# DIG-Beihang/RobustART

Measured on AMD Instinct MI355X. Metric: corrupted+attacked images/sec/node (ResNet-50, PGD-7 + IN-C x5), higher is better.
Workload: dtype bf16x3; 1 GPU; per step and GPU: gaussian_noise sev 1..5 on 256 u8 224x224 images -> normalise -> ResNet-50 eval (1280 img) + PGD-Linf-7 eps 2/255 ResNet-50 eval (256 img); global_batch=256, parallelism=dp1, streams=2

## Files before the change

include/robustart_hip.h:

```cpp
#ifndef ROBUSTART_HIP_H
#define ROBUSTART_HIP_H

#include <stddef.h>
#include <stdint.h>

#ifdef __cplusplus
extern "C" {
#endif

typedef void* rart_stream_t;

typedef enum rart_status {
  RART_OK = 0,
  RART_ERR_INVALID = 1,
  RART_ERR_UNSUPPORTED = 2,
  RART_ERR_WORKSPACE = 3,
  RART_ERR_HIP = 4
} rart_status;

enum {
  RART_GAUSSIAN_NOISE = 0, RART_SHOT_NOISE = 1, RART_IMPULSE_NOISE = 2, RART_DEFOCUS_BLUR = 3,
  RART_GLASS_BLUR = 4, RART_MOTION_BLUR = 5, RART_ZOOM_BLUR = 6, RART_SNOW = 7, RART_FROST = 8,
  RART_FOG = 9, RART_BRIGHTNESS = 10, RART_CONTRAST = 11, RART_ELASTIC_TRANSFORM = 12,
  RART_PIXELATE = 13, RART_JPEG_COMPRESSION = 14, RART_SPECKLE_NOISE = 15, RART_GAUSSIAN_BLUR = 16,
// ... 123 lines not shown
int rart_logit_loss(const float* logits, const int64_t* y, const int64_t* y_target, int batch, int classes,
                    int kind, float scale, float* loss_out, float* dlogits_out, int32_t* pred_out,
                    rart_stream_t stream);

typedef struct rart_conv_desc {
  const void* src;
  const void* wgt;
  const float* bias;
  const void* res;
  const void* mask;
  void* dst;
  int32_t batch, grid_h, grid_w;
  int32_t src_h, src_w, src_pix_stride;
  int32_t k_per_tap, n_taps;
  int32_t sy, sx;
  int32_t tap_dy[32], tap_dx[32];
  int64_t tap_src_off[32];
  int32_t n_cols;
  int32_t dst_h, dst_w, dst_sy, dst_sx, dst_oy, dst_ox, dst_pix_stride;
  int32_t flags;
  int32_t n_batched, z_inner, wgt_row_stride, reserved_;
  int64_t src_z_outer, src_z_inner, wgt_z_outer, wgt_z_inner, dst_z_outer, dst_z_inner;
  void* sign_out;
  int64_t dst_pair_off, res_pair_off;
  float* bn_stats_out;
} rart_conv_desc;

int rart_conv_igemm_bf16(const rart_conv_desc* desc_host, rart_stream_t stream);
int rart_igemm_set_bk64_min_k(long long k);
int rart_gemm_small_m_bf16(const void* a, int lda, const void* w, int ldw, const float* bias, void* out, int ldo, int out_is_f32, int m,
                           int n, int k, rart_stream_t stream);
int rart_igemm_set_gemm256(int enable);
int rart_gemm256_supported(long long rows, int k, int n_cols, int src_ld, int dst_ld);

typedef struct rart_gemm_pair_desc {
  const void *a_hi, *a_lo, *w_hi, *w_lo;
  const float* bias;
  const void *res_hi, *res_lo;
  void *dst_hi, *dst_lo;
  void *aux_hi, *aux_lo;
  int M, N, K, lda, ldw, ldc, w_rows;
  int rows_per_image, src_rows_per_image, src_row_off, dst_rows_per_image, dst_row_off;
  int flags, n_batched, z_inner;
  int64_t a_z_outer, a_z_inner, w_z_outer, w_z_inner, c_z_outer, c_z_inner;
  int conv, batch, grid_h, grid_w, src_h, src_w, sy, sx, k_per_tap, n_taps;
  int tap_dy[16], tap_dx[16];
  int dst_h, dst_w, dst_sy, dst_sx, dst_oy, dst_ox;
  const void* mask_bits;
  void* sign_out;
  int tile_n;
  int tile_m;
} rart_gemm_pair_desc;
int rart_gemm_pair_bf16(const rart_gemm_pair_desc* desc_host, rart_stream_t stream);
int rart_gemm_pair_set_schedule(int mode);
int rart_gemm_pair_get_schedule(void);

typedef struct rart_conv_tail_desc {
  const void* a_hi;  const void* a_lo;
  const void* w_hi;  const void* w_lo;
  const void* t_hi;  const void* t_lo;
  const float* bias_mid;
  const float* bias_out;
  const void* mask_mid;  const void* mask_out;
  void* sign_mid;  void* sign_out;
  const void* res_hi;  const void* res_lo;
  void* dst_hi;  void* dst_lo;
  int batch, h, w, c_mid, ldw, relu_mid, relu_out;
  int tap_dy[9], tap_dx[9];
  const void* n_hi;  const void* n_lo;
  const float* bias_next;
  const void* mask_next;
  void* sign_next;
  void* dstn_hi;  void* dstn_lo;
  int relu_next;
} rart_conv_tail_desc;
int rart_conv3x3_tail_pair_supported(int c_mid);
int rart_conv3x3_tail_pair(const rart_conv_tail_desc* desc_host, rart_stream_t stream);

int rart_vit_add_pos_cls_pair(void* x_hi, void* x_lo, const float* cls_pos0, const float* pos, int n, int tokens, int dim,
                              rart_stream_t stream);
int rart_layernorm_pair(const void* x_hi, const void* x_lo, const float* gamma, const float* beta, void* out_hi, void* out_lo, int rows,
                        int dim, int64_t in_row_stride, int64_t out_row_stride, float eps, rart_stream_t stream);
int rart_layernorm_bwd_pair(const void* dy_hi, const void* dy_lo, const void* x_hi, const void* x_lo, const float* gamma,
                            const void* res_hi, const void* res_lo, void* dx_hi, void* dx_lo, int rows, int dim, int64_t dy_row_stride,
                            int64_t x_row_stride, int64_t res_row_stride, int64_t dx_row_stride, float eps, rart_stream_t stream);
int rart_softmax_rows_pair(const float* scores, void* probs_hi, void* probs_lo, int64_t rows, int n_valid, int ld_in, int ld_out,
                           float scale, rart_stream_t stream);
int rart_softmax_bwd_rows_pair(const void* probs_hi, const void* probs_lo, const float* dprobs, void* ds_hi, void* ds_lo, int64_t rows,
                               int n_valid, int ld_p, int ld_dp, int ld_out, float scale, rart_stream_t stream);
int rart_vit_unpatchify_from_f32(const float* dpatches, float* grad, int n, int h, int w, int patch, int64_t ld, const float* std_host,
                                 rart_stream_t stream);
int rart_vit_attention_pair(const void* qkv_hi, const void* qkv_lo, void* out_hi, void* out_lo, int n, int tokens, int heads, int head_dim,
                            rart_stream_t stream);
int rart_vit_attention_bwd_pair(const void* qkv_hi, const void* qkv_lo, const void* out_hi, const void* out_lo, const void* dout_hi,
                                const void* dout_lo, void* dqkv_hi, void* dqkv_lo, float* stats, int n, int tokens, int heads, int head_dim,
                                rart_stream_t stream);

int rart_conv3x3_halo_supported(int channels, int h, int w);
int rart_conv3x3_pack_frag_bf16(const void* w_rows, void* w_frag, int channels, rart_stream_t stream);
int rart_pack_frag_bf16(const void* w_rows, void* w_frag, int rows, int k, rart_stream_t stream);
int rart_conv3x3_halo_bf16(const void* src, const void* wgt, const float* bias, const void* mask_bits, void* sign_out,
                           void* dst, int n, int h, int w, int channels, const int* tap_dy, const int* tap_dx, int relu,
                           rart_stream_t stream);

int rart_bottleneck_fused_supported(int c_io, int c_mid, int h, int w);
int rart_bottleneck_fused_bf16(const void* x, const void* w1, const void* w2, const void* w3, const float* b1, const float* b2,
                               const float* b3, void* m1, void* m2, void* m3, void* out, int n, int h, int w, int c_io,
                               int c_mid, const int* tap_dy, const int* tap_dx, int backward, rart_stream_t stream);

int rart_bottleneck_first_supported(int c_in, int c_mid, int c_out, int h, int w);
int rart_bottleneck_first_bf16(const void* x, const void* w1, const void* w2, const void* w3, const void* w4, const float* b1,
                               const float* b2, const float* b3, void* m1, void* m2, void* m3, void* out, int n, int h, int w,
                               int c_in, int c_mid, int c_out, const int* tap_dy, const int* tap_dx, int backward,
                               rart_stream_t stream);

int rart_bottleneck_s2_fwd_supported(int c_in, int c_mid, int c_out, int h, int w);
int rart_bottleneck_s2_fwd_bf16(const void* x, const void* w1, const void* w2, const void* w3, const void* wd, const float* b1,
                                const float* b2, const float* b3, void* m1, void* m2, void* m3, void* out, int n, int h, int w,
                                int c_in, int c_mid, int c_out, rart_stream_t stream);

int rart_bottleneck_s2_bwd_bf16(const void* g, const void* w3t, const void* w2t, const void* w1t, const void* wdt, const void* m2,
                                const void* m1, const void* m0, void* dx, int n, int h, int w, int c_in, int c_mid, int c_out,
                                rart_stream_t stream);

int rart_bottleneck14_fused_supported(int c_io, int c_mid, int h, int w);
int rart_bottleneck14_fused_bf16(const void* x, const void* w1, const void* w2, const void* w3, const float* b1, const float* b2,
                                 const float* b3, void* m1, void* m2, void* m3, void* out, int n, int h, int w, int c_io,
// ... 241 lines not shown
```

robustart_amd/_lib.py:

```python
import ctypes
import os

_HERE = os.path.dirname(os.path.abspath(__file__))
LIB_PATH = os.path.join(_HERE, 'lib', 'librobustart_hip.so')

c_void_p, c_int, c_size_t, c_u64, c_float = (ctypes.c_void_p, ctypes.c_int, ctypes.c_size_t,
                                              ctypes.c_uint64, ctypes.c_float)
c_double = ctypes.c_double

ABI_VERSION = 110

SIGNATURES = {
    'rart_version': (c_int, []),
    'rart_last_error_string': (ctypes.c_char_p, []),
    'rart_corruption_name': (ctypes.c_char_p, [c_int]),
    'rart_corrupt_workspace_bytes': (c_size_t, [c_int, c_int, c_int, c_int, c_int]),
    'rart_corrupt_u8': (c_int, [c_void_p, c_void_p, c_int, c_int, c_int, c_int, c_int, c_u64, c_u64,
                                ctypes.POINTER(c_void_p), c_int, c_void_p, c_size_t, c_void_p]),
    'rart_stencil_fixed_point_info': (c_int, [c_int, c_int, c_void_p, c_void_p, c_size_t]),
    'rart_noise_multi_u8': (c_int, [c_void_p, ctypes.POINTER(c_void_p), c_int, c_int, c_int, c_int, c_int, ctypes.POINTER(c_int),
                                    ctypes.POINTER(c_u64), c_u64, c_void_p]),
    'rart_frost_textures_u8': (c_int, [c_void_p, c_void_p, c_int, c_int, c_int, c_int, c_void_p, c_int, c_int, c_int, ctypes.POINTER(c_int),
                                       c_u64, c_u64, c_void_p]),
    'rart_pil_resize_workspace_bytes': (c_size_t, [c_int] * 10),
    'rart_pil_resize_u8': (c_int, [c_void_p, c_void_p] + [c_int] * 10 + [c_void_p, c_size_t, c_void_p]),
    'rart_cv_resize_workspace_bytes': (c_size_t, [c_int] * 10),
    'rart_cv_resize_u8': (c_int, [c_void_p, c_void_p] + [c_int] * 10 + [c_void_p, c_size_t, c_void_p]),
    'rart_u8_to_normalized': (c_int, [c_void_p, c_void_p, c_int, c_int, c_int, c_int, c_int, c_void_p]),
    'rart_u8_to_unit_f32_nchw': (c_int, [c_void_p, c_void_p, c_int, c_int, c_int, c_void_p]),
    'rart_rng_uniform_u32': (c_int, [c_void_p, c_int, c_size_t, c_u64, c_u64, c_int, c_void_p]),
    'rart_rng_normal_f32': (c_int, [c_void_p, c_int, c_size_t, c_u64, c_u64, c_int, c_void_p]),
    'rart_set_normal_generator': (c_int, [c_int]),
    'rart_get_normal_generator': (c_int, []),
    'rart_rng_noise_field_f32': (c_int, [c_void_p, c_int, c_size_t, c_u64, c_u64, c_void_p]),
    'rart_attack_workspace_bytes': (c_size_t, [c_int]),
    'rart_attack_init_linf': (c_int, [c_void_p, c_void_p, c_int, c_size_t, c_float, c_float, c_float,
                                      c_u64, c_u64, c_void_p, c_void_p, c_void_p]),
    'rart_pgd_step_linf': (c_int, [c_void_p, c_void_p, c_void_p, c_size_t, c_float, c_float, c_void_p]),
    'rart_pgd_step_l2': (c_int, [c_void_p, c_void_p, c_void_p, c_int, c_size_t, c_float, c_float,
                                 c_void_p, c_size_t, c_void_p]),
    'rart_pgd_step_l1': (c_int, [c_void_p, c_void_p, c_void_p, c_int, c_size_t, c_float, c_float,
                                 c_void_p, c_size_t, c_void_p]),
    'rart_random_start_l1': (c_int, [c_void_p, c_void_p, c_int, c_size_t, c_float, c_u64, c_u64, c_void_p, c_void_p, c_void_p,
                                     c_void_p, c_size_t, c_void_p]),
    'rart_mim_step': (c_int, [c_void_p, c_void_p, c_void_p, c_void_p, c_int, c_size_t, c_float, c_float,
                              c_float, c_void_p, c_size_t, c_void_p]),
    'rart_apgd_init': (c_int, [c_void_p, c_void_p, c_int, c_size_t, c_int, c_float, c_u64, c_u64, c_void_p,
                               c_void_p, c_void_p, c_size_t, c_void_p]),
    'rart_apgd_step': (c_int, [c_void_p, c_void_p, c_void_p, c_void_p, c_void_p, c_int, c_size_t, c_int,
                               c_float, c_float, c_void_p, c_size_t, c_void_p]),
    'rart_square_init_linf': (c_int, [c_void_p, c_void_p, c_int, c_int, c_int, c_int, c_float, c_u64, c_u64, c_void_p, c_void_p,
                                      c_void_p]),
    'rart_rng_signs_f32': (c_int, [c_void_p, c_int, c_int, c_u64, c_u64, c_void_p, c_int, ctypes.c_uint32, c_void_p]),
    'rart_rng_normal_rows_f32': (c_int, [c_void_p, c_int, c_size_t, c_u64, c_void_p, c_int, c_void_p]),
    'rart_square_propose_linf': (c_int, [c_void_p, c_void_p, c_void_p, c_int, c_int, c_int, c_int, c_float, c_int, c_int,
                                         c_int, c_void_p, c_void_p]),
    'rart_fab_project_linf': (c_int, [c_void_p, c_void_p, c_void_p, c_void_p, c_void_p, c_int, c_size_t, c_void_p]),
    'rart_row_dot': (c_int, [c_void_p, c_void_p, c_void_p, c_int, c_size_t, c_void_p]),
    'rart_row_absmax_diff': (c_int, [c_void_p, c_void_p, c_void_p, c_int, c_size_t, c_void_p]),
    'rart_eot_accumulate': (c_int, [c_void_p, c_void_p, c_size_t, c_int, c_float, c_void_p]),
    'rart_square_init_lp': (c_int, [c_void_p, c_void_p, c_int, c_int, c_int, c_int, c_float, c_int, c_int, c_int, c_int, c_int, c_void_p,
                                    c_void_p, c_void_p, c_void_p]),
    'rart_square_propose_lp': (c_int, [c_void_p, c_void_p, c_void_p, c_int, c_int, c_int, c_int, c_float, c_int, c_int, c_int, c_int, c_int,
                                       c_int, c_void_p, c_void_p, c_void_p]),
    'rart_fab_project': (c_int, [c_void_p, c_void_p, c_void_p, c_void_p, c_void_p, c_int, c_size_t, c_int, c_void_p]),
    'rart_row_norm_diff': (c_int, [c_void_p, c_void_p, c_void_p, c_int, c_size_t, c_int, c_void_p]),
    'rart_fab_update': (c_int, [c_void_p, c_void_p, c_void_p, c_void_p, c_void_p, c_int, c_size_t, c_float, c_void_p]),
    'rart_fab_backoff': (c_int, [c_void_p, c_void_p, c_void_p, c_int, c_size_t, c_float, c_void_p]),
    'rart_l1_project': (c_int, [c_void_p, c_void_p, c_void_p, c_int, c_size_t, c_float, c_int, c_int, c_void_p]),
    'rart_row_kth_abs': (c_int, [c_void_p, c_void_p, c_void_p, c_int, c_size_t, c_void_p]),
    'rart_apgd_l1_move': (c_int, [c_void_p, c_void_p, c_void_p, c_void_p, c_void_p, c_void_p, c_int, c_size_t, c_void_p]),
    'rart_row_count_diff': (c_int, [c_void_p, c_void_p, c_void_p, c_int, c_size_t, c_void_p]),
    'rart_select_rows': (c_int, [c_void_p, c_void_p, c_void_p, c_int, c_size_t, c_void_p]),
    'rart_logit_loss': (c_int, [c_void_p, c_void_p, c_void_p, c_int, c_int, c_int, c_float, c_void_p,
                                c_void_p, c_void_p, c_void_p]),
    'rart_conv_igemm_bf16': (c_int, [c_void_p, c_void_p]),
    'rart_conv3x3_halo_supported': (c_int, [c_int, c_int, c_int]),
    'rart_conv3x3_pack_frag_bf16': (c_int, [c_void_p, c_void_p, c_int, c_void_p]),
    'rart_pack_frag_bf16': (c_int, [c_void_p, c_void_p, c_int, c_int, c_void_p]),
    'rart_conv3x3_halo_bf16': (c_int, [c_void_p, c_void_p, c_void_p, c_void_p, c_void_p, c_void_p, c_int, c_int, c_int, c_int,
                                       ctypes.POINTER(c_int), ctypes.POINTER(c_int), c_int, c_void_p]),
    'rart_bottleneck28_fused_supported': (c_int, [c_int, c_int, c_int, c_int]),
    'rart_bottleneck28_fused_bf16': (c_int, [c_void_p] * 11 + [c_int] * 5 + [ctypes.POINTER(c_int), ctypes.POINTER(c_int), c_int,
                                             c_void_p]),
    'rart_bottleneck7_fused_supported': (c_int, [c_int, c_int, c_int, c_int]),
    'rart_bottleneck7_fused_bf16': (c_int, [c_void_p] * 11 + [c_int] * 5 + [ctypes.POINTER(c_int), ctypes.POINTER(c_int), c_int,
                                            c_void_p]),
    'rart_bottleneck_s2_fwd_supported': (c_int, [c_int] * 5),
    'rart_bottleneck_s2_fwd_bf16': (c_int, [c_void_p] * 12 + [c_int] * 6 + [c_void_p]),
    'rart_bottleneck_s2_bwd_bf16': (c_int, [c_void_p] * 9 + [c_int] * 6 + [c_void_p]),
    'rart_bottleneck14_fused_supported': (c_int, [c_int, c_int, c_int, c_int]),
    'rart_bottleneck14_fused_bf16': (c_int, [c_void_p] * 11 + [c_int] * 5 + [ctypes.POINTER(c_int), ctypes.POINTER(c_int), c_int,
                                             c_void_p]),
    'rart_bottleneck_fused_supported': (c_int, [c_int, c_int, c_int, c_int]),
    'rart_bottleneck_first_supported': (c_int, [c_int] * 5),
    'rart_bottleneck_first_bf16': (c_int, [c_void_p] * 12 + [c_int] * 6 + [ctypes.POINTER(c_int), ctypes.POINTER(c_int), c_int,
                                           c_void_p]),
    'rart_bottleneck_fused_bf16': (c_int, [c_void_p] * 11 + [c_int] * 5 + [ctypes.POINTER(c_int), ctypes.POINTER(c_int), c_int,
                                           c_void_p]),
    'rart_igemm_set_bk64_min_k': (c_int, [ctypes.c_longlong]),
    'rart_gemm_small_m_bf16': (c_int, [c_void_p, c_int, c_void_p, c_int, c_void_p, c_void_p, c_int, c_int, c_int, c_int, c_int, c_void_p]),
    'rart_igemm_set_gemm256': (c_int, [c_int]),
    'rart_gemm256_supported': (c_int, [ctypes.c_longlong, c_int, c_int, c_int, c_int]),
    'rart_gemm_pair_bf16': (c_int, [c_void_p, c_void_p]),
    'rart_copy_calibration': (c_int, [c_void_p, c_void_p, ctypes.c_size_t, c_int, c_void_p]),
    'rart_gemm_pair_set_schedule': (c_int, [c_int]),
    'rart_gemm_pair_get_schedule': (c_int, []),
    'rart_pack_jobs_bf16': (c_int, [c_void_p, c_int, c_int, c_void_p]),
    'rart_vit_add_pos_cls_pair': (c_int, [c_void_p, c_void_p, c_void_p, c_void_p, c_int, c_int, c_int, c_void_p]),
    'rart_layernorm_pair': (c_int, [c_void_p] * 6 + [c_int, c_int, ctypes.c_int64, ctypes.c_int64, c_float, c_void_p]),
    'rart_layernorm_bwd_pair': (c_int, [c_void_p] * 9 + [c_int, c_int] + [ctypes.c_int64] * 4 + [c_float, c_void_p]),
    'rart_softmax_rows_pair': (c_int, [c_void_p, c_void_p, c_void_p, ctypes.c_int64, c_int, c_int, c_int, c_float, c_void_p]),
    'rart_softmax_bwd_rows_pair': (c_int, [c_void_p] * 5 + [ctypes.c_int64, c_int, c_int, c_int, c_int, c_float, c_void_p]),
    'rart_vit_attention_pair': (c_int, [c_void_p, c_void_p, c_void_p, c_void_p, c_int, c_int, c_int, c_int, c_void_p]),
    'rart_vit_attention_bwd_pair': (c_int, [c_void_p] * 9 + [c_int, c_int, c_int, c_int, c_void_p]),
    'rart_vit_unpatchify_from_f32': (c_int, [c_void_p, c_void_p, c_int, c_int, c_int, c_int, ctypes.c_int64, ctypes.POINTER(c_float), c_void_p]),
    'rart_engine_prep_input': (c_int, [c_void_p, c_int, c_void_p, c_void_p, c_int, c_int, c_int, c_void_p, c_void_p,
                                       c_void_p]),
    'rart_engine_maxpool': (c_int, [c_void_p, c_void_p, c_void_p, c_int, c_int, c_int, c_int, c_void_p]),
    'rart_engine_maxpool_keep': (c_int, [c_void_p, c_void_p, c_void_p, c_void_p, c_int, c_int, c_int, c_int, c_void_p]),
    'rart_engine_maxpool_bwd': (c_int, [c_void_p, c_void_p, c_void_p, c_void_p, c_int, c_int, c_int, c_int, c_void_p]),
    'rart_engine_avgpool': (c_int, [c_void_p, c_void_p, c_int, c_int, c_int, c_void_p]),
    'rart_engine_avgpool_bwd': (c_int, [c_void_p, c_void_p, c_void_p, c_int, c_int, c_int, c_void_p]),
    'rart_engine_stem_col2im': (c_int, [c_void_p, c_void_p, c_int, c_int, c_int, c_int, c_void_p, c_void_p]),
    'rart_engine_stem_fwd_fused': (c_int, [c_void_p, c_int, c_void_p, c_int, c_void_p, c_void_p, c_void_p, c_void_p, c_int, c_int,
                                           c_int, c_void_p, c_void_p, c_void_p]),
    'rart_wgrad_direct_supported': (c_int, [c_int, c_int, c_int]),
    'rart_wgrad_direct_bf16': (c_int, [c_void_p, c_void_p, c_void_p] + [c_int] * 10 + [c_void_p, c_void_p, c_int, c_int, c_int, c_void_p]),
    'rart_conv3x3_tail_pair_supported': (c_int, [c_int]),
# ... 107 lines not shown
                ('k_per_tap', ctypes.c_int32), ('n_taps', ctypes.c_int32), ('sy', ctypes.c_int32), ('sx', ctypes.c_int32),
                ('tap_dy', ctypes.c_int32 * 32), ('tap_dx', ctypes.c_int32 * 32), ('tap_src_off', ctypes.c_int64 * 32),
                ('n_cols', ctypes.c_int32),
                ('dst_h', ctypes.c_int32), ('dst_w', ctypes.c_int32), ('dst_sy', ctypes.c_int32), ('dst_sx', ctypes.c_int32),
                ('dst_oy', ctypes.c_int32), ('dst_ox', ctypes.c_int32), ('dst_pix_stride', ctypes.c_int32),
                ('flags', ctypes.c_int32),
                ('n_batched', ctypes.c_int32), ('z_inner', ctypes.c_int32), ('wgt_row_stride', ctypes.c_int32),
                ('reserved_', ctypes.c_int32),
                ('src_z_outer', ctypes.c_int64), ('src_z_inner', ctypes.c_int64), ('wgt_z_outer', ctypes.c_int64),
                ('wgt_z_inner', ctypes.c_int64), ('dst_z_outer', ctypes.c_int64), ('dst_z_inner', ctypes.c_int64),
                ('sign_out', c_void_p), ('dst_pair_off', ctypes.c_int64), ('res_pair_off', ctypes.c_int64), ('bn_stats_out', c_void_p)]


class JitterRec(ctypes.Structure):
    _fields_ = [('op', ctypes.c_uint8 * 4), ('factor', ctypes.c_float * 3), ('hue_shift', ctypes.c_uint32)]


class JpegInfo(ctypes.Structure):
    _fields_ = [(n, ctypes.c_int32) for n in ('status', 'height', 'width', 'ncomp')] + \
               [(n, ctypes.c_int32 * 3) for n in ('h_samp', 'v_samp', 'blocks_w', 'blocks_h')] + \
               [('coef_count', ctypes.c_int64), ('qt', (ctypes.c_uint16 * 64) * 3)]


class JpegDesc(ctypes.Structure):
    _fields_ = [('block_start', ctypes.c_int64 * 3), ('plane_off', ctypes.c_int64 * 3), ('qt_off', ctypes.c_int64),
                ('out_off', ctypes.c_int64)] + \
               [(n, ctypes.c_int32) for n in ('height', 'width', 'ncomp', 'h_samp', 'v_samp')] + \
               [('blocks_w', ctypes.c_int32 * 3), ('blocks_h', ctypes.c_int32 * 3), ('reserved_', ctypes.c_int32)]


class FixedPointInfo(ctypes.Structure):
    _fields_ = [(n, ctypes.c_int32) for n in ('kind', 'ksize', 'n_steps', 'frac_bits', 'out_frac_bits')] + \
               [('corr', ctypes.c_longlong), ('band', ctypes.c_longlong), ('max_abs_weight_error', ctypes.c_double),
                ('sum_abs_weight_error', ctypes.c_double)]


class PackJob(ctypes.Structure):
    _fields_ = [(n, ctypes.c_int32) for n in ('kind', 'n_out', 'channels', 'r', 's', 'n_taps', 'transpose', 'rows_padded', 'rows', 'k')] + \
               [('tap_r', ctypes.c_int32 * 16), ('tap_s', ctypes.c_int32 * 16), ('weight', c_void_p), ('out_channel_scale', c_void_p),
                ('src16', c_void_p), ('out', c_void_p)]


class GemmPairDesc(ctypes.Structure):
    _fields_ = [(n, c_void_p) for n in ('a_hi', 'a_lo', 'w_hi', 'w_lo', 'bias', 'res_hi', 'res_lo', 'dst_hi', 'dst_lo', 'aux_hi', 'aux_lo')] + \
               [(n, ctypes.c_int32) for n in ('M', 'N', 'K', 'lda', 'ldw', 'ldc', 'w_rows', 'rows_per_image', 'src_rows_per_image',
                                              'src_row_off', 'dst_rows_per_image', 'dst_row_off', 'flags', 'n_batched', 'z_inner')] + \
               [(n, ctypes.c_int64) for n in ('a_z_outer', 'a_z_inner', 'w_z_outer', 'w_z_inner', 'c_z_outer', 'c_z_inner')] + \
               [(n, ctypes.c_int32) for n in ('conv', 'batch', 'grid_h', 'grid_w', 'src_h', 'src_w', 'sy', 'sx', 'k_per_tap', 'n_taps')] + \
               [('tap_dy', ctypes.c_int32 * 16), ('tap_dx', ctypes.c_int32 * 16)] + \
               [(n, ctypes.c_int32) for n in ('dst_h', 'dst_w', 'dst_sy', 'dst_sx', 'dst_oy', 'dst_ox')] + \
               [('mask_bits', c_void_p), ('sign_out', c_void_p), ('tile_n', ctypes.c_int32), ('tile_m', ctypes.c_int32)]


class TokmixDesc(ctypes.Structure):
    _fields_ = [(n, c_void_p) for n in ('a_hi', 'a_lo', 'x_hi', 'x_lo', 'dst_hi', 'dst_lo', 'res_hi', 'res_lo', 'aux_hi', 'aux_lo', 'bias')] + \
               [(n, ctypes.c_int32) for n in ('M', 'N', 'K', 'lda', 'ldx', 'ldc', 'batch', 'flags')] + \
               [(n, ctypes.c_int64) for n in ('x_stride', 'c_stride')]


class TokmixWgradDesc(ctypes.Structure):
    _fields_ = [(n, c_void_p) for n in ('p', 'q', 'partial')] + \
               [(n, ctypes.c_int32) for n in ('M', 'N', 'D', 'batch', 'splits', 'images_per_split', 'ld_partial', 'reserved')] + \
               [(n, ctypes.c_int64) for n in ('p_stride', 'q_stride')]


class ConvTailDesc(ctypes.Structure):
    _fields_ = [(n, c_void_p) for n in ('a_hi', 'a_lo', 'w_hi', 'w_lo', 't_hi', 't_lo', 'bias_mid', 'bias_out', 'mask_mid', 'mask_out',
                                        'sign_mid', 'sign_out', 'res_hi', 'res_lo', 'dst_hi', 'dst_lo')] + \
               [(n, ctypes.c_int32) for n in ('batch', 'h', 'w', 'c_mid', 'ldw', 'relu_mid', 'relu_out')] + \
               [('tap_dy', ctypes.c_int32 * 9), ('tap_dx', ctypes.c_int32 * 9)] + \
               [(n, c_void_p) for n in ('n_hi', 'n_lo', 'bias_next', 'mask_next', 'sign_next', 'dstn_hi', 'dstn_lo')] + [('relu_next', ctypes.c_int32)]


_lib = None


class RartError(RuntimeError):

    def __init__(self, status, message):
        super().__init__('robustart_hip status %d: %s' % (status, message))
        self.status = status


def load():
    global _lib
    if _lib is not None:
        return _lib
    if not os.path.exists(LIB_PATH):
        raise RuntimeError(
            'robustart_amd: %s is missing -- build it with `python robustart_amd/csrc/build.py` '
            '(or __graft_entry__.build()).  There is no CPU fallback for the product path.' % LIB_PATH)
    import torch
    lib = ctypes.CDLL(LIB_PATH)
    for name, (res, args) in SIGNATURES.items():
        fn = getattr(lib, name)
        fn.restype = res
        fn.argtypes = args
    got = lib.rart_version()
    if got != ABI_VERSION:
        raise RuntimeError('robustart_amd: %s reports ABI version %d, this binding expects %d (struct layouts / signatures '
                           'differ) -- rebuild it with `python robustart_amd/csrc/build.py --force`' % (LIB_PATH, got, ABI_VERSION))
    _lib = lib
    return lib


def check(status):
    if status != 0:
        raise RartError(status, load().rart_last_error_string().decode('utf-8', 'replace'))


def require_gpu():
    import torch
    if not torch.cuda.is_available():
        raise RuntimeError('robustart_amd: no GPU visible (torch.cuda.is_available() is False); '
                           'the HIP hot path has no CPU fallback')
    return torch


def stream_ptr():
    import torch
    return c_void_p(torch.cuda.current_stream().cuda_stream)


def ptr(t):
# ... 18 lines not shown
```

robustart_amd/csrc/conv_tail_pair.hip:

```cpp
#include "rart_common.h"
#include "rart_lds_dma.h"

typedef __attribute__((ext_vector_type(8))) __bf16 bf16x8;
typedef __attribute__((ext_vector_type(16))) float f32x16;

namespace {
constexpr int CT_TM = 128;
constexpr int CT_LDE = 68;
constexpr int CT_PLANE_A = CT_TM * 64;
constexpr int CT_NLD = 144;
constexpr int CT_WREG = 2 * 32 * CT_NLD;
static_assert(CT_WREG >= 32 * CT_LDE * 4, "the staging must fit the wave's region");

struct ConvTailDev {
  const uint16_t *a_hi, *a_lo, *w_hi, *w_lo, *t_hi, *t_lo;
  const float *bias_mid, *bias_out;
  const uint8_t *mask_mid, *mask_out;
  uint8_t *sign_mid, *sign_out;
  const uint16_t *res_hi, *res_lo;
  uint16_t *dst_hi, *dst_lo;
  int M, H, W, ldw, relu_mid, relu_out;
  int tap_dy[9], tap_dx[9];
  uint32_t w_magic, w_shift, h_magic, h_shift;
  const uint16_t *n_hi, *n_lo;
  const float* bias_next;
  const uint8_t* mask_next;
  uint8_t* sign_next;
  uint16_t *dstn_hi, *dstn_lo;
  int relu_next;
};
typedef __attribute__((ext_vector_type(4))) uint32_t ct_u4;
__device__ __forceinline__ uint4 ct_nt_load(const uint16_t* p) {
  const ct_u4 v = __builtin_nontemporal_load(reinterpret_cast<const ct_u4*>(p));
  return make_uint4(v[0], v[1], v[2], v[3]);
}
__device__ __forceinline__ void ct_nt_store(uint16_t* p, const uint4& v) {
  ct_u4 w = {v.x, v.y, v.z, v.w};
  __builtin_nontemporal_store(w, reinterpret_cast<ct_u4*>(p));
}
__device__ __forceinline__ uint32_t ct_fastdiv(uint32_t n, uint32_t magic, uint32_t shift) { return (uint32_t)(((uint64_t)n * magic) >> shift); }

__device__ __forceinline__ uint32_t ct_pack_bf16x2(float lo, float hi) {
  typedef __attribute__((ext_vector_type(2))) float f2_t;
  typedef __attribute__((ext_vector_type(2))) __bf16 b2_t;
  f2_t f = {lo, hi};
  return __builtin_bit_cast(uint32_t, __builtin_convertvector(f, b2_t));
}
__device__ __forceinline__ void ct_split8(const float* v, uint4& hi, uint4& lo) {
  uint32_t h[4], l[4];
#pragma unroll
  for (int j = 0; j < 4; ++j) {
    h[j] = ct_pack_bf16x2(v[2 * j], v[2 * j + 1]);
    l[j] = ct_pack_bf16x2(v[2 * j] - __uint_as_float(h[j] << 16), v[2 * j + 1] - __uint_as_float(h[j] & 0xFFFF0000u));
  }
  hi = make_uint4(h[0], h[1], h[2], h[3]);
  lo = make_uint4(l[0], l[1], l[2], l[3]);
}
__device__ __forceinline__ void ct_join8(const uint4& hi, const uint4& lo, float* v) {
  const uint32_t h[4] = {hi.x, hi.y, hi.z, hi.w}, l[4] = {lo.x, lo.y, lo.z, lo.w};
#pragma unroll
  for (int j = 0; j < 4; ++j) {
    v[2 * j] = __uint_as_float(h[j] << 16) + __uint_as_float(l[j] << 16);
    v[2 * j + 1] = __uint_as_float(h[j] & 0xFFFF0000u) + __uint_as_float(l[j] & 0xFFFF0000u);
  }
}
__device__ __forceinline__ uint32_t ct_sign_byte(const uint4& v) {
  const uint32_t hw[4] = {v.x, v.y, v.z, v.w};
  uint32_t sb = 0;
#pragma unroll
  for (int j = 0; j < 4; ++j) {
    sb |= ((short)(hw[j] & 0xFFFFu) > 0 ? 1u : 0u) << (2 * j);
    sb |= ((short)(hw[j] >> 16) > 0 ? 1u : 0u) << (2 * j + 1);
  }
  return sb;
}

template <int NJ>
__device__ __forceinline__ void ct_pointwise_frags(const f32x16* acc, const uint32_t* mw, bool relu, int h, uint4* fh, uint4* fl) {
#pragma unroll
  for (int j = 0; j < NJ; ++j)
#pragma unroll
    for (int ge = 0; ge < 4; ge += 2) {
      uint32_t eh[2], el[2], oh[2], ol[2];
#pragma unroll
      for (int w = 0; w < 2; ++w) {
        float ve[2], vo[2];
#pragma unroll
        for (int i = 0; i < 2; ++i) {
          ve[i] = acc[j][4 * ge + 2 * w + i];
          vo[i] = acc[j][4 * ge + 4 + 2 * w + i];
          if (relu) { ve[i] = fmaxf(ve[i], 0.f); vo[i] = fmaxf(vo[i], 0.f); }
          if (!((mw[j] >> (8 * ge + 4 * h + 2 * w + i)) & 1u)) ve[i] = 0.f;
          if (!((mw[j] >> (8 * ge + 8 + 4 * h + 2 * w + i)) & 1u)) vo[i] = 0.f;
        }
        eh[w] = ct_pack_bf16x2(ve[0], ve[1]);
        el[w] = ct_pack_bf16x2(ve[0] - __uint_as_float(eh[w] << 16), ve[1] - __uint_as_float(eh[w] & 0xFFFF0000u));
        oh[w] = ct_pack_bf16x2(vo[0], vo[1]);
        ol[w] = ct_pack_bf16x2(vo[0] - __uint_as_float(oh[w] << 16), vo[1] - __uint_as_float(oh[w] & 0xFFFF0000u));
        const auto sh = __builtin_amdgcn_permlane32_swap(eh[w], oh[w], false, false);
        eh[w] = sh[0]; oh[w] = sh[1];
        const auto sl = __builtin_amdgcn_permlane32_swap(el[w], ol[w], false, false);
        el[w] = sl[0]; ol[w] = sl[1];
      }
      fh[j * 2 + ge / 2] = make_uint4(eh[0], eh[1], oh[0], oh[1]);
      fl[j * 2 + ge / 2] = make_uint4(el[0], el[1], ol[0], ol[1]);
    }
}

template <int C, bool NEXT>
__global__ __launch_bounds__(256, (C == 64 && !NEXT) ? 3 : 2) void k_conv3x3_tail_pair(const ConvTailDev d) {
  constexpr int NJ = C / 32;
  constexpr int KS = C / 16;
  constexpr int NOUT = 4 * C, NC = NOUT / 64;
  constexpr int TPT_SHIFT = C == 64 ? 1 : 2;
  constexpr int KT = 9 << TPT_SHIFT;
  constexpr int PLANE_B = C * 64, STAGE = 2 * CT_PLANE_A + 2 * PLANE_B;
  constexpr int BQ = (C / 16) / 4;
  static_assert(4 * CT_WREG <= 2 * STAGE, "the waves' epilogue regions must fit the tile buffers");
  __shared__ __attribute__((aligned(16))) uint8_t lds[2 * STAGE];
  const int tid = threadIdx.x, lane = tid & 63;
  const int wave = __builtin_amdgcn_readfirstlane(tid >> 6);
  uint32_t tile;
  {
    const uint32_t nb = gridDim.x, bid = blockIdx.x, xcd = bid & 7u, slot = bid >> 3, q = nb >> 3, r = nb & 7u;
    tile = (xcd < r ? xcd * (q + 1u) : r * (q + 1u) + (xcd - r) * q) + slot;
  }
  const int m0 = (int)tile * CT_TM;

  uint32_t avoff[2], nok[2] = {0u, 0u};
  int tap_min = 0;
  for (int t = 0; t < 9; ++t) tap_min = min(tap_min, (d.tap_dy[t] * d.W + d.tap_dx[t]) * (C * 2));
  const int tapreg = lane < 9 ? (d.tap_dy[lane] * d.W + d.tap_dx[lane]) * (C * 2) - tap_min : 0;
#pragma unroll
  for (int q = 0; q < 2; ++q) {
    const int r = 16 * (wave + 4 * q) + (lane >> 2);
    const int cs = ((lane & 3) ^ ((r >> 2) & 3)) * 16;
    const int m = m0 + r;
    const bool ok = m < d.M;
    const uint32_t mm = ok ? (uint32_t)m : 0u;
    const uint32_t t = ct_fastdiv(mm, d.w_magic, d.w_shift);
    const int ax = (int)(mm - t * (uint32_t)d.W);
    const int n = (int)ct_fastdiv(t, d.h_magic, d.h_shift);
    const int ay = (int)(t - (uint32_t)n * (uint32_t)d.H);
    avoff[q] = (uint32_t)((n * d.H * d.W + ay * d.W + ax) * (C * 2) + cs);
    for (int t2 = 0; t2 < 9; ++t2) {
      const int iy = ay + d.tap_dy[t2], ix = ax + d.tap_dx[t2];
      if (!(ok && (unsigned)iy < (unsigned)d.H && (unsigned)ix < (unsigned)d.W)) nok[q] |= 1u << t2;
    }
  }
  uint32_t wvoff[BQ];
#pragma unroll
  for (int q = 0; q < BQ; ++q) {
    const int r = 16 * (wave + 4 * q) + (lane >> 2);
    wvoff[q] = (uint32_t)((r * d.ldw + (((lane & 3) ^ ((r >> 2) & 3)) * 8)) * 2);
  }
  const rart_srd_t srd_ah = rart_dma_srd(reinterpret_cast<const char*>(d.a_hi) + tap_min), srd_al = rart_dma_srd(reinterpret_cast<const char*>(d.a_lo) + tap_min);
  const rart_srd_t srd_wh = rart_dma_srd(d.w_hi), srd_wl = rart_dma_srd(d.w_lo);
  const uint32_t lds_base = (uint32_t)(uintptr_t)(__attribute__((address_space(3))) uint8_t*)lds;
#define RART_CT_ISSUE(KT_, BUF)                                                                                 \
  {                                                                                                             \
    const uint32_t st_ = lds_base + (BUF)*STAGE;                                                                \
    const int kt_ = (KT_);                                                                                      \
    const int tap_ = kt_ >> TPT_SHIFT;                                                                          \
// ... 19 lines not shown
    for (int g = 0; g < 4; ++g) {
      float4 bv = make_float4(0.f, 0.f, 0.f, 0.f);
      if (d.bias_mid) bv = *reinterpret_cast<const float4*>(d.bias_mid + j * 32 + 8 * g + 4 * h);
      acc[j][4 * g] = bv.x; acc[j][4 * g + 1] = bv.y; acc[j][4 * g + 2] = bv.z; acc[j][4 * g + 3] = bv.w;
    }
  RART_CT_ISSUE(0, 0)
  rart_dma_wait<0>();
  __syncthreads();
  for (int kt = 0; kt < KT; ++kt) {
    const int buf = kt & 1;
    if (kt + 1 < KT) RART_CT_ISSUE(kt + 1, buf ^ 1)
    const uint8_t* Pb = lds + buf * STAGE + (wave * 32) * 64;
    const uint8_t* Wb = lds + buf * STAGE + 2 * CT_PLANE_A;
#pragma unroll
    for (int ks = 0; ks < 2; ++ks) {
      const bf16x8 ph = *reinterpret_cast<const bf16x8*>(Pb + xo[ks]);
      const bf16x8 pl = *reinterpret_cast<const bf16x8*>(Pb + CT_PLANE_A + xo[ks]);
#pragma unroll
      for (int j = 0; j < NJ; ++j) {
        const bf16x8 wh = *reinterpret_cast<const bf16x8*>(Wb + j * 32 * 64 + xo[ks]);
        const bf16x8 wl = *reinterpret_cast<const bf16x8*>(Wb + PLANE_B + j * 32 * 64 + xo[ks]);
        acc[j] = __builtin_amdgcn_mfma_f32_32x32x16_bf16(wh, pl, acc[j], 0, 0, 0);
        acc[j] = __builtin_amdgcn_mfma_f32_32x32x16_bf16(wl, ph, acc[j], 0, 0, 0);
        acc[j] = __builtin_amdgcn_mfma_f32_32x32x16_bf16(wh, ph, acc[j], 0, 0, 0);
      }
    }
    rart_dma_wait<0>();
    __syncthreads();
  }
#undef RART_CT_ISSUE

  const int p = m0 + wave * 32 + fr;
  const bool p_ok = p < d.M;
  bf16x8 a2h[KS], a2l[KS];
  {
    uint32_t mw[NJ];
#pragma unroll
    for (int j = 0; j < NJ; ++j) mw[j] = 0xFFFFFFFFu;
    if (d.mask_mid && p_ok) {
      const uint32_t* mp = reinterpret_cast<const uint32_t*>(d.mask_mid + (size_t)p * (C / 8));
#pragma unroll
      for (int j = 0; j < NJ; ++j) mw[j] = mp[j];
    }
    uint4 fh[KS], fl[KS];
    ct_pointwise_frags<NJ>(acc, mw, d.relu_mid != 0, h, fh, fl);
#pragma unroll
    for (int s = 0; s < KS; ++s) {
      a2h[s] = __builtin_bit_cast(bf16x8, fh[s]);
      a2l[s] = __builtin_bit_cast(bf16x8, fl[s]);
      if (d.sign_mid && p_ok) d.sign_mid[(size_t)p * (C / 8) + 2 * s + h] = (uint8_t)ct_sign_byte(fh[s]);
    }
  }

  uint8_t* const wreg = lds + wave * CT_WREG;
  float* sE = reinterpret_cast<float*>(wreg);
  const int cw = lane & 7, rw = lane >> 3;
  f32x16 accn[NEXT ? NJ : 1];
  if (NEXT) {
#pragma unroll
    for (int j = 0; j < NJ; ++j)
#pragma unroll
      for (int g = 0; g < 4; ++g) {
        float4 bv = make_float4(0.f, 0.f, 0.f, 0.f);
        if (d.bias_next) bv = *reinterpret_cast<const float4*>(d.bias_next + j * 32 + 8 * g + 4 * h);
        accn[j][4 * g] = bv.x; accn[j][4 * g + 1] = bv.y; accn[j][4 * g + 2] = bv.z; accn[j][4 * g + 3] = bv.w;
      }
  }
  const uint4* th_base = reinterpret_cast<const uint4*>(d.t_hi) + lane;
  const uint4* tl_base = reinterpret_cast<const uint4*>(d.t_lo) + lane;
  const bool relu_out = d.relu_out != 0;
#pragma unroll 1
  for (int c = 0; c < NC; ++c) {
    int eo[4];
    uint4 rh[4], rl[4];
    uint32_t mb[4];
#pragma unroll
    for (int q = 0; q < 4; ++q) {
      const int pp = m0 + wave * 32 + q * 8 + rw;
      eo[q] = -1;
      rh[q] = rl[q] = make_uint4(0, 0, 0, 0);
      mb[q] = 0xFFu;
      if (pp < d.M) {
        const int e = pp * NOUT + c * 64 + cw * 8;
        eo[q] = e;
        if (d.res_hi) {
          rh[q] = ct_nt_load(d.res_hi + e);
          rl[q] = ct_nt_load(d.res_lo + e);
        }
        if (d.mask_out) mb[q] = d.mask_out[e >> 3];
      }
    }
    f32x16 acc2[2];
#pragma unroll
    for (int b = 0; b < 2; ++b) {
#pragma unroll
      for (int g = 0; g < 4; ++g) {
        float4 bv = make_float4(0.f, 0.f, 0.f, 0.f);
        if (d.bias_out) bv = *reinterpret_cast<const float4*>(d.bias_out + c * 64 + b * 32 + 8 * g + 4 * h);
        acc2[b][4 * g] = bv.x; acc2[b][4 * g + 1] = bv.y; acc2[b][4 * g + 2] = bv.z; acc2[b][4 * g + 3] = bv.w;
      }
#pragma unroll
      for (int sg = 0; sg < KS; sg += 4) {
        uint4 th[4], tl[4];
#pragma unroll
        for (int s = 0; s < 4; ++s) {
          th[s] = th_base[((c * 2 + b) * KS + sg + s) * 64];
          tl[s] = tl_base[((c * 2 + b) * KS + sg + s) * 64];
        }
#pragma unroll
        for (int s = 0; s < 4; ++s) {
          const bf16x8 wh = __builtin_bit_cast(bf16x8, th[s]), wl = __builtin_bit_cast(bf16x8, tl[s]);
          acc2[b] = __builtin_amdgcn_mfma_f32_32x32x16_bf16(wh, a2l[sg + s], acc2[b], 0, 0, 0);
          acc2[b] = __builtin_amdgcn_mfma_f32_32x32x16_bf16(wl, a2h[sg + s], acc2[b], 0, 0, 0);
          acc2[b] = __builtin_amdgcn_mfma_f32_32x32x16_bf16(wh, a2h[sg + s], acc2[b], 0, 0, 0);
        }
      }
    }
#pragma unroll
    for (int b = 0; b < 2; ++b)
#pragma unroll
      for (int g = 0; g < 4; ++g)
        *reinterpret_cast<float4*>(sE + fr * CT_LDE + b * 32 + 8 * g + 4 * h) =
            make_float4(acc2[b][4 * g], acc2[b][4 * g + 1], acc2[b][4 * g + 2], acc2[b][4 * g + 3]);
    __builtin_amdgcn_fence(__ATOMIC_RELEASE, "wavefront");
    __builtin_amdgcn_wave_barrier();
    __builtin_amdgcn_fence(__ATOMIC_ACQUIRE, "wavefront");
    uint4 oph[4], opl[4];
#pragma unroll
    for (int q = 0; q < 4; ++q) {
      const int r = q * 8 + rw;
      const float4 v0 = *reinterpret_cast<const float4*>(sE + r * CT_LDE + cw * 8);
      const float4 v1 = *reinterpret_cast<const float4*>(sE + r * CT_LDE + cw * 8 + 4);
      const int e = eo[q];
      oph[q] = opl[q] = make_uint4(0, 0, 0, 0);
      if (e >= 0) {
        float v[8] = {v0.x, v0.y, v0.z, v0.w, v1.x, v1.y, v1.z, v1.w};
        if (d.res_hi) {
          float rv[8];
          ct_join8(rh[q], rl[q], rv);
#pragma unroll
          for (int j = 0; j < 8; ++j) v[j] += rv[j];
        }
#pragma unroll
        for (int j = 0; j < 8; ++j)
          if (!((mb[q] >> j) & 1u)) v[j] = 0.f;
        if (relu_out) {
#pragma unroll
          for (int j = 0; j < 8; ++j) v[j] = fmaxf(v[j], 0.f);
        }
        uint4 ph, pl;
        ct_split8(v, ph, pl);
        ct_nt_store(d.dst_hi + e, ph);
        ct_nt_store(d.dst_lo + e, pl);
        if (d.sign_out) d.sign_out[e >> 3] = (uint8_t)ct_sign_byte(ph);
        oph[q] = ph;
        opl[q] = pl;
      }
    }
    __builtin_amdgcn_fence(__ATOMIC_RELEASE, "wavefront");
    __builtin_amdgcn_wave_barrier();
    if (NEXT) {
#pragma unroll
      for (int q = 0; q < 4; ++q) {
        *reinterpret_cast<uint4*>(wreg + (q * 8 + rw) * CT_NLD + cw * 16) = oph[q];
        *reinterpret_cast<uint4*>(wreg + 32 * CT_NLD + (q * 8 + rw) * CT_NLD + cw * 16) = opl[q];
      }
      __builtin_amdgcn_fence(__ATOMIC_RELEASE, "wavefront");
      __builtin_amdgcn_wave_barrier();
      __builtin_amdgcn_fence(__ATOMIC_ACQUIRE, "wavefront");
// ... 17 lines not shown
        for (int s = 0; s < 4; ++s) {
          const bf16x8 wh = __builtin_bit_cast(bf16x8, nh[s]), wl = __builtin_bit_cast(bf16x8, nl[s]);
          accn[j] = __builtin_amdgcn_mfma_f32_32x32x16_bf16(wh, xl[s], accn[j], 0, 0, 0);
          accn[j] = __builtin_amdgcn_mfma_f32_32x32x16_bf16(wl, xh[s], accn[j], 0, 0, 0);
          accn[j] = __builtin_amdgcn_mfma_f32_32x32x16_bf16(wh, xh[s], accn[j], 0, 0, 0);
        }
      }
      __builtin_amdgcn_fence(__ATOMIC_RELEASE, "wavefront");
      __builtin_amdgcn_wave_barrier();
    }
  }
  if (NEXT) {
    uint32_t mw[NJ];
#pragma unroll
    for (int j = 0; j < NJ; ++j) mw[j] = 0xFFFFFFFFu;
    if (d.mask_next && p_ok) {
      const uint32_t* mp = reinterpret_cast<const uint32_t*>(d.mask_next + (size_t)p * (C / 8));
#pragma unroll
      for (int j = 0; j < NJ; ++j) mw[j] = mp[j];
    }
    uint4 fh[KS], fl[KS];
    ct_pointwise_frags<NJ>(accn, mw, d.relu_next != 0, h, fh, fl);
    if (p_ok) {
#pragma unroll
      for (int s = 0; s < KS; ++s) {
        ct_nt_store(d.dstn_hi + (size_t)p * C + 16 * s + 8 * h, fh[s]);
        ct_nt_store(d.dstn_lo + (size_t)p * C + 16 * s + 8 * h, fl[s]);
        if (d.sign_next) d.sign_next[(size_t)p * (C / 8) + 2 * s + h] = (uint8_t)ct_sign_byte(fh[s]);
      }
    }
  }
}

void ct_magic(uint32_t dv, uint32_t& mg, uint32_t& sh) {
  uint32_t l = 0;
  while ((1ull << l) < dv) ++l;
  sh = 31 + l;
  mg = (uint32_t)(((1ull << sh) + dv - 1) / dv);
}
}

extern "C" int rart_conv3x3_tail_pair_supported(int c_mid) { return (c_mid == 64 || c_mid == 128) ? 1 : 0; }

extern "C" int rart_conv3x3_tail_pair(const rart_conv_tail_desc* t, rart_stream_t stream) {
  RART_CHECK_ARG(t != nullptr, "rart_conv3x3_tail_pair: null descriptor");
  RART_CHECK_ARG(t->a_hi && t->a_lo && t->w_hi && t->w_lo && t->t_hi && t->t_lo && t->dst_hi && t->dst_lo,
                 "rart_conv3x3_tail_pair: null operand plane");
  RART_CHECK_ARG(t->c_mid == 64 || t->c_mid == 128, "rart_conv3x3_tail_pair: c_mid must be 64 or 128 (layer1 / layer2)");
  RART_CHECK_ARG(t->batch > 0 && t->h > 0 && t->w > 0, "rart_conv3x3_tail_pair: empty geometry");
  RART_CHECK_ARG((t->res_hi == nullptr) == (t->res_lo == nullptr), "rart_conv3x3_tail_pair: the skip is a pair: both planes or none");
  RART_CHECK_ARG(t->ldw % 8 == 0 && t->ldw >= 9 * t->c_mid, "rart_conv3x3_tail_pair: ldw must cover 9 taps x c_mid and keep 16-byte alignment");
  const long long M = (long long)t->batch * t->h * t->w;
  RART_CHECK_ARG(M * 4 * t->c_mid < (1ll << 31), "rart_conv3x3_tail_pair: tensors must stay below 2^31 elements (split the batch)");
  ConvTailDev d;
  d.a_hi = (const uint16_t*)t->a_hi; d.a_lo = (const uint16_t*)t->a_lo; d.w_hi = (const uint16_t*)t->w_hi; d.w_lo = (const uint16_t*)t->w_lo;
  d.t_hi = (const uint16_t*)t->t_hi; d.t_lo = (const uint16_t*)t->t_lo;
  d.bias_mid = t->bias_mid; d.bias_out = t->bias_out;
  d.mask_mid = (const uint8_t*)t->mask_mid; d.mask_out = (const uint8_t*)t->mask_out;
  d.sign_mid = (uint8_t*)t->sign_mid; d.sign_out = (uint8_t*)t->sign_out;
  d.res_hi = (const uint16_t*)t->res_hi; d.res_lo = (const uint16_t*)t->res_lo;
  d.dst_hi = (uint16_t*)t->dst_hi; d.dst_lo = (uint16_t*)t->dst_lo;
  d.M = (int)M; d.H = t->h; d.W = t->w; d.ldw = t->ldw; d.relu_mid = t->relu_mid; d.relu_out = t->relu_out;
  for (int i = 0; i < 9; ++i) { d.tap_dy[i] = t->tap_dy[i]; d.tap_dx[i] = t->tap_dx[i]; }
  const bool next = t->n_hi != nullptr;
  RART_CHECK_ARG(!next || (t->n_lo && t->dstn_hi && t->dstn_lo), "rart_conv3x3_tail_pair: the neighbour's reduction needs both table planes and its destination pair");
  d.n_hi = (const uint16_t*)t->n_hi; d.n_lo = (const uint16_t*)t->n_lo; d.bias_next = t->bias_next; d.mask_next = (const uint8_t*)t->mask_next;
  d.sign_next = (uint8_t*)t->sign_next; d.dstn_hi = (uint16_t*)t->dstn_hi; d.dstn_lo = (uint16_t*)t->dstn_lo; d.relu_next = t->relu_next;
  ct_magic((uint32_t)d.W, d.w_magic, d.w_shift);
  ct_magic((uint32_t)d.H, d.h_magic, d.h_shift);
  const dim3 grid((uint32_t)((M + CT_TM - 1) / CT_TM));
  hipStream_t st = (hipStream_t)stream;
  if (t->c_mid == 64) {
    if (next) hipLaunchKernelGGL((k_conv3x3_tail_pair<64, true>), grid, dim3(256), 0, st, d);
    else hipLaunchKernelGGL((k_conv3x3_tail_pair<64, false>), grid, dim3(256), 0, st, d);
  } else {
    if (next) hipLaunchKernelGGL((k_conv3x3_tail_pair<128, true>), grid, dim3(256), 0, st, d);
    else hipLaunchKernelGGL((k_conv3x3_tail_pair<128, false>), grid, dim3(256), 0, st, d);
  }
  RART_CHECK_LAUNCH("rart_conv3x3_tail_pair");
  return RART_OK;
}
```

robustart_amd/csrc/gemm_pair.hip:

```cpp
#include "rart_common.h"
#include <stdlib.h>

#include "rart_gemm_pair_dev.h"
#include "rart_lds_dma.h"

namespace {
template <int TM, int TN, bool CONV>
__global__ __launch_bounds__(TM * 2, 1) void k_gemm_pair(const GemmPairDev d) {
  constexpr int NW = TM / 32;
  constexpr int WN = (TN / 64 < NW) ? TN / 64 : NW, WM = NW / WN, RW = TM / WM, MI = RW / 32, NJ = TN / (32 * WN);
  static_assert(NJ == 2, "a wave owns 64 columns");
  constexpr int GP_PLANE_A = TM * GP_BK * 2;
  constexpr int PLANE_B = TN * GP_BK * 2, STAGE = 2 * GP_PLANE_A + 2 * PLANE_B;
  constexpr int A_PIECES = TM / 16, AQ = A_PIECES / NW;
  constexpr int B_PIECES = TN / 16, BQ = (B_PIECES + NW - 1) / NW;
  constexpr int GP_STAGING = NW * 32 * GP_LDE * 4;
  static_assert(AQ == 2, "two A pieces per wave");
  static_assert(GP_STAGING + TM * 4 <= 2 * STAGE, "epilogue staging + row table must fit the tile buffers");
  __shared__ __attribute__((aligned(16))) uint8_t lds[2 * STAGE];
  const int tid = threadIdx.x, lane = tid & 63;
  const int wave = __builtin_amdgcn_readfirstlane(tid >> 6), wm = wave / WN, wn = wave % WN;
  const uint16_t *a_hi = d.a_hi, *a_lo = d.a_lo, *w_hi = d.w_hi, *w_lo = d.w_lo;
  long long c_off = 0;
  if (!CONV && gridDim.y > 1) {
    const int z = blockIdx.y, zo = z / d.z_inner, zi = z - zo * d.z_inner;
    const long long ao = zo * d.a_zo + zi * d.a_zi, wo = zo * d.w_zo + zi * d.w_zi;
    a_hi += ao; a_lo += ao; w_hi += wo; w_lo += wo;
    c_off = zo * d.c_zo + zi * d.c_zi;
  }
  const int TMV = d.tile_rows;
  const int n_tiles = (d.N + TN - 1) / TN, m_tiles = (d.M + TMV - 1) / TMV;
  int m_tile, n_tile;
  if (m_tiles >= 16) {
    const int bid = blockIdx.x, xcd = bid & 7, slot = bid >> 3;
    m_tile = (slot / n_tiles) * 8 + xcd;
    n_tile = slot % n_tiles;
    if (m_tile >= m_tiles) return;
  } else {
    m_tile = blockIdx.x / n_tiles;
    n_tile = blockIdx.x - m_tile * n_tiles;
  }
  const int m0 = m_tile * TMV, n0 = n_tile * TN;

  uint32_t avoff[2], nok[2] = {0u, 0u};
  int tapreg = 0, tap_min = 0;
  const bool one_tap = !CONV || d.n_taps == 1;
  if (CONV) {
    for (int t = 0; t < d.n_taps; ++t) tap_min = min(tap_min, (d.tap_dy[t] * d.src_w + d.tap_dx[t]) * d.lda * 2);
    if (lane < d.n_taps) tapreg = (d.tap_dy[lane] * d.src_w + d.tap_dx[lane]) * d.lda * 2 - tap_min;
  }
  const uint32_t tap0 = CONV ? (uint32_t)__builtin_amdgcn_readfirstlane((d.tap_dy[0] * d.src_w + d.tap_dx[0]) * d.lda * 2 - tap_min) : 0u;
#pragma unroll
  for (int q = 0; q < 2; ++q) {
    const int r = 16 * (wave + NW * q) + (lane >> 2);
    const int csrc = (lane & 3) ^ ((r >> 2) & 3);
    const int m = m0 + r;
    const bool ok = m < d.M;
    if (CONV) {
      const uint32_t mm = ok ? (uint32_t)m : 0u;
      const uint32_t t = gp_fastdiv(mm, d.gw_magic, d.gw_shift);
      const int ox = (int)(mm - t * (uint32_t)d.grid_w);
      const int n = (int)gp_fastdiv(t, d.gh_magic, d.gh_shift);
      const int oy = (int)(t - (uint32_t)n * (uint32_t)d.grid_h);
      const int by = oy * d.sy, bx = ox * d.sx;
      avoff[q] = (uint32_t)((n * d.src_h * d.src_w + by * d.src_w + bx) * d.lda * 2 + csrc * 16);
      for (int t2 = 0; t2 < d.n_taps; ++t2) {
        const int iy = by + d.tap_dy[t2], ix = bx + d.tap_dx[t2];
        if (!(ok && (unsigned)iy < (unsigned)d.src_h && (unsigned)ix < (unsigned)d.src_w)) nok[q] |= 1u << t2;
      }
      if (one_tap && (nok[q] & 1u)) avoff[q] = RART_DMA_OOR;
    } else {
      long long srow = m;
      if (d.map_rows) {
        const int img = m / d.rpi;
        srow = (long long)img * d.src_rpi + (m - img * d.rpi);
      }
      avoff[q] = ok ? (uint32_t)(((srow + d.src_off) * d.lda + csrc * 8) * 2) : RART_DMA_OOR;
    }
  }
  uint32_t wvoff[BQ];
#pragma unroll
  for (int q = 0; q < BQ; ++q) {
    const int r = 16 * (wave + NW * q) + (lane >> 2);
    const int csrc = (lane & 3) ^ ((r >> 2) & 3);
    const int n = n0 + r;
    wvoff[q] = (r < TN && n < d.w_rows) ? (uint32_t)((n * d.ldw + csrc * 8) * 2) : RART_DMA_OOR;
  }
  const rart_srd_t srd_ah = rart_dma_srd(reinterpret_cast<const char*>(a_hi) + tap_min), srd_al = rart_dma_srd(reinterpret_cast<const char*>(a_lo) + tap_min);
  const rart_srd_t srd_wh = rart_dma_srd(w_hi), srd_wl = rart_dma_srd(w_lo);
  const uint32_t lds_base = (uint32_t)(uintptr_t)(__attribute__((address_space(3))) uint8_t*)lds;
  const int w_step = (d.flags & GP_W_INTERLEAVED) ? 128 : 64;
#define RART_GP_ISSUE(KT, BUF)                                                                                  \
  {                                                                                                             \
    const uint32_t st_ = lds_base + (BUF)*STAGE;                                                                \
    const int kt_ = (KT);                                                                                       \
    if (one_tap) {                                                                                              \
      const uint32_t so_ = tap0 + (uint32_t)kt_ * 64u;                                                          \
      _Pragma("unroll") for (int q = 0; q < 2; ++q) {                                                           \
        rart_dma_load16(avoff[q], srd_ah, so_, st_ + (wave + NW * q) * 1024);                                   \
        rart_dma_load16(avoff[q], srd_al, so_, st_ + GP_PLANE_A + (wave + NW * q) * 1024);                      \
      }                                                                                                         \
    } else {                                                                                                    \
      const int tap_ = kt_ >> d.tpt_shift;                                                                      \
      const uint32_t so_ = (uint32_t)(__builtin_amdgcn_readlane(tapreg, tap_) + (kt_ - (tap_ << d.tpt_shift)) * 64); \
      _Pragma("unroll") for (int q = 0; q < 2; ++q) {                                                           \
        const uint32_t vo_ = avoff[q] | ((uint32_t)__builtin_amdgcn_sbfe(nok[q], tap_, 1) & RART_DMA_OOR);      \
        rart_dma_load16(vo_, srd_ah, so_, st_ + (wave + NW * q) * 1024);                                        \
        rart_dma_load16(vo_, srd_al, so_, st_ + GP_PLANE_A + (wave + NW * q) * 1024);                           \
      }                                                                                                         \
    }                                                                                                           \
    {                                                                                                           \
      const uint32_t so_ = (uint32_t)(kt_ * w_step);                                                            \
      _Pragma("unroll") for (int q = 0; q < BQ; ++q) {                                                          \
        if (NW * q + NW <= B_PIECES || wave + NW * q < B_PIECES) {     \
          rart_dma_load16(wvoff[q], srd_wh, so_, st_ + 2 * GP_PLANE_A + (wave + NW * q) * 1024);                \
          rart_dma_load16(wvoff[q], srd_wl, so_, st_ + 2 * GP_PLANE_A + PLANE_B + (wave + NW * q) * 1024);      \
        }                                                                                                       \
      }                                                                                                         \
    }                                                                                                           \
  }
  const int fr = lane & 31, h = lane >> 5;
  uint32_t xo[2];
#pragma unroll
  for (int ks = 0; ks < 2; ++ks) xo[ks] = (uint32_t)(fr * 64 + (((2 * ks + h) ^ ((fr >> 2) & 3)) << 4));
  f32x16 acc[MI][2];
#pragma unroll
  for (int j = 0; j < 2; ++j) {
    const int bc = n0 + wn * 64 + j * 32 + fr;
    const float bv = (d.bias && bc < d.N) ? d.bias[bc] : 0.f;
#pragma unroll
    for (int i = 0; i < MI; ++i)
#pragma unroll
      for (int r = 0; r < 16; ++r) acc[i][j][r] = bv;
  }
  const int KT = d.K / GP_BK;
  const bool skip_last = wm * RW + MI * 32 > TMV;
  RART_GP_ISSUE(0, 0)
  rart_dma_wait<0>();
  __syncthreads();
  for (int kt = 0; kt < KT; ++kt) {
    const int buf = kt & 1;
    if (kt + 1 < KT) RART_GP_ISSUE(kt + 1, buf ^ 1)
    const uint8_t* Ah = lds + buf * STAGE + (wm * RW) * 64;
    const uint8_t* Bh = lds + buf * STAGE + 2 * GP_PLANE_A + (wn * 64) * 64;
#pragma unroll
    for (int ks = 0; ks < 2; ++ks) {
      bf16x8 ah[MI], al[MI], bh[2], bl[2];
#pragma unroll
      for (int i = 0; i < MI; ++i) {
// ... 23 lines not shown
  gp_epilogue<TM, TN, CONV, MI>(d, lds, acc, m0, n0, c_off, TMV);
}

int g_pair_schedule = -1;
int gp_schedule() {
  if (g_pair_schedule < 0) {
    const char* e = getenv("RART_PAIR_SCHEDULE");
    g_pair_schedule = e ? atoi(e) : 1;
  }
  return g_pair_schedule;
}

int gp_rows224() {
  const char* e = getenv("RART_PAIR_ROWS224");
  return e ? atoi(e) : 1;
}
int gp_split() {
  const char* e = getenv("RART_PAIR_SPLIT");
  return e ? atoi(e) : 1;
}

void gp_magic(uint32_t dv, uint32_t& mg, uint32_t& sh) {
  uint32_t l = 0;
  while ((1ull << l) < dv) ++l;
  sh = 31 + l;
  mg = (uint32_t)(((1ull << sh) + dv - 1) / dv);
}
}

bool rart_gemm_pair_pp_launch(const void* dev_desc, int tn, bool conv, unsigned grid_x, unsigned grid_y, hipStream_t st, unsigned walk_wgs);
void rart_gemm_pair_ps_launch(const void* dev_desc, bool conv, unsigned wgs, hipStream_t st);

namespace {
int gp_cu_count() {
  static int cus[64] = {0};
  int dev = 0;
  if (hipGetDevice(&dev) != hipSuccess || dev < 0 || dev >= 64) return 256;
  if (cus[dev] == 0) {
    int n = 0;
    cus[dev] = (hipDeviceGetAttribute(&n, hipDeviceAttributeMultiprocessorCount, dev) == hipSuccess && n > 0) ? n : 256;
  }
  return cus[dev];
}
}

extern "C" int rart_gemm_pair_set_schedule(int mode) {
  RART_CHECK_ARG(mode >= 0 && mode <= 3,
                 "rart_gemm_pair_set_schedule: mode must be 0 (two-stage loop), 1 (ping-pong), 2 (ping-pong + deferred-epilogue persistent) or 3 (ping-pong, tiles walked)");
  g_pair_schedule = mode;
  return RART_OK;
}
extern "C" int rart_gemm_pair_get_schedule(void) { return gp_schedule(); }

extern "C" int rart_gemm_pair_bf16(const rart_gemm_pair_desc* h, rart_stream_t stream) {
  RART_CHECK_ARG(h != nullptr, "rart_gemm_pair_bf16: null descriptor");
  RART_CHECK_ARG(h->a_hi && h->a_lo && h->w_hi && h->w_lo && h->dst_hi, "rart_gemm_pair_bf16: null operand plane");
  const bool conv = h->conv != 0;
  GemmPairDev d;
  d.M = h->M; d.K = h->K;
  if (conv) {
    RART_CHECK_ARG(h->batch > 0 && h->grid_h > 0 && h->grid_w > 0 && h->src_h > 0 && h->src_w > 0 && h->dst_h > 0 && h->dst_w > 0,
                   "rart_gemm_pair_bf16 (conv): empty geometry");
    RART_CHECK_ARG(h->n_taps >= 1 && h->n_taps <= 16, "rart_gemm_pair_bf16 (conv): n_taps must be 1..16");
    RART_CHECK_ARG(h->k_per_tap >= 32 && (h->k_per_tap & (h->k_per_tap - 1)) == 0,
                   "rart_gemm_pair_bf16 (conv): k_per_tap must be a power of two >= 32");
    RART_CHECK_ARG(h->n_batched <= 1 && h->rows_per_image == 0 && h->src_row_off == 0 && h->dst_row_off == 0,
                   "rart_gemm_pair_bf16 (conv): no batching / row re-basing in conv mode");
    const long long M = (long long)h->batch * h->grid_h * h->grid_w;
    RART_CHECK_ARG(M < (1ll << 31), "rart_gemm_pair_bf16 (conv): row grid must stay below 2^31 rows");
    RART_CHECK_ARG((long long)h->batch * h->src_h * h->src_w * h->lda < (1ll << 30) && (long long)h->batch * h->dst_h * h->dst_w * h->ldc < (1ll << 31),
                   "rart_gemm_pair_bf16 (conv): a source plane must stay below 2 GiB (32-bit byte offsets of the stage loads) and the destination "
                   "below 2^31 elements (split the batch)");
    RART_CHECK_ARG(h->lda % 8 == 0 || h->lda == 4, "rart_gemm_pair_bf16 (conv): source pixels must keep 16-byte alignment of the K chunks");
    d.M = (int)M;
    d.K = h->k_per_tap * h->n_taps;
    d.grid_h = h->grid_h; d.grid_w = h->grid_w; d.src_h = h->src_h; d.src_w = h->src_w; d.sy = h->sy; d.sx = h->sx; d.n_taps = h->n_taps;
    int sh = 0;
    while ((32 << sh) < h->k_per_tap) ++sh;
    d.tpt_shift = sh;
    for (int i = 0; i < 16; ++i) { d.tap_dy[i] = i < h->n_taps ? h->tap_dy[i] : 0; d.tap_dx[i] = i < h->n_taps ? h->tap_dx[i] : 0; }
    d.dst_h = h->dst_h; d.dst_w = h->dst_w; d.dst_sy = h->dst_sy; d.dst_sx = h->dst_sx; d.dst_oy = h->dst_oy; d.dst_ox = h->dst_ox;
    gp_magic((uint32_t)d.grid_w, d.gw_magic, d.gw_shift);
    gp_magic((uint32_t)d.grid_h, d.gh_magic, d.gh_shift);
    d.mask_bits = (const uint8_t*)h->mask_bits; d.sign_out = (uint8_t*)h->sign_out;
    RART_CHECK_ARG(!(d.sign_out && (h->flags & GP_OUT_F32)), "rart_gemm_pair_bf16 (conv): sign_out needs a pair destination");
  } else {
    RART_CHECK_ARG(!h->mask_bits && !h->sign_out, "rart_gemm_pair_bf16: mask_bits / sign_out are served by conv mode only");
    RART_CHECK_ARG(h->lda % 8 == 0 && h->lda >= h->K, "rart_gemm_pair_bf16: lda must cover the row and keep 16-byte alignment");
    d.grid_h = d.grid_w = d.src_h = d.src_w = d.sy = d.sx = d.n_taps = 1; d.tpt_shift = 0;
    for (int i = 0; i < 16; ++i) d.tap_dy[i] = d.tap_dx[i] = 0;
    d.dst_h = d.dst_w = d.dst_sy = d.dst_sx = 1; d.dst_oy = d.dst_ox = 0;
    d.gw_magic = d.gw_shift = d.gh_magic = d.gh_shift = 0;
    d.mask_bits = nullptr; d.sign_out = nullptr;
  }
  d.N = h->N;
  RART_CHECK_ARG(d.M > 0 && d.N > 0 && d.N % 8 == 0, "rart_gemm_pair_bf16: M > 0, N a positive multiple of 8");
  RART_CHECK_ARG(d.K > 0 && d.K % GP_BK == 0, "rart_gemm_pair_bf16: K must be a positive multiple of 32");
  RART_CHECK_ARG(h->ldw % 8 == 0 && h->ldc % 8 == 0 && h->ldw >= d.K && h->ldc >= d.N,
                 "rart_gemm_pair_bf16: leading dimensions must cover the row and keep 16-byte alignment");
  RART_CHECK_ARG((long long)(h->w_rows > 0 ? h->w_rows : h->N) * h->ldw < (1ll << 30), "rart_gemm_pair_bf16: a weight plane must stay below 2 GiB");
  if (!conv) {
    const long long imgs = (h->rows_per_image > 0 && h->rows_per_image < d.M) ? (d.M + h->rows_per_image - 1) / h->rows_per_image : 1;
    const long long src_rows = imgs > 1 ? imgs * (h->src_rows_per_image > 0 ? h->src_rows_per_image : h->rows_per_image) : d.M;
    RART_CHECK_ARG((src_rows + h->src_row_off) * h->lda < (1ll << 30), "rart_gemm_pair_bf16: a source plane must stay below 2 GiB (per batched problem)");
  }
  const bool out_f32 = (h->flags & GP_OUT_F32) != 0;
  RART_CHECK_ARG(out_f32 || h->dst_lo, "rart_gemm_pair_bf16: a pair destination needs its lo plane");
  RART_CHECK_ARG((h->res_hi == nullptr) == (h->res_lo == nullptr), "rart_gemm_pair_bf16: the residual is a pair: both planes or none");
  RART_CHECK_ARG(!(h->flags & (GP_GELU_KEEP | GP_GELU_BWD)) || (h->aux_hi && h->aux_lo),
                 "rart_gemm_pair_bf16: GELU_KEEP / GELU_BWD need the pre-activation pair (aux)");
  RART_CHECK_ARG(!(h->flags & ~(GP_OUT_F32 | GP_GELU | GP_GELU_BWD | GP_GELU_KEEP | GP_RELU | GP_W_INTERLEAVED)), "rart_gemm_pair_bf16: unknown flag");
  RART_CHECK_ARG(!(h->flags & GP_W_INTERLEAVED) || h->ldw >= 2 * d.K, "rart_gemm_pair_bf16: an interleaved weight table has rows of 2 K elements");
  {
    const int g = (h->flags & GP_GELU ? 1 : 0) + (h->flags & GP_GELU_BWD ? 1 : 0) + (h->flags & GP_GELU_KEEP ? 1 : 0);
    RART_CHECK_ARG(g <= 1 && !((h->flags & GP_GELU_KEEP) && out_f32), "rart_gemm_pair_bf16: at most one GELU mode; GELU_KEEP writes pairs");
  }
  d.a_hi = (const uint16_t*)h->a_hi; d.a_lo = (const uint16_t*)h->a_lo; d.w_hi = (const uint16_t*)h->w_hi; d.w_lo = (const uint16_t*)h->w_lo;
  d.bias = h->bias; d.res_hi = (const uint16_t*)h->res_hi; d.res_lo = (const uint16_t*)h->res_lo;
  d.dst_hi = (uint16_t*)h->dst_hi; d.dst_lo = (uint16_t*)h->dst_lo; d.aux_hi = (uint16_t*)h->aux_hi; d.aux_lo = (uint16_t*)h->aux_lo;
  d.lda = h->lda; d.ldw = h->ldw; d.ldc = h->ldc;
  d.w_rows = h->w_rows > 0 ? h->w_rows : h->N;
  d.map_rows = (!conv && h->rows_per_image > 0 && h->rows_per_image < d.M) ? 1 : 0;
  d.rpi = d.map_rows ? h->rows_per_image : d.M;
  d.src_rpi = h->src_rows_per_image > 0 ? h->src_rows_per_image : d.rpi;
  d.dst_rpi = h->dst_rows_per_image > 0 ? h->dst_rows_per_image : d.rpi;
  d.src_off = h->src_row_off; d.dst_off = h->dst_row_off;
  RART_CHECK_ARG(d.src_off >= 0 && d.dst_off >= 0, "rart_gemm_pair_bf16: row offsets must be >= 0");
  d.flags = h->flags;
  {
    const char* e = getenv("RART_PAIR_NT_MIN_MB");
    const long long min_mb = e ? atoll(e) : 0;
    d.nt = (long long)d.M * d.N * 4 >= min_mb * (1ll << 20) ? 1 : 0;
  }
  const int nz = h->n_batched > 1 ? h->n_batched : 1;
  RART_CHECK_ARG(nz <= 65535, "rart_gemm_pair_bf16: n_batched must be <= 65535");
  d.z_inner = h->z_inner > 0 ? h->z_inner : 1;
  d.a_zo = h->a_z_outer; d.a_zi = h->a_z_inner; d.w_zo = h->w_z_outer; d.w_zi = h->w_z_inner; d.c_zo = h->c_z_outer; d.c_zi = h->c_z_inner;
  int tn = d.N <= 64 ? 64 : (d.N <= 128 ? 128 : 256), tm = 256;
  if (conv) {
    if (gp_schedule() >= 1 && d.N >= 256 && (d.K >= 512 || (d.K >= 256 && d.N <= 512))) {
      tm = 256;
      tn = (long long)((d.M + 255) / 256) * ((d.N + 255) / 256) < 128 ? 128 : 256;
    } else if (d.K <= 256) { tm = 256; tn = 64; }
    else if (d.K < 1024 || d.N <= 128) { tm = 128; tn = d.N <= 64 ? 64 : 128; }
    else if ((long long)((d.M + 255) / 256) * ((d.N + 255) / 256) < 128) { tm = 256; tn = 128; }
    if (d.M <= 256) { tm = 128; tn = 64; }
  }
  if (h->tile_n == 64 || h->tile_n == 128 || h->tile_n == 256) tn = h->tile_n;
  if (h->tile_m == 128 || h->tile_m == 256) tm = h->tile_m;
  if (h->tile_m == 224) tm = 256;
  const int m_tiles = (d.M + tm - 1) / tm, n_tiles = (d.N + tn - 1) / tn;
  const int m_enum = m_tiles >= 16 ? (m_tiles + 7) / 8 * 8 : m_tiles;
  const long long blocks = (long long)m_enum * n_tiles;
  RART_CHECK_ARG(blocks < (1ll << 31), "rart_gemm_pair_bf16: grid too large");
  const dim3 grid((uint32_t)blocks, nz);
  hipStream_t st = (hipStream_t)stream;
  if (gp_schedule() == 2 && tm == 256 && tn >= 128 && h->tile_n == 0 && h->tile_m == 0 && nz == 1 && !d.map_rows && d.src_off == 0 &&
      (conv ? d.n_taps == 1 : true) && !(h->flags & (GP_GELU | GP_GELU_BWD | GP_GELU_KEEP)) && d.K / GP_BK >= 6) {
    const int cus = gp_cu_count();
    const long long tiles = (long long)((d.M + 255) / 256) * ((d.N + 127) / 128);
    if (tiles >= 2ll * cus) {
      rart_gemm_pair_ps_launch(&d, conv, (unsigned)cus, st);
      RART_CHECK_LAUNCH("rart_gemm_pair_bf16 (persistent)");
      return RART_OK;
    }
  }
  d.m_begin = 0;
  d.tile_rows = 256;
  if (tm == 256 && tn >= 128 && gp_schedule() >= 1 && nz == 1 && (h->tile_m == 224 || (h->tile_m == 0 && gp_rows224()))) {
    auto passes = [&](int mt, int nt) { const int cx = gp_cu_count() / 8; return ((mt >= 16 ? (mt + 7) / 8 * nt : (mt * nt + 7) / 8) + cx - 1) / cx; };
    const int mt224 = (d.M + 223) / 224;
    if (h->tile_m == 224 || passes(mt224, n_tiles) * 0.92 < passes(m_tiles, n_tiles) - 0.01) {
      d.tile_rows = 224;
      const int me = mt224 >= 16 ? (mt224 + 7) / 8 * 8 : mt224;
      if (rart_gemm_pair_pp_launch(&d, tn, conv, (unsigned)(me * n_tiles), 1, st, 0)) {
        RART_CHECK_LAUNCH("rart_gemm_pair_bf16 (ping-pong, 224-row tiles)");
        return RART_OK;
      }
      d.tile_rows = 256;
    }
  }
  if (!conv && tm == 256 && tn == 256 && gp_schedule() >= 1 && gp_split() && nz == 1 && h->tile_n == 0 && h->tile_m == 0) {
    const int cx = gp_cu_count() / 8;
    auto passes = [&](int mt, int nt) { return ((mt >= 16 ? (mt + 7) / 8 * nt : (mt * nt + 7) / 8) + cx - 1) / cx; };
    const double half_cost = 0.8;
    const int n128 = (d.N + 127) / 128;
    double best = passes(m_tiles, n_tiles);
    int best_ma = 0;
    for (int pa = 1; pa < passes(m_tiles, n_tiles); ++pa) {
      const int ma = pa * cx / n_tiles * 8;
      if (ma < 16 || ma >= m_tiles) continue;
      const double c = passes(ma, n_tiles) + half_cost * passes(m_tiles - ma, n128) + 0.05;
      if (c < best - 0.1) { best = c; best_ma = ma; }
    }
    if (best_ma > 0) {
      GemmPairDev da = d, db = d;
      da.M = best_ma * 256;
      db.m_begin = best_ma * 256;
      const int mb = m_tiles - best_ma, mb_enum = mb >= 16 ? (mb + 7) / 8 * 8 : mb;
      if (rart_gemm_pair_pp_launch(&da, 256, conv, (unsigned)(best_ma * n_tiles), 1, st, 0) &&
          rart_gemm_pair_pp_launch(&db, 128, conv, (unsigned)(mb_enum * n128), 1, st, 0)) {
        RART_CHECK_LAUNCH("rart_gemm_pair_bf16 (ping-pong, remainder split)");
        return RART_OK;
      }
    }
  }
  const unsigned walk_wgs = (gp_schedule() == 3 && nz == 1 && blocks > (long long)gp_cu_count()) ? (unsigned)(gp_cu_count() & ~7) : 0u;
  if (tm == 256 && tn >= 128 && gp_schedule() >= 1 && rart_gemm_pair_pp_launch(&d, tn, conv, grid.x, grid.y, st, walk_wgs)) {
    RART_CHECK_LAUNCH("rart_gemm_pair_bf16 (ping-pong)");
    return RART_OK;
  }
  d.tile_rows = tm;
  dim3 grid2 = grid;
  if ((gp_rows224() == 2 || (gp_rows224() == 3 && d.K >= 1024)) && nz == 1 && h->tile_m == 0 && h->tile_n == 0 && gp_schedule() >= 1) {
    const int lds = 2 * (2 * tm * 64 + 2 * tn * 64), res = lds > 80 * 1024 ? 1 : (lds > 53 * 1024 ? 2 : 3), cx = gp_cu_count() / 8 * res;
    auto passes = [&](int mt) { return ((mt >= 16 ? (mt + 7) / 8 * n_tiles : (mt * n_tiles + 7) / 8) + cx - 1) / cx; };
    const int rows = tm - 32, mt2 = (d.M + rows - 1) / rows;
    if (passes(mt2) * (double)rows / tm * 1.03 < passes(m_tiles)) {
      d.tile_rows = rows;
      grid2 = dim3((uint32_t)((mt2 >= 16 ? (mt2 + 7) / 8 * 8 : mt2) * n_tiles), nz);
    }
  }
#define RART_GP_LAUNCH(TM_, TN_, CONV_) hipLaunchKernelGGL((k_gemm_pair<TM_, TN_, CONV_>), grid2, dim3(TM_ * 2), 0, st, d)
#define RART_GP_BY_TN(TM_, CONV_)                                          \
  do {                                                                     \
    if (tn == 64) RART_GP_LAUNCH(TM_, 64, CONV_);                          \
    else if (tn == 128) RART_GP_LAUNCH(TM_, 128, CONV_);                   \
    else RART_GP_LAUNCH(TM_, 256, CONV_);                                  \
  } while (0)
  if (conv) {
    if (tm == 128) RART_GP_BY_TN(128, true);
    else RART_GP_BY_TN(256, true);
  } else {
    if (tm == 128) RART_GP_BY_TN(128, false);
    else RART_GP_BY_TN(256, false);
  }
#undef RART_GP_BY_TN
#undef RART_GP_LAUNCH
  RART_CHECK_LAUNCH("rart_gemm_pair_bf16");
  return RART_OK;
}
```

robustart_amd/csrc/gemm_pair_pp.hip:

```cpp
#include "rart_common.h"
#include <stdlib.h>

#include "rart_gemm_pair_dev.h"
#include "rart_lds_dma.h"

namespace {

typedef rart_srd_t pp_srd_t;
__device__ __forceinline__ void pp_bload(uint32_t voff, pp_srd_t srd, uint32_t soff, uint32_t lds_addr) { rart_dma_load16(voff, srd, soff, lds_addr); }
__device__ __forceinline__ pp_srd_t pp_make_srd(const void* base) { return rart_dma_srd(base); }
constexpr uint32_t PP_OOR = RART_DMA_OOR;
template <int N>
__device__ __forceinline__ void pp_vmcnt() { rart_dma_wait<N>(); }
__device__ __forceinline__ void pp_slot_end() {
  __builtin_amdgcn_sched_barrier(0);
  __builtin_amdgcn_s_barrier();
  asm volatile("" ::: "memory");
  __builtin_amdgcn_sched_barrier(0);
}

#ifdef RART_PP_STAMPS
__device__ unsigned long long g_pp_stamps[2][16];
__device__ unsigned long long g_pp_trace[4096][4];
#define PP_T(V) const unsigned long long V = __builtin_amdgcn_s_memtime();
#define PP_ACC(I, A, B) st_acc[I] += (B) - (A);
#else
#define PP_T(V)
#define PP_ACC(I, A, B)
#endif
#ifdef RART_PP_KO_NOLOAD
#define PP_LOOP_LOADS false
#else
#define PP_LOOP_LOADS true
#endif
#ifdef RART_PP_KO_NOWAIT
#define PP_VM(N) ((void)0)
#else
#define PP_VM(N) pp_vmcnt<N>()
#endif

template <int TN, bool CONV, int OPT>
__global__ __launch_bounds__(512, 1) void k_gemm_pair_pp(const GemmPairDev d) {
  constexpr bool BAL = OPT & 1, WALK = OPT & 2;
  constexpr int TM = 256, NW = 8, WN = TN / 64, WM = NW / WN, RW = TM / WM, MI = RW / 32, MH = MI / 2;
  static_assert(TN == 256 || TN == 128, "column tiles of 256 or 128");
  constexpr int PLANE_A = TM * 64, PLANE_B = TN * 64, STAGE = 2 * PLANE_A + 2 * PLANE_B;
  constexpr int WQ = TN / 64;
  constexpr int WH = WQ / 2, NB = WH + 2;
  constexpr int N0 = 2, N1 = WQ + 2;
  constexpr int VM_ALPHA = BAL ? 3 * NB : 2 * N1 + N0, VM_BETA = BAL ? 2 + NB : N0 + N1, VM_GAMMA = BAL ? 2 + NB : 2 + N0 + N1,
                VM_DELTA = 2 * N0 + N1;
  constexpr int GP_STAGING = NW * 32 * GP_LDE * 4;
  static_assert(GP_STAGING + TM * 4 <= 2 * STAGE, "epilogue staging + row table must fit the tile buffers");
  constexpr int EP_OFF = WALK ? STAGE : 0;
  constexpr int LDS_BYTES = (WALK && STAGE + GP_STAGING + TM * 4 > 2 * STAGE) ? STAGE + GP_STAGING + TM * 4 : 2 * STAGE;
  __shared__ __attribute__((aligned(16))) uint8_t lds[LDS_BYTES];
  const uint32_t lds_base = (uint32_t)(uintptr_t)(__attribute__((address_space(3))) uint8_t*)lds;
#ifdef RART_PP_STAMPS
  unsigned long long t_tile = __builtin_amdgcn_s_memtime();
#endif
  const int tid = threadIdx.x, lane = tid & 63;
  const int wave = __builtin_amdgcn_readfirstlane(tid >> 6), wm = wave / WN, wn = wave % WN;
  const int g = wave >> 2, w4 = wave & 3, og = 1 - g;
  const uint16_t *a_hi = d.a_hi, *a_lo = d.a_lo, *w_hi = d.w_hi, *w_lo = d.w_lo;
  long long c_off = 0;
  if (!CONV && gridDim.y > 1) {
    const int z = blockIdx.y, zo = z / d.z_inner, zi = z - zo * d.z_inner;
    const long long ao = zo * d.a_zo + zi * d.a_zi, wo = zo * d.w_zo + zi * d.w_zi;
    a_hi += ao; a_lo += ao; w_hi += wo; w_lo += wo;
    c_off = zo * d.c_zo + zi * d.c_zi;
  }
  const int TMV = d.tile_rows;
  const int n_tiles = (d.N + TN - 1) / TN, m_tiles = (d.M - d.m_begin + TMV - 1) / TMV;
#define RART_PP_TILE_OF(BID, M0_, N0_, OK_)                                                                      \
  {                                                                                                              \
    const int bid_ = (BID);                                                                                      \
    int mt_, nt_;                                                                                                \
    if (m_tiles >= 16) {                                                                                         \
      const int xcd_ = bid_ & 7, slot_ = bid_ >> 3;                                                              \
      mt_ = (slot_ / n_tiles) * 8 + xcd_;                                                                        \
      nt_ = slot_ % n_tiles;                                                                                     \
    } else {                                                                                                     \
      mt_ = bid_ / n_tiles;                                                                                      \
      nt_ = bid_ - mt_ * n_tiles;                                                                                \
    }                                                                                                            \
    OK_ = mt_ < m_tiles;                                                                                         \
    M0_ = d.m_begin + mt_ * TMV; N0_ = nt_ * TN;                                                                             \
  }
  const int n_blocks = (m_tiles >= 16 ? (m_tiles + 7) / 8 * 8 : m_tiles) * n_tiles;
  int bid = blockIdx.x, m0 = 0, n0 = 0;
  {
    bool ok = false;
    while (bid < n_blocks) {
      RART_PP_TILE_OF(bid, m0, n0, ok)
      if (ok || !WALK) break;
      bid += gridDim.x;
    }
    if (!ok) return;
  }

  int pr[2];
#pragma unroll
  for (int q = 0; q < 2; ++q) {
    const int hh = q == 0 ? og : g;
    pr[q] = (WM == 2) ? og * 128 + hh * 64 + 16 * w4 : (2 * og + (w4 >> 1)) * 64 + hh * 32 + (w4 & 1) * 16;
  }
  uint32_t avoff[2], nok[2];
  int tapreg = 0, tap_min = 0;
  const bool one_tap = !CONV || d.n_taps == 1;
  if (CONV) {
    for (int t = 0; t < d.n_taps; ++t) tap_min = min(tap_min, (d.tap_dy[t] * d.src_w + d.tap_dx[t]) * d.lda * 2);
    if (lane < d.n_taps) tapreg = (d.tap_dy[lane] * d.src_w + d.tap_dx[lane]) * d.lda * 2 - tap_min;
  }
  const uint32_t tap0 = CONV ? (uint32_t)__builtin_amdgcn_readfirstlane((d.tap_dy[0] * d.src_w + d.tap_dx[0]) * d.lda * 2 - tap_min) : 0u;
  uint32_t wvoff[WQ];
#define RART_PP_ADDR(M0_, N0_)                                                                                   \
  {                                                                                                              \
    nok[0] = nok[1] = 0u;                                                                                        \
  _Pragma("unroll")                                                                                              \
    for (int q = 0; q < 2; ++q) {                                                                                \
      const int r = pr[q] + (lane >> 2);                                                                         \
      const int csrc = (lane & 3) ^ ((r >> 2) & 3);                                                              \
      const int m = (M0_) + r;                                                                                   \
      const bool ok = m < d.M && r < TMV;       \
      if (CONV) {                                                                                                \
        const uint32_t mm = ok ? (uint32_t)m : 0u;                                                               \
        const uint32_t t = gp_fastdiv(mm, d.gw_magic, d.gw_shift);                                               \
        const int ox = (int)(mm - t * (uint32_t)d.grid_w);                                                       \
        const int n = (int)gp_fastdiv(t, d.gh_magic, d.gh_shift);                                                \
        const int oy = (int)(t - (uint32_t)n * (uint32_t)d.grid_h);                                              \
        const int by = oy * d.sy, bx = ox * d.sx;                                                                \
        avoff[q] = (uint32_t)((n * d.src_h * d.src_w + by * d.src_w + bx) * d.lda * 2 + csrc * 16);              \
        for (int t2 = 0; t2 < d.n_taps; ++t2) {                                                                  \
          const int iy = by + d.tap_dy[t2], ix = bx + d.tap_dx[t2];                                              \
          if (!(ok && (unsigned)iy < (unsigned)d.src_h && (unsigned)ix < (unsigned)d.src_w)) nok[q] |= 1u << t2; \
        }                                                                                                        \
        if (one_tap && (nok[q] & 1u)) avoff[q] = PP_OOR;                                                         \
      } else {                                                                                                   \
        long long srow = m;                                                                                      \
        if (d.map_rows) {                                                                                        \
          const int img = m / d.rpi;                                                                             \
          srow = (long long)img * d.src_rpi + (m - img * d.rpi);                                                 \
        }                                                                                                        \
        avoff[q] = ok ? (uint32_t)(((srow + d.src_off) * d.lda + csrc * 8) * 2) : PP_OOR;                        \
      }                                                                                                          \
    }                                                                                                            \
  _Pragma("unroll")                                                                                              \
    for (int q = 0; q < WQ; ++q) {                                                                               \
      const int r = 16 * (w4 + 4 * q) + (lane >> 2);                                                             \
      const int csrc = (lane & 3) ^ ((r >> 2) & 3);                                                              \
      const int n = (N0_) + r;                                                                                   \
      wvoff[q] = n < d.w_rows ? (uint32_t)((n * d.ldw + csrc * 8) * 2) : PP_OOR;                                 \
    }                                                                                                            \
  }
  RART_PP_ADDR(m0, n0)
  const pp_srd_t srd_ah = pp_make_srd(reinterpret_cast<const char*>(a_hi) + tap_min), srd_al = pp_make_srd(reinterpret_cast<const char*>(a_lo) + tap_min);
  const pp_srd_t srd_w = pp_make_srd(g ? w_lo : w_hi);
  const int w_step = (d.flags & GP_W_INTERLEAVED) ? 128 : 64;
  const uint32_t w_dst = lds_base + 2 * PLANE_A + g * PLANE_B + w4 * 1024;
  const int KT = d.K / GP_BK;

#define RART_PP_ISSUE_A(Q, ST)                                                                                   \
  {                                                                                                              \
    const int s_ = (ST);                                                                                         \
    const uint32_t dst_ = lds_base + (s_ & 1) * STAGE + pr[Q] * 64;                                              \
    if (one_tap) {                                                                                               \
      const uint32_t so_ = tap0 + (uint32_t)s_ * 64u;                                                            \
      pp_bload(avoff[Q], srd_ah, so_, dst_);                                                                     \
      pp_bload(avoff[Q], srd_al, so_, dst_ + PLANE_A);                                                           \
    } else {                                                                                                     \
      const int tap_ = s_ >> d.tpt_shift;                                                                        \
      const uint32_t so_ = (uint32_t)(__builtin_amdgcn_readlane(tapreg, tap_) + (s_ - (tap_ << d.tpt_shift)) * 64); \
      const uint32_t vo_ = avoff[Q] | ((uint32_t)__builtin_amdgcn_sbfe(nok[Q], tap_, 1) & PP_OOR);               \
      pp_bload(vo_, srd_ah, so_, dst_);                                                                          \
      pp_bload(vo_, srd_al, so_, dst_ + PLANE_A);                                                                \
    }                                                                                                            \
  }
#define RART_PP_ISSUE_W(ST, Q0, Q1)                                                                              \
  {                                                                                                              \
    const int s_ = (ST);                                                                                         \
    const uint32_t so_ = (uint32_t)(s_ * w_step);                                                                \
    _Pragma("unroll") for (int q = (Q0); q < (Q1); ++q) pp_bload(wvoff[q], srd_w, so_, w_dst + (s_ & 1) * STAGE + q * 4096); \
  }

  const int fr = lane & 31, h = lane >> 5;
  uint32_t xo[2];
#pragma unroll
  for (int ks = 0; ks < 2; ++ks) xo[ks] = (uint32_t)(fr * 64 + (((2 * ks + h) ^ ((fr >> 2) & 3)) << 4));
  f32x16 acc[MI][2];
  RART_PP_ISSUE_W(0, 0, WQ)
  RART_PP_ISSUE_A(0, 0)
  RART_PP_ISSUE_A(1, 0)
  bf16x8 ah[MH][2], al[MH][2], bh[2][2], bl[2][2];
  const bool skip_last = wm * RW + MI * 32 > TMV;
#define RART_PP_READ_A(HALF)                                                                                     \
  _Pragma("unroll") for (int ii = 0; ii < MH; ++ii) if (!((HALF) == 1 && ii == MH - 1 && skip_last))           \
      _Pragma("unroll") for (int ks = 0; ks < 2; ++ks) {                                                        \
    ah[ii][ks] = *reinterpret_cast<const bf16x8*>(Ah + ((HALF)*MH + ii) * 32 * 64 + xo[ks]);                     \
    al[ii][ks] = *reinterpret_cast<const bf16x8*>(Ah + PLANE_A + ((HALF)*MH + ii) * 32 * 64 + xo[ks]);           \
  }
#ifdef RART_PP_KO_NOMFMA
#define RART_PP_MFMA(HALF)                                                                                       \
  _Pragma("unroll") for (int ks = 0; ks < 2; ++ks) _Pragma("unroll") for (int ii = 0; ii < MH; ++ii)           \
      _Pragma("unroll") for (int j = 0; j < 2; ++j)                                                             \
          asm volatile("" ::"v"(al[ii][ks]), "v"(ah[ii][ks]), "v"(bh[j][ks]), "v"(bl[j][ks]));
#else
#define RART_PP_MFMA(HALF)                                                                                       \
  __builtin_amdgcn_s_setprio(1);                                                                                 \
  _Pragma("unroll") for (int ks = 0; ks < 2; ++ks) _Pragma("unroll") for (int ii = 0; ii < MH; ++ii)           \
      if (!((HALF) == 1 && ii == MH - 1 && skip_last)) _Pragma("unroll") for (int j = 0; j < 2; ++j) {          \
    acc[(HALF)*MH + ii][j] = __builtin_amdgcn_mfma_f32_32x32x16_bf16(al[ii][ks], bh[j][ks], acc[(HALF)*MH + ii][j], 0, 0, 0); \
    acc[(HALF)*MH + ii][j] = __builtin_amdgcn_mfma_f32_32x32x16_bf16(ah[ii][ks], bl[j][ks], acc[(HALF)*MH + ii][j], 0, 0, 0); \
    acc[(HALF)*MH + ii][j] = __builtin_amdgcn_mfma_f32_32x32x16_bf16(ah[ii][ks], bh[j][ks], acc[(HALF)*MH + ii][j], 0, 0, 0); \
  }                                                                                                              \
  __builtin_amdgcn_s_setprio(0);
#endif
#ifdef RART_PP_STAMPS
  unsigned long long st_acc[12] = {0, 0, 0, 0, 0, 0, 0, 0, 0, 0, 0, 0};
#endif
// ... 353 lines not shown
      RART_PS_ISSUE_W(kt + 2, 0, WH)
      RART_PS_ISSUE_A(1, kt + 2)
#pragma unroll
      for (int ks = 0; ks < 2; ++ks) {
        ah[ks] = *reinterpret_cast<const bf16x8*>(Ah + 32 * 64 + xo[ks]);
        al[ks] = *reinterpret_cast<const bf16x8*>(Ah + PLANE_A + 32 * 64 + xo[ks]);
      }
      RART_PS_EP_STEP()
      asm volatile("s_waitcnt lgkmcnt(0)" ::: "memory");
      if (tail) pp_vmcnt<0>();
      else if (g) pp_vmcnt<VM_GAMMA>();
      else pp_vmcnt<VM_ALPHA>();
      pp_slot_end();
      RART_PS_MFMA(1)
      RART_PS_EP_STEP()
      asm volatile("s_waitcnt lgkmcnt(0)" ::: "memory");
      if (!g) {
        if (tail) pp_vmcnt<0>(); else pp_vmcnt<VM_BETA>();
      }
      pp_slot_end();
    }
#undef RART_PS_MFMA
    while (esp < NMS) { RART_PS_EP_STEP() }
#pragma unroll
    for (int i = 0; i < MI; ++i)
#pragma unroll
      for (int j = 0; j < 2; ++j) accp[i][j] = acc[i][j];
    esp = 0; n0p = n0; tabp = s % 3;
    par = (par + KT) & 1;
#pragma unroll
    for (int q = 0; q < 2; ++q) av[q] = avn[q];
#pragma unroll
    for (int q = 0; q < WQ; ++q) wv[q] = wvn[q];
    has_next = s + 2 < count;
    if (has_next) RART_PS_ADDR(first + s + 2, avn, wvn)
  }
  if (!g) pp_slot_end();
  pp_vmcnt<0>();
  __syncthreads();
  while (esp < NMS) { RART_PS_EP_STEP() }
#undef RART_PS_EP_STEP
#undef RART_PS_EP_PUT
#undef RART_PS_EP_LOAD
#undef RART_PS_ISSUE_W
#undef RART_PS_ISSUE_A
#undef RART_PS_ADDR
}

#ifndef RART_PP_DEFAULT_OPT
#define RART_PP_DEFAULT_OPT 1
#endif
template <int OPT>
bool pp_launch_opt(const GemmPairDev& d, int tn, bool conv, dim3 grid, hipStream_t st, unsigned walk_wgs = 0) {
  if (walk_wgs && !(OPT & 2)) return pp_launch_opt<OPT | 2>(d, tn, conv, dim3(walk_wgs < grid.x ? walk_wgs : grid.x, 1), st);
  if (tn == 256) {
    if (conv) hipLaunchKernelGGL((k_gemm_pair_pp<256, true, OPT>), grid, dim3(512), 0, st, d);
    else hipLaunchKernelGGL((k_gemm_pair_pp<256, false, OPT>), grid, dim3(512), 0, st, d);
  } else if (tn == 128) {
    if (conv) hipLaunchKernelGGL((k_gemm_pair_pp<128, true, OPT>), grid, dim3(512), 0, st, d);
    else hipLaunchKernelGGL((k_gemm_pair_pp<128, false, OPT>), grid, dim3(512), 0, st, d);
  } else {
    return false;
  }
  return true;
}
}

__attribute__((visibility("hidden"))) bool rart_gemm_pair_pp_launch(const void* dev_desc, int tn, bool conv, unsigned grid_x, unsigned grid_y,
                                                                    hipStream_t st, unsigned walk_wgs) {
  const GemmPairDev& d = *static_cast<const GemmPairDev*>(dev_desc);
  const dim3 grid(grid_x, grid_y);
#ifdef RART_PP_LAB
  const char* e = getenv("RART_PP_OPT");
  if ((e ? atoi(e) : RART_PP_DEFAULT_OPT) & 1) return pp_launch_opt<1>(d, tn, conv, grid, st, walk_wgs);
  return pp_launch_opt<0>(d, tn, conv, grid, st, walk_wgs);
#else
  return pp_launch_opt<RART_PP_DEFAULT_OPT>(d, tn, conv, grid, st, walk_wgs);
#endif
}

__attribute__((visibility("hidden"))) void rart_gemm_pair_ps_launch(const void* dev_desc, bool conv, unsigned wgs, hipStream_t st) {
  const GemmPairDev& d = *static_cast<const GemmPairDev*>(dev_desc);
  if (conv) hipLaunchKernelGGL((k_gemm_pair_ps<true>), dim3(wgs), dim3(512), 0, st, d);
  else hipLaunchKernelGGL((k_gemm_pair_ps<false>), dim3(wgs), dim3(512), 0, st, d);
}

#ifdef RART_PP_STAMPS
extern "C" int rart_debug_pp_trace(unsigned long long* out) {
  if (hipDeviceSynchronize() != hipSuccess) return RART_ERR_HIP;
  return hipMemcpyFromSymbol(out, HIP_SYMBOL(g_pp_trace), sizeof(unsigned long long) * 4096 * 4) == hipSuccess ? RART_OK : RART_ERR_HIP;
}
extern "C" int rart_debug_pp_stamps(unsigned long long* out) {
  if (hipDeviceSynchronize() != hipSuccess) return RART_ERR_HIP;
  if (hipMemcpyFromSymbol(out, HIP_SYMBOL(g_pp_stamps), sizeof(unsigned long long) * 32) != hipSuccess) return RART_ERR_HIP;
  unsigned long long z[32] = {0};
  if (hipMemcpyToSymbol(HIP_SYMBOL(g_pp_stamps), z, sizeof(z)) != hipSuccess) return RART_ERR_HIP;
  return RART_OK;
}
#endif
```

robustart_amd/csrc/rart_gemm_pair_dev.h:

```cpp
#pragma once
#include "rart_common.h"

typedef __attribute__((ext_vector_type(8))) __bf16 bf16x8;
typedef __attribute__((ext_vector_type(16))) float f32x16;

namespace {
enum { GP_OUT_F32 = 2, GP_GELU = 4, GP_GELU_BWD = 8, GP_GELU_KEEP = 64, GP_RELU = 1, GP_W_INTERLEAVED = 16 };
constexpr int GP_BK = 32;
constexpr int GP_LDE = 68;

struct GemmPairDev {
  const uint16_t *a_hi, *a_lo, *w_hi, *w_lo;
  const float* bias;
  const uint16_t *res_hi, *res_lo;
  uint16_t *dst_hi, *dst_lo;
  uint16_t *aux_hi, *aux_lo;
  int M, N, K, lda, ldw, ldc, w_rows;
  int rpi, src_rpi, src_off, dst_rpi, dst_off, map_rows;
  int flags, z_inner;
  long long a_zo, a_zi, w_zo, w_zi, c_zo, c_zi;
  int grid_h, grid_w, src_h, src_w, sy, sx, n_taps, tpt_shift;
  int tap_dy[16], tap_dx[16];
  int dst_h, dst_w, dst_sy, dst_sx, dst_oy, dst_ox;
  uint32_t gw_magic, gw_shift, gh_magic, gh_shift;
  const uint8_t* mask_bits;
  uint8_t* sign_out;
  int m_begin;
  int tile_rows;
  int nt;
};
__device__ __forceinline__ uint32_t gp_fastdiv(uint32_t n, uint32_t magic, uint32_t shift) {
  return (uint32_t)(((uint64_t)n * magic) >> shift);
}

__device__ __forceinline__ uint32_t gp_pack_bf16x2(float lo, float hi) {
  typedef __attribute__((ext_vector_type(2))) float f2_t;
  typedef __attribute__((ext_vector_type(2))) __bf16 b2_t;
  f2_t f = {lo, hi};
  return __builtin_bit_cast(uint32_t, __builtin_convertvector(f, b2_t));
}
__device__ __forceinline__ float gp_half_erfc_abs(float u, float& e) {
  const float x = fabsf(u) * 0.70710678118654752f;
  const float t = __builtin_amdgcn_rcpf(fmaf(0.5f, x, 1.0f));
  float q = fmaf(-2.548219442e-02f, t, 1.698278524e-01f);
  q = fmaf(q, t, -4.384240636e-01f);
  q = fmaf(q, t, 4.869355765e-01f);
  q = fmaf(q, t, -1.740313807e-01f);
  q = fmaf(q, t, 2.156719095e-01f);
  q = fmaf(q, t, 1.229157723e-01f);
  q = fmaf(q, t, 1.425865282e-01f);
  e = __builtin_amdgcn_exp2f(x * x * -1.4426950408889634f);
  return q * t * e;
}
__device__ __forceinline__ float gp_gelu(float v) {
  float e;
  const float hc = gp_half_erfc_abs(v, e);
  return v * (v < 0.f ? hc : 1.0f - hc);
}
__device__ __forceinline__ float gp_gelu_grad(float u) {
  float e;
  const float hc = gp_half_erfc_abs(u, e);
  return fmaf(u * 0.3989422804014327f, e, u < 0.f ? hc : 1.0f - hc);
}
__device__ __forceinline__ void gp_split8(const float* v, uint4& hi, uint4& lo) {
  uint32_t h[4], l[4];
#pragma unroll
  for (int j = 0; j < 4; ++j) {
    h[j] = gp_pack_bf16x2(v[2 * j], v[2 * j + 1]);
    l[j] = gp_pack_bf16x2(v[2 * j] - __uint_as_float(h[j] << 16), v[2 * j + 1] - __uint_as_float(h[j] & 0xFFFF0000u));
  }
  hi = make_uint4(h[0], h[1], h[2], h[3]);
  lo = make_uint4(l[0], l[1], l[2], l[3]);
}
typedef __attribute__((ext_vector_type(4))) uint32_t gp_u4;
__device__ __forceinline__ uint4 gp_nt_load(const uint16_t* p) {
  const gp_u4 v = __builtin_nontemporal_load(reinterpret_cast<const gp_u4*>(p));
  return make_uint4(v[0], v[1], v[2], v[3]);
}
__device__ __forceinline__ void gp_nt_store(uint16_t* p, const uint4& v) {
  gp_u4 w = {v.x, v.y, v.z, v.w};
  __builtin_nontemporal_store(w, reinterpret_cast<gp_u4*>(p));
}
// ... 175 lines not shown
```

robustart_amd/model/engine.py:

```python
import ctypes
import os as _os

from .. import _lib
from .engine_base import (F_MASK_BITS, F_OUT_F32, F_PAIR, F_RELU, EngineBase, cints as _cints, conv_desc, conv_tap_classes,
                          gemm_pair_desc, interleave_k32, k32, lo_off, pad_k, pad_rows, rows_mult, pair, split_hi_lo, stem_rows)


def _bf16(t):
    import torch
    return t.to(torch.bfloat16).contiguous()


def _planes(w, split):
    hi, lo = split_hi_lo(w)
    return (hi.float(), lo.float()) if split else (hi.float(),)


def _table(build, planes, device):
    import torch
    t = [build(p) for p in planes]
    return _bf16(torch.cat(t + t[:1], 1) if len(t) == 2 else t[0]).to(device)


class _Conv:

    def __init__(self, conv, bn, device, split=False):
        import torch
        w = conv.weight.detach().float()
        if bn is not None:
            inv = (bn.running_var.detach().float() + bn.eps).rsqrt() * bn.weight.detach().float()
            w = w * inv.view(-1, 1, 1, 1)
            b = bn.bias.detach().float() - bn.running_mean.detach().float() * inv
        else:
            b = conv.bias.detach().float() if conv.bias is not None else torch.zeros(w.shape[0])
        self.cout, self.cin, self.r, self.s = w.shape
        self.stride = conv.stride[0]
        self.pad = pad = conv.padding[0]
        self.w_folded = w
        self.b_folded = b
        self.bias = b.contiguous().to(device)
        self.fwd_taps, rs_all, classes = conv_tap_classes(self.r, self.s, self.stride, pad)
        planes = _planes(w, split)

        def table(rs, transpose):
            rows = self.cin if transpose else self.cout
            return _table(lambda wb: pad_rows(torch.cat([wb[:, :, r, s].t() if transpose else wb[:, :, r, s] for r, s in rs], 1),
                                              rows_mult(rows)), planes, device)
        self.w_fwd = table(rs_all, False)
        self.bwd = [(parity, taps, table(rs, True) if rs else None) for parity, taps, rs in classes]


class ResNet50Engine(EngineBase):

    def __init__(self, model, device='cuda', precision='bf16'):
        super().__init__(device, precision)
        torch = _lib.require_gpu()
        split = self.x3
        m = model
        assert not m.training, 'the attack / eval engine folds BatchNorm: call model.eval() first'
        dev = self.device
        st = _Conv(m.conv1, m.bn1, dev, split)
        self.stem = st
        pl = _planes(st.w_folded, split)
        self.stem_patch_cols = 152
        self.stem_wd = _table(lambda p: pad_rows(p.permute(2, 3, 1, 0).reshape(147, 64), rows_mult(self.stem_patch_cols)), pl, dev)
        if not split:
            self.stem_w = _table(lambda p: stem_rows(p).repeat(1, 2), pl, dev)
            self.stem_wt = self._stem_bwd_table(pl[0]).to(dev)
        else:
            self.stem_w = _table(stem_rows, pl, dev)
            self.stem_w_pair = _bf16(torch.stack([stem_rows(p) for p in pl])).to(dev)
            self.stem_wt_pair = pair(self._stem_bwd_table(st.w_folded, dtype=torch.float32)).to(dev)
        self.fused_stem_bwd = True
        self.sign_bit_masks = True
        self.halo_conv3x3 = True
        self.fused_stem_fwd = True
        self.fused_bottleneck = True
        self.fused_bottleneck14 = True
        self.fused_bottleneck28 = True
        self.fused_bottleneck7 = True
        self.fused_bottleneck_s2 = True
        self.fused_bottleneck_s2_bwd = True
        self.small_m_fc = True
        self.pair_tile = (0, 0)
        self.fused_next_pair = True
        self.fused_next_channels = (64,)
        self.fused_tail_channels = (64,)
        self.fused_tail_pair = True
        self.pair_gemm_kernel = True
        self.blocks = []
        for layer in (m.layer1, m.layer2, m.layer3, m.layer4):
            for blk in layer:
                ds = _Conv(blk.downsample[0], blk.downsample[1], dev, split) if blk.downsample is not None else None
                self.blocks.append((_Conv(blk.conv1, blk.bn1, dev, split), _Conv(blk.conv2, blk.bn2, dev, split),
                                    _Conv(blk.conv3, blk.bn3, dev, split), ds))
        wfc = m.fc.weight.detach().float()
        self.n_classes, self.fc_in = wfc.shape
        self.fc_b = m.fc.bias.detach().float().contiguous().to(dev)
        self.fc_kpad = k32(self.n_classes)
        pl = _planes(wfc, split)
        self.fc_w = _table(lambda p: pad_rows(p, 128), pl, dev)
        self.fc_wd = _table(lambda p: pad_k(p.t(), self.fc_kpad), pl, dev)
        self.pair_w_interleaved = _os.environ.get('RART_PAIR_WIL', '0') == '1'
        if not split:
            self._pack_frag_tables()
        else:
            self._pack_tail_tables()

    def _pack_tail_tables(self):
        torch = _lib.require_gpu()

        def frag(tab, rows, k):
            out = []
            for pl in range(2):
                w = tab[:rows, pl * k:(pl + 1) * k]
                out.append(w.reshape(rows // 32, 32, k // 16, 2, 8).permute(0, 2, 3, 1, 4).contiguous().view(-1))
            return torch.stack(out).contiguous()
        def frag_next(tab, rows, k):
            out = []
            for pl in range(2):
                w = tab[:rows, pl * k:(pl + 1) * k]
                out.append(w.reshape(rows // 32, 32, k // 64, 4, 2, 8).permute(2, 0, 3, 4, 1, 5).contiguous().view(-1))
            return torch.stack(out).contiguous()
        for bi, (ca, cb, cc, ds) in enumerate(self.blocks):
            if not (cb.r == 3 and cb.stride == 1 and cb.pad == 1 and cb.cin == cb.cout and self.lib.rart_conv3x3_tail_pair_supported(cb.cin)):
                continue
            if cc.cin == cb.cout and cc.cout == 4 * cb.cout and cc.r == 1 and cc.stride == 1:
                cc.tail_fwd = frag(cc.w_fwd, cc.cout, cc.cin)
                if bi + 1 < len(self.blocks):
                    na = self.blocks[bi + 1][0]
                    if na.r == 1 and na.stride == 1 and na.cin == cc.cout and na.cout == cb.cout:
                        na.next_fwd = frag_next(na.w_fwd, na.cout, na.cin)
            if ds is None and ca.cout == cb.cin and ca.cin == 4 * cb.cin and ca.r == 1 and ca.stride == 1:
                ca.tail_bwd = frag(ca.bwd[0][2], ca.cin, ca.cout)
                pc = self.blocks[bi - 1][2]
                if bi > 0 and pc.r == 1 and pc.stride == 1 and pc.cout == ca.cin and pc.cin == cb.cin:
                    pc.next_bwd = frag_next(pc.bwd[0][2], pc.cin, pc.cout)

    def _pack_frag_tables(self, record=None, sums=None):
        torch = _lib.require_gpu()
        sp = _lib.stream_ptr()
        lib_pack = self.lib.rart_pack_frag_bf16

        def pack(tab, dst, rows, k):
            if record is not None:
                record.append((tab, dst, rows, k))
            else:
                _lib.check(lib_pack(_lib.ptr(tab), _lib.ptr(dst), rows, k, sp))

        def bias_sum(a, b, out):
            if sums is not None:
                sums.append((a, b, out))
            else:
                torch.add(a, b, out=out)
        for ca, cb, cc, ds in self.blocks:
            if cb.r == 3 and cb.stride == 1 and cb.cin == cb.cout and cb.cin in (64, 128, 256, 512):
                for name, tab in (('w_fwd_frag', cb.w_fwd), ('w_bwd_frag', cb.bwd[0][2])):
                    if getattr(cb, name, None) is None:
                        setattr(cb, name, torch.empty(9 * cb.cin * cb.cin, dtype=torch.bfloat16, device=self.device))
                    pack(tab, getattr(cb, name), cb.cin, 9 * cb.cin)
            if ds is None and cb.stride == 1 and (ca.cin, ca.cout, cc.cout) in ((1024, 256, 1024), (512, 128, 512), (2048, 512, 2048)):
                for c_, rows, k in ((ca, ca.cout, ca.cin), (cc, cc.cout, cc.cin)):
                    for name, tab in (('w_fwd_frag', c_.w_fwd), ('w_bwd_frag', c_.bwd[0][2])):
                        r_, k_ = (rows, k) if name == 'w_fwd_frag' else (k, rows)
                        if getattr(c_, name, None) is None:
                            setattr(c_, name, torch.empty(rows * k, dtype=torch.bfloat16, device=self.device))
                        pack(tab, getattr(c_, name), r_, k_)
            if (ds is not None and cb.stride == 2 and cb.r == 3 and ds.stride == 2 and ds.r == 1
                    and (ca.cin, ca.cout, cc.cout) in ((256, 128, 512), (512, 256, 1024))):
                for c_, name, rows, k in ((ca, 's2_w1', ca.cout, ca.cin), (cb, 's2_w2', cb.cout, 9 * cb.cin), (cc, 's2_w3', cc.cout, cc.cin),
                                          (ds, 's2_wd', ds.cout, ds.cin)):
                    if getattr(c_, name, None) is None:
                        setattr(c_, name, torch.empty(rows * k, dtype=torch.bfloat16, device=self.device))
                    pack(c_.w_fwd, getattr(c_, name), rows, k)
                if getattr(ds, 'bias_sum', None) is None:
                    ds.bias_sum = torch.empty_like(cc.bias)
                bias_sum(cc.bias, ds.bias, ds.bias_sum)
# ... 107 lines not shown
        for nm in ('var', 'gamma', 'beta', 'mean', 'scale', 'tmp', 'bias'):
            st[nm] = torch.empty(n_tot, dtype=torch.float32, device=dev)
        jobs, big, off = [], [], 0
        for c, conv, bn in pairs:
            w = conv.weight
            assert w.is_cuda and w.dtype == torch.float32 and w.is_contiguous()
            old = c.bias
            c.bias = st['bias'][off:off + c.cout]
            c.bias.copy_(old)
            scale_ptr = st['scale'][off:off + c.cout].data_ptr()
            rs = [(r, s_) for r in range(c.r) for s_ in range(c.s)]
            todo = [(c.w_fwd, rs, 0)]
            for parity, taps, tab in c.bwd:
                if tab is not None:
                    prs = rs if parity is None else [(r, s_) for r, s_ in rs if (parity[0] + c.pad - r) % 2 == 0 and (parity[1] + c.pad - s_) % 2 == 0]
                    todo.append((tab, prs, 1))
            for tab, trs, tr in todo:
                if len(trs) <= 16:
                    jobs.append(self._pack_job(w, scale_ptr, tab, c, trs, tr))
                else:
                    big.append((w, st['scale'][off:off + c.cout], tab, c, trs, tr))
            off += c.cout
        frag, sums = [], []
        self._pack_frag_tables(record=frag, sums=sums)
        fj = []
        for src, dst, rows, k in frag:
            j = _lib.PackJob()
            j.kind, j.rows, j.k, j.src16, j.out = 1, rows, k, src.data_ptr(), dst.data_ptr()
            fj.append(j)
        st['pack_jobs'], st['n_pack'] = self._upload_jobs(jobs), len(jobs)
        st['frag_jobs'], st['n_frag'] = (self._upload_jobs(fj) if fj else None), len(fj)
        st['bias_sums'], st['big'] = sums, big
        st['_keep'] = (jobs, fj)
        self._refold_state = st
        return st

    @staticmethod
    def _pack_job(w, scale_ptr, tab, c, rs, transpose):
        j = _lib.PackJob()
        j.kind, j.n_out, j.channels, j.r, j.s, j.n_taps, j.transpose, j.rows_padded = 0, c.cout, c.cin, c.r, c.s, len(rs), transpose, tab.shape[0]
        for i, (a, b) in enumerate(rs):
            j.tap_r[i], j.tap_s[i] = a, b
        j.weight, j.out_channel_scale, j.out = w.data_ptr(), scale_ptr, tab.data_ptr()
        return j

    def _upload_jobs(self, jobs):
        torch = _lib.require_gpu()
        arr = (_lib.PackJob * len(jobs))(*jobs)
        host = torch.frombuffer(bytearray(bytes(arr)), dtype=torch.uint8)
        return host.to(self.device)

    def _gemm(self, src, wgt, dst, batch, grid, src_hw, src_pix, k_per_tap, taps, n_cols, dst_hw, dst_pix,
              bias=None, res=None, mask=None, flags=0, stride=(1, 1), dst_stride=(1, 1), dst_off=(0, 0),
              tap_src_off=None, sign_out=None, pair=False):
        if pair and self.pair_gemm_kernel and len(taps) <= 16 and k_per_tap >= 32 and (k_per_tap & (k_per_tap - 1)) == 0:
            return self._gemm_pair(src, wgt, dst, batch, grid, src_hw, src_pix, k_per_tap, taps, n_cols, dst_hw, dst_pix, bias, res,
                                   mask, flags, stride, dst_stride, dst_off, sign_out)
        dst_pair_off = res_pair_off = 0
        if pair:
            assert tap_src_off is None and src.shape[0] == 2
            tap_src_off = [0] * (2 * len(taps)) + [lo_off(src)] * len(taps)
            taps = list(taps) * 3
            flags |= F_PAIR
            if not (flags & F_OUT_F32):
                dst_pair_off = lo_off(dst)
            if res is not None:
                res_pair_off = lo_off(res)
        self._launch_conv(conv_desc(src, wgt, dst, batch, grid, src_hw, src_pix, k_per_tap, taps, n_cols, dst_hw, dst_pix, bias=bias,
                                    res=res, mask=mask, sign_out=sign_out, flags=flags, stride=stride, dst_stride=dst_stride,
                                    dst_org=dst_off, tap_src_off=tap_src_off, dst_pair_off=dst_pair_off, res_pair_off=res_pair_off))

    def _gemm_pair(self, src, wgt, dst, batch, grid, src_hw, src_pix, k_per_tap, taps, n_cols, dst_hw, dst_pix, bias, res, mask, flags,
                   stride, dst_stride, dst_off, sign_out):
        assert src.shape[0] == 2
        k_tot = k_per_tap * len(taps)
        assert wgt.shape[1] == 3 * k_tot
        il = None
        if self.pair_w_interleaved:
            il = self._w_il.get(wgt.data_ptr())
            if il is None:
                il = self._w_il[wgt.data_ptr()] = interleave_k32(wgt[:, :k_tot], wgt[:, k_tot:2 * k_tot])
        nbytes = None
        if self.profile is not None:
            rows = batch * grid[0] * grid[1]
            nbytes = 4.0 * batch * src_hw[0] * src_hw[1] * k_per_tap + 4.0 * rows * n_cols * (2 if res is not None else 1) + 4.0 * k_tot * n_cols \
                + rows * n_cols / 8.0 * ((mask is not None) + (sign_out is not None))
        self._launch_pair(gemm_pair_desc(src, wgt, dst, n_cols, src_pix, 3 * k_tot, dst_pix, wgt.shape[0], bias=bias, res=res, mask_bits=mask,
                                         sign_out=sign_out, flags=flags & (F_RELU | F_OUT_F32), w_lo_off=k_tot, w_il=il, batch=batch,
                                         grid=grid, src_hw=src_hw, stride=stride, k_per_tap=k_per_tap, taps=taps, dst_hw=dst_hw,
                                         dst_stride=dst_stride, dst_org=dst_off, tile=self.pair_tile), nbytes)

    def _tail(self, src, wgt, taps, tail, dst, batch, hw, c_mid, bias_mid=None, bias_out=None, res=None, mask_mid=None, mask_out=None,
              sign_mid=None, sign_out=None, relu=False, nxt=None):
        k_tot = 9 * c_mid
        assert src.shape[0] == 2 and wgt.shape[1] == 3 * k_tot and len(taps) == 9
        d = _lib.ConvTailDesc()
        d.a_hi, d.a_lo = src[0].data_ptr(), src[1].data_ptr()
        d.w_hi, d.w_lo = wgt.data_ptr(), wgt.data_ptr() + 2 * k_tot
        d.t_hi, d.t_lo = tail[0].data_ptr(), tail[1].data_ptr()
        d.bias_mid, d.bias_out = _lib.ptr(bias_mid), _lib.ptr(bias_out)
        d.mask_mid, d.mask_out, d.sign_mid, d.sign_out = _lib.ptr(mask_mid), _lib.ptr(mask_out), _lib.ptr(sign_mid), _lib.ptr(sign_out)
        if res is not None:
            d.res_hi, d.res_lo = res[0].data_ptr(), res[1].data_ptr()
        d.dst_hi, d.dst_lo = dst[0].data_ptr(), dst[1].data_ptr()
        d.batch, d.h, d.w, d.c_mid, d.ldw = batch, hw[0], hw[1], c_mid, 3 * k_tot
        d.relu_mid = d.relu_out = 1 if relu else 0
        for i, (dy, dx) in enumerate(taps):
            d.tap_dy[i], d.tap_dx[i] = dy, dx
        if nxt is not None:
            d.n_hi, d.n_lo = nxt['tab'][0].data_ptr(), nxt['tab'][1].data_ptr()
            d.dstn_hi, d.dstn_lo = nxt['dst'][0].data_ptr(), nxt['dst'][1].data_ptr()
            d.bias_next, d.mask_next, d.sign_next = _lib.ptr(nxt.get('bias')), _lib.ptr(nxt.get('mask')), _lib.ptr(nxt.get('sign'))
            d.relu_next = 1 if nxt.get('relu') else 0
        ev = self._prof_begin()
        _lib.check(self.lib.rart_conv3x3_tail_pair(ctypes.byref(d), _lib.stream_ptr()))
        if ev is not None:
            px = batch * hw[0] * hw[1]
            nbytes = 4.0 * px * c_mid * (1 + 4 + (4 if res is not None else 0) + (1 if nxt is not None else 0)) \
                + 4.0 * c_mid * c_mid * (9 + 4 + (4 if nxt is not None else 0))
            self._prof_end(ev, 3 * 2.0 * px * (k_tot * c_mid + (8 if nxt is not None else 4) * c_mid * c_mid), 'conv_tail_pair',
                           nbytes)

    def _fc(self, a, w, out, m, n, k, bias=None):
        torch = _lib.require_gpu()
        ev = self._prof_begin()
        _lib.check(self.lib.rart_gemm_small_m_bf16(_lib.ptr(a), a.shape[-1], _lib.ptr(w), w.shape[-1], _lib.ptr(bias), _lib.ptr(out),
                                                   out.shape[-1], 1 if out.dtype == torch.float32 else 0, m, n, k, _lib.stream_ptr()))
        if ev is not None:
            self._prof_end(ev, 2.0 * m * n * k, 'fc_small_m')

    @staticmethod
    def _fits32(n, hw, channels):
        return n * hw[0] * hw[1] * channels < (1 << 31)

    def _halo_ok(self, c, hw, n=1):
        return (self._fits32(n, hw, c.cin) and self.halo_conv3x3 and c.r == 3 and c.s == 3 and c.stride == 1 and c.pad == 1
                and c.cin == c.cout and getattr(c, 'w_fwd_frag', None) is not None and self.lib.rart_conv3x3_halo_supported(c.cin, hw[0], hw[1]))

    def _halo(self, src, w, dst, B, hw, ch, taps, bias=None, mask=None, sign=None, relu=False):
        ev = self._prof_begin()
        _lib.check(self.lib.rart_conv3x3_halo_bf16(_lib.ptr(src), _lib.ptr(w), _lib.ptr(bias), _lib.ptr(mask), _lib.ptr(sign),
                                                   _lib.ptr(dst), B, hw[0], hw[1], ch, _cints([t[0] for t in taps]),
                                                   _cints([t[1] for t in taps]), 1 if relu else 0, _lib.stream_ptr()))
        if ev is not None:
            self._prof_end(ev, 2.0 * B * hw[0] * hw[1] * 9 * ch * ch, 'halo3x3')

    def _bneck_ok(self, ca, cb, cc, ds, xhw, n=1):
        return (self._fits32(n, xhw, cc.cout) and self.fused_bottleneck and ds is None and cb.stride == 1 and cb.r == 3 and ca.r == 1 and cc.r == 1
                and ca.cin == cc.cout and getattr(cb, 'w_fwd_frag', None) is not None
                and self.lib.rart_bottleneck_fused_supported(cc.cout, ca.cout, xhw[0], xhw[1]))

    def _image_block_fn(self, ca, cb, cc, ds, xhw, n=1):
        if not (self._fits32(n, xhw, cc.cout) and self.fused_bottleneck14 and ds is None and getattr(ca, 'w_fwd_frag', None) is not None
                and getattr(cb, 'w_fwd_frag', None) is not None and getattr(cc, 'w_fwd_frag', None) is not None):
            return None
        if self.lib.rart_bottleneck14_fused_supported(cc.cout, ca.cout, xhw[0], xhw[1]):
            return self.lib.rart_bottleneck14_fused_bf16
        if self.fused_bottleneck28 and self.lib.rart_bottleneck28_fused_supported(cc.cout, ca.cout, xhw[0], xhw[1]):
            return self.lib.rart_bottleneck28_fused_bf16
        if self.fused_bottleneck7 and self.lib.rart_bottleneck7_fused_supported(cc.cout, ca.cout, xhw[0], xhw[1]):
            return self.lib.rart_bottleneck7_fused_bf16
        return None

    def _bneck_image(self, x, w1, w2, w3, b1, b2, b3, m1, m2, m3, out, B, hw, c_io, c_mid, taps, backward, fn):
        ev = self._prof_begin()
        _lib.check(fn(
            _lib.ptr(x), _lib.ptr(w1), _lib.ptr(w2), _lib.ptr(w3), _lib.ptr(b1), _lib.ptr(b2), _lib.ptr(b3), _lib.ptr(m1),
            _lib.ptr(m2), _lib.ptr(m3), _lib.ptr(out), B, hw[0], hw[1], c_io, c_mid, _cints([t[0] for t in taps]),
            _cints([t[1] for t in taps]), 1 if backward else 0, _lib.stream_ptr()))
        if ev is not None:
            m_ = B * hw[0] * hw[1]
            by = 2 * m_ * c_io * 2 + (2 * c_io * c_mid + 9 * c_mid * c_mid) * 2 + sum(m_ * c // 8 for c, t in ((c_mid, m1), (c_mid, m2), (c_io, m3)) if t is not None)
            self._prof_end(ev, 2.0 * B * hw[0] * hw[1] * c_mid * (2 * c_io + 9 * c_mid), {14: 'bottleneck14', 28: 'bottleneck28', 7: 'bottleneck7'}[hw[0]],
# ... 138 lines not shown
            else:
                self._gemm(hi[0], self.stem_w, y1, B, (h1, w1), (H + 8, W + 8), 4, 32, rows * 2, 64, (h1, w1), 64, bias=self.stem.bias,
                           flags=F_RELU, stride=(2, 2), tap_src_off=[0] * 7 + [lo_off(hi)] * 7)
            _lib.check((lib.rart_engine_maxpool_pair if x3 else lib.rart_engine_maxpool_keep)(
                *self._po(y1), *self._po(p1), _lib.ptr(parg), _lib.ptr(xs), B, h1, w1, 64, sp))
        acts['y1'], acts['p1'], acts['p1_argmax'] = y1, p1, parg
        return p1, (h2, w2), xs

    def _fused_block(self, ca, cb, cc, ds, xhw, B, backward):
        if self.x3:
            c = ca if backward else cc
            return 'tail' if (self.fused_tail_pair and cb.cin in self.fused_tail_channels
                              and getattr(c, 'tail_bwd' if backward else 'tail_fwd', None) is not None
                              and self._fits32(B, xhw, c.cin if backward else c.cout)) else None
        if self._bneck_ok(ca, cb, cc, ds, xhw, B):
            return 'bneck'
        fn = self._image_block_fn(ca, cb, cc, ds, xhw, B)
        if fn is not None:
            return fn
        if self._first_ok(ca, cb, cc, ds, xhw, B):
            return 'first'
        if (not backward or (self.fused_bottleneck_s2_bwd and getattr(cb, 's2_w2t', None) is not None)) and self._s2_ok(ca, cb, cc, ds, xhw, B):
            return 's2'
        return None

    def _block_fwd(self, bi, x, xhw, xs, B, keep, bits, pre_a, acts):
        import torch
        x3 = self.x3
        get, lead = self._get, ((2, B) if x3 else (B,))
        ca, cb, cc, ds = self.blocks[bi]
        ohw = (xhw[0] // cb.stride, xhw[1] // cb.stride)
        sa = get('b%d_a_sign' % bi, (B, xhw[0], xhw[1], ca.cout // 8), torch.uint8) if bits else None
        sb = get('b%d_b_sign' % bi, (B, ohw[0], ohw[1], cb.cout // 8), torch.uint8) if bits else None
        sc = get('b%d_c_sign' % bi, (B, ohw[0], ohw[1], cc.cout // 8), torch.uint8) if bits else None
        yc = get('b%d_c' % bi, lead + (ohw[0], ohw[1], cc.cout))
        ya = yb = None
        nxt = None
        kind = self._fused_block(ca, cb, cc, ds, xhw, B, False) if (bits or not keep) else None
        if kind == 'bneck':
            self._bneck(x, ca.w_fwd, cb.w_fwd_frag, cc.w_fwd, ca.bias, cb.bias, cc.bias, sa, sb, sc, yc, B, xhw, cc.cout, ca.cout,
                        cb.fwd_taps, False)
        elif kind == 'first':
            self._bneck(x, ca.w_fwd, cb.w_fwd_frag, cc.w_fwd, ca.bias, cb.bias, ds.bias_sum, sa, sb, sc, yc, B, xhw, cc.cout, ca.cout,
                        cb.fwd_taps, False, w4=ds.w_fwd_frag, c_in=ca.cin)
        elif kind == 's2':
            self._bneck_s2(x, ca, cb, cc, ds, sa, sb, sc, yc, B, xhw)
        elif kind not in (None, 'tail'):
            self._bneck_image(x, ca.w_fwd_frag, cb.w_fwd_frag, cc.w_fwd_frag, ca.bias, cb.bias, cc.bias, sa, sb, sc, yc, B, xhw, cc.cout,
                              ca.cout, cb.fwd_taps, False, kind)
        else:
            ya = get('b%d_a' % bi, lead + (xhw[0], xhw[1], ca.cout))
            if not pre_a:
                self._conv_fwd(ca, x, xhw, ya, True, sign=sa, pair=x3)
            if x3:
                sk = x if ds is None else self._shortcut_fwd(bi, ds, x, xhw, ohw, B)
            if kind == 'tail':
                na = self.blocks[bi + 1][0] if bi + 1 < len(self.blocks) else None
                if self.fused_next_pair and na is not None and getattr(na, 'next_fwd', None) is not None and cb.cout in self.fused_next_channels:
                    nxt = dict(tab=na.next_fwd, bias=na.bias, relu=True, dst=get('b%d_a' % (bi + 1), lead + (ohw[0], ohw[1], na.cout)),
                               sign=get('b%d_a_sign' % (bi + 1), (B, ohw[0], ohw[1], na.cout // 8), torch.uint8) if keep else None)
                self._tail(ya, cb.w_fwd, cb.fwd_taps, cc.tail_fwd, yc, B, ohw, cb.cout, bias_mid=cb.bias, bias_out=cc.bias, res=sk,
                           sign_mid=sb, sign_out=sc, relu=True, nxt=nxt)
            else:
                yb = get('b%d_b' % bi, lead + (ohw[0], ohw[1], cb.cout))
                self._conv_fwd(cb, ya, xhw, yb, True, sign=sb, pair=x3)
                if not x3:
                    sk = x if ds is None else self._shortcut_fwd(bi, ds, x, xhw, ohw, B)
                self._conv_fwd(cc, yb, ohw, yc, True, res=sk, sign=sc, pair=x3)
        acts['b%d' % bi] = (x, xhw, ya, yb, yc, ohw)
        acts['b%d_masks' % bi] = (xs, sa, sb) if (bits or x3 or kind is not None) else (x, ya, yb)
        return yc, ohw, sc, nxt is not None

    def _shortcut_fwd(self, bi, ds, x, xhw, ohw, B):
        sk = self._act('b%d_ds' % bi, (B, ohw[0], ohw[1], ds.cout))
        self._conv_fwd(ds, x, xhw, sk, False, pair=self.x3)
        return sk

    def _head_fwd(self, x, xhw, B):
        torch = _lib.require_gpu()
        lib, x3 = self.lib, self.x3
        pooled = self._act('pooled', (B, self.fc_in))
        _lib.check((lib.rart_engine_avgpool_pair if x3 else lib.rart_engine_avgpool)(
            *self._po(x), *self._po(pooled), B, xhw[0] * xhw[1], self.fc_in, _lib.stream_ptr()))
        logits = torch.empty(B, self.n_classes, dtype=torch.float32, device=self.device)
        if self.small_m_fc and not x3:
            self._fc(pooled, self.fc_w, logits, B, self.n_classes, self.fc_in, bias=self.fc_b)
        else:
            self._gemm(pooled, self.fc_w, logits, B, (1, 1), (1, 1), self.fc_in, self.fc_in, [(0, 0)], self.n_classes,
                       (1, 1), self.n_classes, bias=self.fc_b, flags=F_OUT_F32, pair=x3)
        return logits

    def _head_bwd(self, acts, dl, B):
        lib, x3 = self.lib, self.x3
        dlb = self._dlogits_rows(dl, 'g_dl', B, self.fc_kpad)
        dpool = self._act('dpool', (B, self.fc_in))
        if self.small_m_fc and not x3:
            self._fc(dlb, self.fc_wd, dpool, B, self.fc_in, self.fc_kpad)
        else:
            self._gemm(dlb, self.fc_wd, dpool, B, (1, 1), (1, 1), self.fc_kpad, self.fc_kpad, [(0, 0)], self.fc_in, (1, 1),
                       self.fc_in, pair=x3)
        xl, xlhw = acts['last']
        dz = self._get('g_out_%d' % (len(self.blocks) - 1), tuple(xl.shape))
        _lib.check((lib.rart_engine_avgpool_bwd_pair if x3 else lib.rart_engine_avgpool_bwd)(
            _lib.ptr(acts['last_sign'] if x3 else xl), *self._po(dpool), *self._po(dz), B, xlhw[0] * xlhw[1], self.fc_in, _lib.stream_ptr()))
        return dz

    def _block_bwd(self, bi, dz, B, pre_b, acts):
        import torch
        x3 = self.x3
        get, lead = self._get, ((2, B) if x3 else (B,))
        ca, cb, cc, ds = self.blocks[bi]
        x, xhw, ya, yb, yc, ohw = acts['b%d' % bi]
        mx, ma, mb = acts['b%d_masks' % bi]
        dx = get('g_out_%d' % (bi - 1), tuple(x.shape))
        if x3:
            bits = ma is not None and mx is not None
        else:
            bits = ma is not None and ma.dtype == torch.uint8 and mb is not None
        kind = self._fused_block(ca, cb, cc, ds, xhw, B, True) if bits else None
        if kind == 'bneck':
            self._bneck(dz, cc.bwd[0][2], cb.w_bwd_frag, ca.bwd[0][2], None, None, None, mb, ma, mx, dx, B, xhw, cc.cout, ca.cout,
                        cb.bwd[0][1], True)
        elif kind == 'first':
            self._bneck(dz, cc.bwd[0][2], cb.w_bwd_frag, ds.bwd[0][2], None, None, None, mb, ma, mx, dx, B, xhw, cc.cout, ca.cout,
                        cb.bwd[0][1], True, w4=ca.bwd[0][2], c_in=ca.cin)
        elif kind == 's2':
            self._bneck_s2_bwd(dz, ca, cb, cc, ds, mb, ma, mx, dx, B, xhw)
        elif kind not in (None, 'tail'):
            self._bneck_image(dz, cc.w_bwd_frag, cb.w_bwd_frag, ca.w_bwd_frag, None, None, None, mb, ma, mx, dx, B, xhw, cc.cout, ca.cout,
                              cb.bwd[0][1], True, kind)
        else:
            dzb = get('g_b%d' % (bi & 1) if x3 else 'g_b', lead + (ohw[0], ohw[1], cb.cout))
            if not pre_b:
                self._conv_bwd(cc, dz, ohw, dzb, ohw, mask=mb, pair=x3)
            if kind == 'tail':
                nxt = None
                pc = self.blocks[bi - 1][2] if bi > 0 else None
                if self.fused_next_pair and pc is not None and getattr(pc, 'next_bwd', None) is not None and cb.cin in self.fused_next_channels:
                    mask = acts['b%d_masks' % (bi - 1)][2]
                    if mask is not None:
                        nxt = dict(tab=pc.next_bwd, mask=mask, dst=get('g_b%d' % ((bi - 1) & 1), lead + (xhw[0], xhw[1], pc.cin)))
                self._tail(dzb, cb.bwd[0][2], cb.bwd[0][1], ca.tail_bwd, dx, B, xhw, cb.cin, res=dz, mask_mid=ma, mask_out=mx, nxt=nxt)
                return dx, nxt is not None
            dza = get('g_a', lead + (xhw[0], xhw[1], ca.cout))
            self._conv_bwd(cb, dzb, ohw, dza, xhw, mask=ma, pair=x3)
            if ds is None:
                self._conv_bwd(ca, dza, xhw, dx, xhw, res=dz, mask=mx, pair=x3)
            else:
                self._conv_bwd(ca, dza, xhw, dx, xhw, mask=mx, pair=x3)
                self._conv_bwd(ds, dz, ohw, dx, xhw, res=dx, mask=mx, pair=x3)
        return dx, False

    def _stem_bwd(self, acts, dz, std):
        torch = _lib.require_gpu()
        lib, sp, x3 = self.lib, _lib.stream_ptr(), self.x3
        B, H, W = acts['in_shape']
        grad = torch.empty(B, 3, H, W, dtype=torch.float32, device=self.device)
        stdf = (ctypes.c_float * 3)(*std)
        parg = acts['p1_argmax']
        if self.fused_stem_bwd and x3:
            ev = self._prof_begin()
            _lib.check(lib.rart_engine_stem_bwd_fused_pair(*self._hl(dz), _lib.ptr(parg), *self._hl(self.stem_wt_pair), _lib.ptr(grad),
                                                           B, H, W, stdf, sp))
            if ev is not None:
                self._prof_end(ev, 3 * 2.0 * B * (H // 2) * (W // 2) * 16 * 64 * 16, 'stem_pair', 4.0 * B * (H // 4) * (W // 4) * 64 * 1.25 + 4.0 * B * H * W * 3)
            return grad
        if self.fused_stem_bwd:
            _lib.check(lib.rart_engine_stem_bwd_fused(_lib.ptr(dz), _lib.ptr(parg), _lib.ptr(self.stem_wt), _lib.ptr(grad), B, H, W, stdf, sp))
            return grad
        y1 = acts['y1']
        assert x3 or y1 is not None, 'the unfused stem backward needs the stem output: set fused_stem_fwd = False as well'
        h1, w1 = H // 2, W // 2
        dz1 = self._act('g_y1', (B, h1, w1, 64))
        if x3:
            _lib.check(lib.rart_engine_maxpool_bwd_pair(_lib.ptr(parg), *self._po(dz), *self._po(dz1), B, h1, w1, 64, sp))
        else:
            _lib.check(lib.rart_engine_maxpool_bwd(_lib.ptr(y1), _lib.ptr(parg), _lib.ptr(dz), _lib.ptr(dz1), B, h1, w1, 64, sp))
        pc = self.stem_patch_cols
        patches = self._get('patches', (B, h1, w1, pc), torch.float32 if x3 else torch.bfloat16)
        self._gemm(dz1, self.stem_wd, patches, B, (h1, w1), (h1, w1), 64, 64, [(0, 0)], pc, (h1, w1), pc, flags=F_OUT_F32 if x3 else 0,
                   pair=x3)
        _lib.check((lib.rart_engine_stem_col2im_f32 if x3 else lib.rart_engine_stem_col2im)(_lib.ptr(patches), _lib.ptr(grad), B, H, W, pc,
                                                                                             stdf, sp))
        return grad

    def forward_backward(self, x01, mean, std, y, kind, y_target=None, scale=1.0):
        from ..noise.adv import logit_loss
        logits, acts = self._forward(x01.detach().float().contiguous(), False, mean, std, keep=True)
        self.last_acts = acts
        loss, dl, pred = logit_loss(logits, y, kind, y_target, scale)
        self.last_dlogits = dl
        return logits, loss, self._backward(acts, dl, std), pred


def make_engine(torch_model, device='cuda', precision='bf16'):
    from .resnet_torch import ResNet
    from .vit_torch import VisionTransformer
    if isinstance(torch_model, ResNet):
        return ResNet50Engine(torch_model, device, precision)
    if isinstance(torch_model, VisionTransformer):
# ... 40 lines not shown
```

robustart_amd/model/engine_base.py:

```python
import ctypes

from .. import _lib

F_RELU, F_OUT_F32, F_GELU, F_GELU_BWD = 1, 2, 4, 8
F_MASK_BITS = 16
F_PAIR = 32
F_GELU_KEEP = 64
F_MASK_RES = 128
GP_RELU, GP_OUT_F32, GP_GELU, GP_GELU_BWD, GP_W_INTERLEAVED, GP_GELU_KEEP = 1, 2, 4, 8, 16, 64

PRECISIONS = {'bf16': 'bf16', 'bf16x3': 'bf16x3', 'fp32x': 'bf16x3'}

ROW_TAPS = [((0, 0),) * n for n in range(33)]


def check_precision(precision):
    if precision not in PRECISIONS:
        raise ValueError('precision must be one of %s' % sorted(PRECISIONS))
    return PRECISIONS[precision]


def _addr(t):
    return None if t is None else t.data_ptr()

# ... 54 lines not shown
    import torch
    t = torch.zeros(64, 7, 8, 4, dtype=w.dtype, device=w.device)
    t[:, :, :7, :3] = w.permute(0, 2, 3, 1)
    return t.reshape(64, 7 * 32)


def conv_tap_classes(r, s, stride, pad):
    all_rs = [(a, b) for a in range(r) for b in range(s)]
    fwd_taps = [(a - pad, b - pad) for a, b in all_rs]
    if stride == 1:
        return fwd_taps, all_rs, [(None, [(pad - a, pad - b) for a, b in all_rs], all_rs)]
    assert stride == 2
    bwd = []
    for ph in range(2):
        for pw in range(2):
            rs = [(a, b) for a, b in all_rs if (ph + pad - a) % 2 == 0 and (pw + pad - b) % 2 == 0]
            bwd.append(((ph, pw), [((ph + pad - a) // 2, (pw + pad - b) // 2) for a, b in rs], rs))
    return fwd_taps, all_rs, bwd


def conv_desc(src, wgt, dst, batch, grid, src_hw, src_pix, k_per_tap, taps, n_cols, dst_hw, dst_pix, bias=None, res=None, mask=None,
              sign_out=None, stats_out=None, flags=0, stride=(1, 1), dst_stride=(1, 1), dst_org=(0, 0), tap_src_off=None, batched=None,
              dst_pair_off=0, res_pair_off=0):
    d = _lib.ConvDesc()
    d.src, d.wgt, d.dst = src.data_ptr(), wgt.data_ptr(), dst.data_ptr()
    d.bias, d.res, d.mask, d.sign_out, d.bn_stats_out = _addr(bias), _addr(res), _addr(mask), _addr(sign_out), _addr(stats_out)
    d.batch, d.grid_h, d.grid_w = batch, grid[0], grid[1]
    d.src_h, d.src_w, d.src_pix_stride = src_hw[0], src_hw[1], src_pix
    d.k_per_tap, d.n_taps = k_per_tap, len(taps)
    d.sy, d.sx = stride
    for i, (dy, dx) in enumerate(taps):
        d.tap_dy[i], d.tap_dx[i] = dy, dx
        if tap_src_off:
            d.tap_src_off[i] = tap_src_off[i]
    d.n_cols = n_cols
    d.dst_h, d.dst_w = dst_hw
    d.dst_sy, d.dst_sx = dst_stride
    d.dst_oy, d.dst_ox = dst_org
    d.dst_pix_stride = dst_pix
    d.flags = flags
    d.dst_pair_off, d.res_pair_off = dst_pair_off, res_pair_off
    if batched:
        d.n_batched, d.z_inner = batched['n'], batched['inner']
        d.src_z_outer, d.src_z_inner = batched['src']
        d.wgt_z_outer, d.wgt_z_inner = batched['wgt']
        d.dst_z_outer, d.dst_z_inner = batched['dst']
        d.wgt_row_stride = batched.get('wgt_row_stride', 0)
    return d


def gemm_pair_desc(a, w, dst, N, lda, ldw, ldc, w_rows, M=0, K=0, bias=None, res=None, aux=None, mask_bits=None, sign_out=None, flags=0,
                   a_off=0, w_off=0, dst_off=0, w_lo_off=None, w_il=None, rows_per_image=0, src_rows_per_image=0, src_row_off=0,
                   dst_rows_per_image=0, dst_row_off=0, batched=None, batch=0, grid=None, src_hw=(0, 0), stride=(1, 1), k_per_tap=0,
                   taps=(), dst_hw=(0, 0), dst_stride=(1, 1), dst_org=(0, 0), tile=(0, 0)):
    d = _lib.GemmPairDesc()
    if grid is not None:
        M, K = batch * grid[0] * grid[1], k_per_tap * len(taps)
    d.a_hi, d.a_lo = a[0].data_ptr() + 2 * a_off, a[1].data_ptr() + 2 * a_off
    if w_il is not None:
        d.w_hi, d.w_lo, ldw = w_il.data_ptr(), w_il.data_ptr() + 64, 2 * K
        flags |= GP_W_INTERLEAVED
    elif w_lo_off is not None:
        w_hi = w.data_ptr() + 2 * w_off
        d.w_hi, d.w_lo = w_hi, w_hi + 2 * w_lo_off
    else:
        d.w_hi, d.w_lo = w[0].data_ptr() + 2 * w_off, w[1].data_ptr() + 2 * w_off
    d.bias = _addr(bias)
    if res is not None:
        d.res_hi, d.res_lo = res[0].data_ptr() + 2 * dst_off, res[1].data_ptr() + 2 * dst_off
    if flags & GP_OUT_F32:
        d.dst_hi = dst.data_ptr() + 4 * dst_off
    else:
        d.dst_hi, d.dst_lo = dst[0].data_ptr() + 2 * dst_off, dst[1].data_ptr() + 2 * dst_off
    if aux is not None:
        d.aux_hi, d.aux_lo = aux[0].data_ptr() + 2 * dst_off, aux[1].data_ptr() + 2 * dst_off
    d.M, d.N, d.K, d.lda, d.ldw, d.ldc, d.w_rows = M, N, K, lda, ldw, ldc, w_rows
    d.rows_per_image, d.src_rows_per_image, d.src_row_off = rows_per_image, src_rows_per_image, src_row_off
    d.dst_rows_per_image, d.dst_row_off = dst_rows_per_image, dst_row_off
    d.flags = flags
    if batched:
        d.n_batched, d.z_inner = batched['n'], batched['inner']
        d.a_z_outer, d.a_z_inner = batched['a']
        d.w_z_outer, d.w_z_inner = batched['w']
        d.c_z_outer, d.c_z_inner = batched['c']
    if grid is not None:
        d.conv, d.batch, d.grid_h, d.grid_w = 1, batch, grid[0], grid[1]
        d.src_h, d.src_w, d.sy, d.sx = src_hw[0], src_hw[1], stride[0], stride[1]
        d.k_per_tap, d.n_taps = k_per_tap, len(taps)
        for i, (dy, dx) in enumerate(taps):
            d.tap_dy[i], d.tap_dx[i] = dy, dx
        d.dst_h, d.dst_w = dst_hw
        d.dst_sy, d.dst_sx = dst_stride
        d.dst_oy, d.dst_ox = dst_org
    d.mask_bits, d.sign_out = _addr(mask_bits), _addr(sign_out)
    d.tile_m, d.tile_n = tile
    return d


def tokmix_desc(a, x, dst, M, N, K, batch, x_stride, c_stride, ldx=None, ldc=None, bias=None, res=None, aux=None, flags=0, pair=False):
    d = _lib.TokmixDesc()
    if pair:
        d.a_hi, d.a_lo, d.x_hi, d.x_lo = a[0].data_ptr(), a[1].data_ptr(), x[0].data_ptr(), x[1].data_ptr()
        if flags & GP_OUT_F32:
            d.dst_hi = dst.data_ptr()
        else:
            d.dst_hi, d.dst_lo = dst[0].data_ptr(), dst[1].data_ptr()
        if res is not None:
            d.res_hi, d.res_lo = res[0].data_ptr(), res[1].data_ptr()
        if aux is not None:
            d.aux_hi, d.aux_lo = aux[0].data_ptr(), aux[1].data_ptr()
    else:
        d.a_hi, d.x_hi, d.dst_hi, d.res_hi, d.aux_hi = a.data_ptr(), x.data_ptr(), dst.data_ptr(), _addr(res), _addr(aux)
    d.bias = _addr(bias)
    d.M, d.N, d.K, d.lda = M, N, K, a.shape[-1]
    d.ldx, d.ldc = ldx or N, ldc or N
    d.batch, d.flags = batch, flags
    d.x_stride, d.c_stride = x_stride, c_stride
    return d


def tokmix_wgrad_desc(p, q, partial, M, N, D, batch, splits, images_per_split, ld_partial, p_stride=None, q_stride=None):
    d = _lib.TokmixWgradDesc()
    d.p, d.q, d.partial = p.data_ptr(), q.data_ptr(), partial.data_ptr()
    d.M, d.N, d.D, d.batch = M, N, D, batch
    d.splits, d.images_per_split, d.ld_partial = splits, images_per_split, ld_partial
    d.p_stride, d.q_stride = p_stride or M * D, q_stride or N * D
    return d


def wgrad_split_direct(M, x_c, n_taps, n_cols, target_wgs, min_chunk):
    tmr = 128
    if x_c == 4:
        row_tiles = (n_taps + 31) // 32
    else:
        row_tiles = n_taps * (x_c // tmr) if x_c >= tmr else (n_taps + tmr // x_c - 1) // (tmr // x_c)
    tiles = row_tiles * (n_cols // (128 if n_cols % 128 == 0 else 64))
    splits = max(1, min(target_wgs // max(tiles, 1), M // min_chunk if M >= 2 * min_chunk else 1, 1024))
    chunk = ((M + splits - 1) // splits + 31) // 32 * 32
    return (M + chunk - 1) // chunk, chunk


def wgrad_split_transposed(M, kp, n_pad):
    bn_tile = 128 if n_pad > 64 else 64
    tiles = ((kp + 127) // 128) * ((n_pad + bn_tile - 1) // bn_tile)
    splits = max(1, min(1024 // max(tiles, 1), M // 512 if M >= 1024 else 1, 256))
    chunk = ((M + splits - 1) // splits + 63) // 64 * 64
    return splits, chunk, (n_pad + bn_tile - 1) // bn_tile * bn_tile

# ... 23 lines not shown

    def _get(self, name, shape, dtype=None, zero=False):
        torch = _lib.require_gpu()
        dtype = dtype or torch.bfloat16
        t = self._buf.get(name)
        if t is None or tuple(t.shape) != tuple(shape) or t.dtype != dtype:
            t = (torch.zeros if zero else torch.empty)(shape, dtype=dtype, device=self.device)
            self._buf[name] = t
        return t

    def _scratch(self, name, nbytes):
        torch = _lib.require_gpu()
        t = self._buf.get(name)
        if t is None or t.numel() < nbytes:
            t = torch.empty(int(nbytes), dtype=torch.uint8, device=self.device)
            self._buf[name] = t
        return t

    def _act(self, name, shape):
        return self._get(name, ((2,) + tuple(shape)) if self.x3 else tuple(shape))

    def _hl(self, t):
        return (_lib.ptr(t[0]), _lib.ptr(t[1])) if self.x3 else (_lib.ptr(t), None)

    def _dlogits_rows(self, dl, name, B, kpad):
        lib, sp = self.lib, _lib.stream_ptr()
        dlb = self._act(name, (B, kpad))
        if self.x3:
            _lib.check(lib.rart_f32_to_pair_rows(_lib.ptr(dl), _lib.ptr(dlb[0]), lo_off(dlb), B, self.n_classes, kpad, sp))
        else:
            _lib.check(lib.rart_f32_to_bf16_rows(_lib.ptr(dl), _lib.ptr(dlb), B, self.n_classes, kpad, sp))
        return dlb

    def _prof_begin(self):
        if self.profile is None:
            return None
        e0 = _lib.require_gpu().cuda.Event(enable_timing=True)
        e0.record()
        return e0

    def _prof_end(self, e0, flops, kind, nbytes=None):
        e1 = _lib.require_gpu().cuda.Event(enable_timing=True)
        e1.record()
        self.profile.append((flops, e0, e1, kind) if nbytes is None else (flops, e0, e1, kind, nbytes))

    def _launch_conv(self, d):
        ev = self._prof_begin()
        _lib.check(self.lib.rart_conv_igemm_bf16(ctypes.byref(d), _lib.stream_ptr()))
        if ev is not None:
            self._prof_end(ev, 2.0 * d.batch * d.grid_h * d.grid_w * d.k_per_tap * d.n_taps * d.n_cols * max(d.n_batched, 1), 'igemm')

    def _launch_pair(self, d, nbytes=None):
        ev = self._prof_begin()
        _lib.check(self.lib.rart_gemm_pair_bf16(ctypes.byref(d), _lib.stream_ptr()))
        if ev is not None:
            self._prof_end(ev, 3 * 2.0 * max(d.n_batched, 1) * d.M * d.N * d.K, 'gemm_pair', nbytes)

    def _launch_tokmix(self, d, pair):
        ev = self._prof_begin()
        _lib.check((self.lib.rart_tokmix_pair if pair else self.lib.rart_tokmix_bf16)(ctypes.byref(d), _lib.stream_ptr()))
        if ev is not None:
            self._prof_end(ev, (3 if pair else 1) * 2.0 * d.batch * d.M * d.N * d.K, 'tokmix')

    def _wgrad_direct(self, x, dz, B, x_hw, x_c, grid_hw, n_out, n_pad_cols, taps, stride, grad, c_valid=None):
        lib, sp = self.lib, _lib.stream_ptr()
        splits, chunk = wgrad_split_direct(B * grid_hw[0] * grid_hw[1], x_c, len(taps), n_pad_cols, self.wgrad_target_wgs,
                                           self.wgrad_min_chunk)
        part = self._scratch('wg_part', splits * len(taps) * x_c * n_pad_cols * 4)
        _lib.check(lib.rart_wgrad_direct_bf16(_lib.ptr(x), _lib.ptr(dz), _lib.ptr(part), B, x_hw[0], x_hw[1], x_c, grid_hw[0], grid_hw[1],
                                              n_pad_cols, stride, stride, len(taps), cints([t[0] for t in taps]), cints([t[1] for t in taps]),
                                              splits, chunk, n_pad_cols, sp))
        _lib.check(lib.rart_wgrad_reduce_f32(_lib.ptr(part), splits, len(taps), c_valid if c_valid is not None else x_c, x_c, n_out,
                                             n_pad_cols, _lib.ptr(grad), 0, sp))

    def _wgrad_transposed(self, dz, dz_geom, x, x_geom, n_out, grad, reduce, row_grid=False):
        lib, sp = self.lib, _lib.stream_ptr()
        n_pad = dz_geom[3]
        images, x_h, x_w, x_c, grid_h, grid_w, stride, taps = x_geom
        kp = len(taps) * x_c
        splits, chunk, n_rows = wgrad_split_transposed(images * grid_h * grid_w, kp, n_pad)
        m_pad = chunk * splits
        dzt = self._scratch('wg_dzT', n_rows * m_pad * 2)
        colt = self._scratch('wg_colT', kp * m_pad * 2)
        zero = cints([0])
        if n_rows > n_pad:
            dzt[:n_rows * m_pad * 2].zero_()
        _lib.check(lib.rart_transpose_gather_bf16(_lib.ptr(dz), _lib.ptr(dzt), *dz_geom, 1, 1, 1, zero, zero, m_pad, chunk, n_rows, sp))
        _lib.check(lib.rart_transpose_gather_bf16(_lib.ptr(x), _lib.ptr(colt), images, x_h, x_w, x_c, grid_h, grid_w, stride, stride,
                                                  len(taps), cints([t[0] for t in taps]), cints([t[1] for t in taps]), m_pad, chunk,
                                                  kp, sp))
        ld_n = (n_pad + 7) // 8 * 8
        part = self._scratch('wg_part', splits * kp * ld_n * 4)
        grid = (kp, 1) if row_grid else (1, kp)
        self._launch_conv(conv_desc(colt, dzt, part, 1, grid, grid, chunk, chunk, ROW_TAPS[1], ld_n, grid, ld_n, flags=F_OUT_F32,
                                    batched=dict(n=splits, inner=splits, src=(0, kp * chunk), wgt=(0, n_rows * chunk), dst=(0, kp * ld_n),
                                                 wgt_row_stride=chunk)))
        _lib.check(lib.rart_wgrad_reduce_f32(_lib.ptr(part), splits, *reduce, n_out, ld_n, _lib.ptr(grad), 0, sp))

    def _colsum(self, x, ld, rows, cols, out):
        lib = self.lib
        need = lib.rart_colsum_workspace_bytes(rows, cols)
        ws = self._scratch('cs_ws', need)
        _lib.check(lib.rart_colsum_bf16(_lib.ptr(x), ld, rows, cols, _lib.ptr(out), 0, _lib.ptr(ws), need, _lib.stream_ptr()))

    def logits(self, x01, mean, std):
        return self._logits(x01.detach().float().contiguous(), False, mean, std)

# ... 179 lines not shown
```

scratch/prof_engine2.py:

```python
import os, sys; sys.path.insert(0, os.path.dirname(os.path.dirname(os.path.abspath(__file__))))
import os, time, torch
if os.environ.get('RART_LIB'):
    from robustart_amd import _lib as _l; _l.LIB_PATH = os.environ['RART_LIB']
from robustart_amd.model import get_model
from robustart_amd.model.engine import ResNet50Engine
MEAN, STD = (0.485, 0.456, 0.406), (0.229, 0.224, 0.225)
PEAK_F, PEAK_B = 2.5e15, 8.0e12
torch.manual_seed(0)
eng = ResNet50Engine(get_model({'type': 'resnet50_official'}).eval(), 'cuda', os.environ.get('PREC', 'bf16'))
for a in sys.argv[1:]:
    if '=' in a:
        k, v = a.split('='); setattr(eng, k, bool(int(v)))
import os
if os.environ.get('BK64'):
    eng.lib.rart_igemm_set_bk64_min_k(int(os.environ['BK64']))
B = 256
x = torch.rand(B, 3, 224, 224, device='cuda'); y = torch.randint(0, 1000, (B,), device='cuda')
rows = []
orig = eng._gemm
def wrapped(src, wgt, dst, batch, grid, src_hw, src_pix, k_per_tap, taps, n_cols, dst_hw, dst_pix, **kw):
    M = batch * grid[0] * grid[1]; K = k_per_tap * len(taps)
    stride = kw.get('stride', (1, 1))
    src_bytes = min(src.numel() * src.element_size(), M * K * 2) if len(taps) > 1 else M * K * 2
    by = src_bytes + K * n_cols * 2 + M * n_cols * (4 if kw.get('flags', 0) & 2 else 2)
    if kw.get('res') is not None: by += M * n_cols * 2
    mk = kw.get('mask')
    if mk is not None: by += M * n_cols * (2 if mk.dtype != torch.uint8 else 0.125)
    if kw.get('sign_out') is not None: by += M * n_cols * 0.125
    fl = 2.0 * M * K * n_cols
    e0, e1 = torch.cuda.Event(enable_timing=True), torch.cuda.Event(enable_timing=True)
    e0.record(); r = orig(src, wgt, dst, batch, grid, src_hw, src_pix, k_per_tap, taps, n_cols, dst_hw, dst_pix, **kw); e1.record()
    rows.append(((M, K, n_cols, len(taps)), fl, by, e0, e1))
    return r
orig_halo = eng._halo
def wrapped_halo(src, w, dst, B_, hw, ch, taps, **kw):
    M = B_ * hw[0] * hw[1]
    by = 2 * M * ch * 2 + 9 * ch * ch * 2 + (M * ch * 0.125 if (kw.get('mask') is not None or kw.get('sign') is not None) else 0)
    e0, e1 = torch.cuda.Event(enable_timing=True), torch.cuda.Event(enable_timing=True)
    e0.record(); r = orig_halo(src, w, dst, B_, hw, ch, taps, **kw); e1.record()
    rows.append(((M, 9 * ch, ch, 99), 2.0 * M * 9 * ch * ch, by, e0, e1))
    return r
orig_bneck = eng._bneck
def wrapped_bneck(x_, w1, w2, w3, b1, b2, b3, m1, m2, m3, out, B_, hw, c_io, c_mid, taps, backward, w4=None, c_in=None):
    M = B_ * hw[0] * hw[1]
    cin = c_io if w4 is None else c_in
    by = M * (c_io + cin) * 2 + ((c_io + cin) * c_mid + 9 * c_mid * c_mid + (0 if w4 is None else c_in * c_io)) * 2 + sum(M * c * 0.125 for c, m_ in ((c_mid, m1), (c_mid, m2), (c_io, m3)) if m_ is not None)
    e0, e1 = torch.cuda.Event(enable_timing=True), torch.cuda.Event(enable_timing=True)
    e0.record(); r = orig_bneck(x_, w1, w2, w3, b1, b2, b3, m1, m2, m3, out, B_, hw, c_io, c_mid, taps, backward, w4, c_in); e1.record()
    k_all = (2 * c_io + 9 * c_mid) if w4 is None else (c_in + 9 * c_mid + c_io + c_in * c_io // c_mid)
    rows.append(((M, k_all, c_mid, 98), 2.0 * M * c_mid * k_all, by, e0, e1))
    return r
orig_b14 = eng._bneck_image
def wrapped_b14(x_, w1, w2, w3, b1, b2, b3, m1, m2, m3, out, B_, hw, c_io, c_mid, taps, backward, fn=None):
    M = B_ * hw[0] * hw[1]
    by = 2 * M * c_io * 2 + (2 * c_io * c_mid + 9 * c_mid * c_mid) * 2 + sum(M * c * 0.125 for c, m_ in ((c_mid, m1), (c_mid, m2), (c_io, m3)) if m_ is not None)
    e0, e1 = torch.cuda.Event(enable_timing=True), torch.cuda.Event(enable_timing=True)
    e0.record(); r = orig_b14(x_, w1, w2, w3, b1, b2, b3, m1, m2, m3, out, B_, hw, c_io, c_mid, taps, backward, fn); e1.record()
    rows.append(((M, 2 * c_io + 9 * c_mid, c_mid, {14: 97, 28: 96, 7: 95}[hw[0]]), 2.0 * M * c_mid * (2 * c_io + 9 * c_mid), by, e0, e1))
    return r
orig_s2 = eng._bneck_s2
def wrapped_s2(x_, ca, cb, cc, ds, m1, m2, m3, out, B_, xhw):
    pin, pout = B_ * xhw[0] * xhw[1], B_ * xhw[0] * xhw[1] // 4
    fl = 2.0 * (pin * ca.cin * ca.cout + pout * (9 * cb.cin * cb.cout + cc.cin * cc.cout + ds.cin * ds.cout))
    by = pin * ca.cin * 2 + pout * cc.cout * 2 + (ca.cin * ca.cout + 9 * cb.cin * cb.cout + cc.cin * cc.cout + ds.cin * ds.cout) * 2 + \
        sum(n_ * c * 0.125 for n_, c, m_ in ((pin, ca.cout, m1), (pout, cb.cout, m2), (pout, cc.cout, m3)) if m_ is not None)
    e0, e1 = torch.cuda.Event(enable_timing=True), torch.cuda.Event(enable_timing=True)
    e0.record(); r = orig_s2(x_, ca, cb, cc, ds, m1, m2, m3, out, B_, xhw); e1.record()
    rows.append(((pout, ca.cin * 4 + 9 * cb.cin + cc.cin + ds.cin, cc.cout, 94), fl, by, e0, e1))
    return r
orig_s2b = eng._bneck_s2_bwd
def wrapped_s2b(g_, ca, cb, cc, ds, m2, m1, m0, dx_, B_, xhw):
    pin, pout = B_ * xhw[0] * xhw[1], B_ * xhw[0] * xhw[1] // 4
    fl = 2.0 * (pin * ca.cin * ca.cout + pout * (9 * cb.cin * cb.cout + cc.cin * cc.cout + ds.cin * ds.cout))
    by = pin * ca.cin * 2 + pout * cc.cout * 2 + (ca.cin * ca.cout + 9 * cb.cin * cb.cout + cc.cin * cc.cout + ds.cin * ds.cout) * 2 + \
        (pin * ca.cout + pout * cb.cout + (pin * ca.cin if m0 is not None else 0)) * 0.125
    e0, e1 = torch.cuda.Event(enable_timing=True), torch.cuda.Event(enable_timing=True)
# ... 50 lines not shown
```

Measured before the change: 8513 images/s.

## Fuse Bottleneck downsample shortcut into expansion GEMM via a second K source

```diff
diff --git a/include/robustart_hip.h b/include/robustart_hip.h
--- a/include/robustart_hip.h
+++ b/include/robustart_hip.h
@@ -199,6 +199,13 @@
   int tile_m;
 } rart_gemm_pair_desc;
 int rart_gemm_pair_bf16(const rart_gemm_pair_desc* desc_host, rart_stream_t stream);
+typedef struct rart_gemm_pair2_desc {
+  rart_gemm_pair_desc one;
+  const void *a2_hi, *a2_lo;
+  int lda2, k2, src2_h, src2_w, sy2, sx2;
+} rart_gemm_pair2_desc;
+int rart_gemm_pair2_bf16(const rart_gemm_pair2_desc* desc_host, rart_stream_t stream);
+int rart_gemm_pair_max_sources(void);
 int rart_gemm_pair_set_schedule(int mode);
 int rart_gemm_pair_get_schedule(void);
 
@@ -220,6 +227,8 @@
   void* sign_next;
   void* dstn_hi;  void* dstn_lo;
   int relu_next;
+  const void* x_hi;  const void* x_lo;
+  const void* tx_hi;  const void* tx_lo;
 } rart_conv_tail_desc;
 int rart_conv3x3_tail_pair_supported(int c_mid);
 int rart_conv3x3_tail_pair(const rart_conv_tail_desc* desc_host, rart_stream_t stream);
diff --git a/robustart_amd/_lib.py b/robustart_amd/_lib.py
--- a/robustart_amd/_lib.py
+++ b/robustart_amd/_lib.py
@@ -75,6 +75,8 @@
     'rart_logit_loss': (c_int, [c_void_p, c_void_p, c_void_p, c_int, c_int, c_int, c_float, c_void_p,
                                 c_void_p, c_void_p, c_void_p]),
     'rart_conv_igemm_bf16': (c_int, [c_void_p, c_void_p]),
+    'rart_gemm_pair2_bf16': (c_int, [c_void_p, c_void_p]),
+    'rart_gemm_pair_max_sources': (c_int, []),
     'rart_conv3x3_halo_supported': (c_int, [c_int, c_int, c_int]),
     'rart_conv3x3_pack_frag_bf16': (c_int, [c_void_p, c_void_p, c_int, c_void_p]),
     'rart_pack_frag_bf16': (c_int, [c_void_p, c_void_p, c_int, c_int, c_void_p]),
@@ -288,6 +290,11 @@
                [('mask_bits', c_void_p), ('sign_out', c_void_p), ('tile_n', ctypes.c_int32), ('tile_m', ctypes.c_int32)]
 
 
+class GemmPair2Desc(ctypes.Structure):
+    _fields_ = [('one', GemmPairDesc), ('a2_hi', c_void_p), ('a2_lo', c_void_p)] + \
+               [(n, ctypes.c_int32) for n in ('lda2', 'k2', 'src2_h', 'src2_w', 'sy2', 'sx2')]
+
+
 class TokmixDesc(ctypes.Structure):
     _fields_ = [(n, c_void_p) for n in ('a_hi', 'a_lo', 'x_hi', 'x_lo', 'dst_hi', 'dst_lo', 'res_hi', 'res_lo', 'aux_hi', 'aux_lo', 'bias')] + \
                [(n, ctypes.c_int32) for n in ('M', 'N', 'K', 'lda', 'ldx', 'ldc', 'batch', 'flags')] + \
@@ -305,7 +312,8 @@
                                         'sign_mid', 'sign_out', 'res_hi', 'res_lo', 'dst_hi', 'dst_lo')] + \
                [(n, ctypes.c_int32) for n in ('batch', 'h', 'w', 'c_mid', 'ldw', 'relu_mid', 'relu_out')] + \
                [('tap_dy', ctypes.c_int32 * 9), ('tap_dx', ctypes.c_int32 * 9)] + \
-               [(n, c_void_p) for n in ('n_hi', 'n_lo', 'bias_next', 'mask_next', 'sign_next', 'dstn_hi', 'dstn_lo')] + [('relu_next', ctypes.c_int32)]
+               [(n, c_void_p) for n in ('n_hi', 'n_lo', 'bias_next', 'mask_next', 'sign_next', 'dstn_hi', 'dstn_lo')] + [('relu_next', ctypes.c_int32)] + \
+               [(n, c_void_p) for n in ('x_hi', 'x_lo', 'tx_hi', 'tx_lo')]
 
 
 _lib = None
diff --git a/robustart_amd/csrc/conv_tail_pair.hip b/robustart_amd/csrc/conv_tail_pair.hip
--- a/robustart_amd/csrc/conv_tail_pair.hip
+++ b/robustart_amd/csrc/conv_tail_pair.hip
@@ -28,6 +28,7 @@
   uint8_t* sign_next;
   uint16_t *dstn_hi, *dstn_lo;
   int relu_next;
+  const uint16_t *x_hi, *x_lo, *tx_hi, *tx_lo;
 };
 typedef __attribute__((ext_vector_type(4))) uint32_t ct_u4;
 __device__ __forceinline__ uint4 ct_nt_load(const uint16_t* p) {
@@ -107,8 +108,10 @@
     }
 }
 
-template <int C, bool NEXT>
-__global__ __launch_bounds__(256, (C == 64 && !NEXT) ? 3 : 2) void k_conv3x3_tail_pair(const ConvTailDev d) {
+template <int C, bool NEXT, bool XS = false>
+__global__ __launch_bounds__(256, (C == 64 && !NEXT && !XS) ? 3 : 2) void k_conv3x3_tail_pair(const ConvTailDev d) {
+  static_assert(!XS || C == 64, "the shortcut source is built for layer1's first block: 64 input channels");
+  constexpr int KX = 4;
   constexpr int NJ = C / 32;
   constexpr int KS = C / 16;
   constexpr int NOUT = 4 * C, NC = NOUT / 64;
@@ -234,6 +237,19 @@
     }
   }
 
+  bf16x8 xfh[XS ? KX : 1], xfl[XS ? KX : 1];
+  if (XS) {
+#pragma unroll
+    for (int s = 0; s < KX; ++s) {
+      uint4 vh = make_uint4(0, 0, 0, 0), vl = vh;
+      if (p_ok) {
+        vh = *reinterpret_cast<const uint4*>(d.x_hi + (size_t)p * 64 + 16 * s + 8 * h);
+        vl = *reinterpret_cast<const uint4*>(d.x_lo + (size_t)p * 64 + 16 * s + 8 * h);
+      }
+      xfh[s] = __builtin_bit_cast(bf16x8, vh);
+      xfl[s] = __builtin_bit_cast(bf16x8, vl);
+    }
+  }
   uint8_t* const wreg = lds + wave * CT_WREG;
   float* sE = reinterpret_cast<float*>(wreg);
   const int cw = lane & 7, rw = lane >> 3;
@@ -250,6 +266,8 @@
   }
   const uint4* th_base = reinterpret_cast<const uint4*>(d.t_hi) + lane;
   const uint4* tl_base = reinterpret_cast<const uint4*>(d.t_lo) + lane;
+  const uint4* txh_base = reinterpret_cast<const uint4*>(XS ? d.tx_hi : d.t_hi) + lane;
+  const uint4* txl_base = reinterpret_cast<const uint4*>(XS ? d.tx_lo : d.t_lo) + lane;
   const bool relu_out = d.relu_out != 0;
 #pragma unroll 1
   for (int c = 0; c < NC; ++c) {
@@ -297,6 +315,21 @@
           acc2[b] = __builtin_amdgcn_mfma_f32_32x32x16_bf16(wh, a2h[sg + s], acc2[b], 0, 0, 0);
         }
       }
+      if (XS) {
+        uint4 th[KX], tl[KX];
+#pragma unroll
+        for (int s = 0; s < KX; ++s) {
+          th[s] = txh_base[((c * 2 + b) * KX + s) * 64];
+          tl[s] = txl_base[((c * 2 + b) * KX + s) * 64];
+        }
+#pragma unroll
+        for (int s = 0; s < KX; ++s) {
+          const bf16x8 wh = __builtin_bit_cast(bf16x8, th[s]), wl = __builtin_bit_cast(bf16x8, tl[s]);
+          acc2[b] = __builtin_amdgcn_mfma_f32_32x32x16_bf16(wh, xfl[s], acc2[b], 0, 0, 0);
+          acc2[b] = __builtin_amdgcn_mfma_f32_32x32x16_bf16(wl, xfh[s], acc2[b], 0, 0, 0);
+          acc2[b] = __builtin_amdgcn_mfma_f32_32x32x16_bf16(wh, xfh[s], acc2[b], 0, 0, 0);
+        }
+      }
     }
 #pragma unroll
     for (int b = 0; b < 2; ++b)
@@ -420,7 +453,11 @@
   RART_CHECK_ARG(t->ldw % 8 == 0 && t->ldw >= 9 * t->c_mid, "rart_conv3x3_tail_pair: ldw must cover 9 taps x c_mid and keep 16-byte alignment");
   const long long M = (long long)t->batch * t->h * t->w;
   RART_CHECK_ARG(M * 4 * t->c_mid < (1ll << 31), "rart_conv3x3_tail_pair: tensors must stay below 2^31 elements (split the batch)");
-  ConvTailDev d;
+  const bool xs = t->x_hi != nullptr;
+  RART_CHECK_ARG(!xs || (t->x_lo && t->tx_hi && t->tx_lo), "rart_conv3x3_tail_pair: the shortcut source needs both input planes and both table planes");
+  RART_CHECK_ARG(!xs || (t->c_mid == 64 && !t->res_hi), "rart_conv3x3_tail_pair: the shortcut source is served at c_mid = 64 and takes the place of the skip pair");
+  ConvTailDev d{};
+  d.x_hi = (const uint16_t*)t->x_hi; d.x_lo = (const uint16_t*)t->x_lo; d.tx_hi = (const uint16_t*)t->tx_hi; d.tx_lo = (const uint16_t*)t->tx_lo;
   d.a_hi = (const uint16_t*)t->a_hi; d.a_lo = (const uint16_t*)t->a_lo; d.w_hi = (const uint16_t*)t->w_hi; d.w_lo = (const uint16_t*)t->w_lo;
   d.t_hi = (const uint16_t*)t->t_hi; d.t_lo = (const uint16_t*)t->t_lo;
   d.bias_mid = t->bias_mid; d.bias_out = t->bias_out;
@@ -438,7 +475,10 @@
   ct_magic((uint32_t)d.H, d.h_magic, d.h_shift);
   const dim3 grid((uint32_t)((M + CT_TM - 1) / CT_TM));
   hipStream_t st = (hipStream_t)stream;
-  if (t->c_mid == 64) {
+  if (xs) {
+    if (next) hipLaunchKernelGGL((k_conv3x3_tail_pair<64, true, true>), grid, dim3(256), 0, st, d);
+    else hipLaunchKernelGGL((k_conv3x3_tail_pair<64, false, true>), grid, dim3(256), 0, st, d);
+  } else if (t->c_mid == 64) {
     if (next) hipLaunchKernelGGL((k_conv3x3_tail_pair<64, true>), grid, dim3(256), 0, st, d);
     else hipLaunchKernelGGL((k_conv3x3_tail_pair<64, false>), grid, dim3(256), 0, st, d);
   } else {
diff --git a/robustart_amd/csrc/gemm_pair.hip b/robustart_amd/csrc/gemm_pair.hip
--- a/robustart_amd/csrc/gemm_pair.hip
+++ b/robustart_amd/csrc/gemm_pair.hip
@@ -5,8 +5,9 @@
 #include "rart_lds_dma.h"
 
 namespace {
-template <int TM, int TN, bool CONV>
+template <int TM, int TN, bool CONV, bool SRC2 = false>
 __global__ __launch_bounds__(TM * 2, 1) void k_gemm_pair(const GemmPairDev d) {
+  static_assert(CONV || !SRC2, "the second source is served by the conv instances");
   constexpr int NW = TM / 32;
   constexpr int WN = (TN / 64 < NW) ? TN / 64 : NW, WM = NW / WN, RW = TM / WM, MI = RW / 32, NJ = TN / (32 * WN);
   static_assert(NJ == 2, "a wave owns 64 columns");
@@ -78,6 +79,22 @@
       avoff[q] = ok ? (uint32_t)(((srow + d.src_off) * d.lda + csrc * 8) * 2) : RART_DMA_OOR;
     }
   }
+  uint32_t avoff2[2] = {RART_DMA_OOR, RART_DMA_OOR};
+  if (SRC2) {
+#pragma unroll
+    for (int q = 0; q < 2; ++q) {
+      const int r = 16 * (wave + NW * q) + (lane >> 2);
+      const int csrc = (lane & 3) ^ ((r >> 2) & 3);
+      const int m = m0 + r;
+      if (m < d.M) {
+        const uint32_t t = gp_fastdiv((uint32_t)m, d.gw_magic, d.gw_shift);
+        const int ox = (int)((uint32_t)m - t * (uint32_t)d.grid_w);
+        const int n = (int)gp_fastdiv(t, d.gh_magic, d.gh_shift);
+        const int oy = (int)(t - (uint32_t)n * (uint32_t)d.grid_h);
+        avoff2[q] = (uint32_t)(((n * d.src2_h + oy * d.sy2) * d.src2_w + ox * d.sx2) * d.lda2 * 2 + csrc * 16);
+      }
+    }
+  }
   uint32_t wvoff[BQ];
 #pragma unroll
   for (int q = 0; q < BQ; ++q) {
@@ -88,13 +105,21 @@
   }
   const rart_srd_t srd_ah = rart_dma_srd(reinterpret_cast<const char*>(a_hi) + tap_min), srd_al = rart_dma_srd(reinterpret_cast<const char*>(a_lo) + tap_min);
   const rart_srd_t srd_wh = rart_dma_srd(w_hi), srd_wl = rart_dma_srd(w_lo);
+  const rart_srd_t srd_a2h = rart_dma_srd(SRC2 ? d.a2_hi : a_hi), srd_a2l = rart_dma_srd(SRC2 ? d.a2_lo : a_lo);
+  const int kt1 = SRC2 ? d.kt1 : 0;
   const uint32_t lds_base = (uint32_t)(uintptr_t)(__attribute__((address_space(3))) uint8_t*)lds;
   const int w_step = (d.flags & GP_W_INTERLEAVED) ? 128 : 64;
 #define RART_GP_ISSUE(KT, BUF)                                                                                  \
   {                                                                                                             \
     const uint32_t st_ = lds_base + (BUF)*STAGE;                                                                \
     const int kt_ = (KT);                                                                                       \
-    if (one_tap) {                                                                                              \
+    if (SRC2 && kt_ >= kt1) {                                                                                   \
+      const uint32_t so_ = (uint32_t)(kt_ - kt1) * 64u;                                                         \
+      _Pragma("unroll") for (int q = 0; q < 2; ++q) {                                                           \
+        rart_dma_load16(avoff2[q], srd_a2h, so_, st_ + (wave + NW * q) * 1024);                                 \
+        rart_dma_load16(avoff2[q], srd_a2l, so_, st_ + GP_PLANE_A + (wave + NW * q) * 1024);                    \
+      }                                                                                                         \
+    } else if (one_tap) {                                                                                       \
       const uint32_t so_ = tap0 + (uint32_t)kt_ * 64u;                                                          \
       _Pragma("unroll") for (int q = 0; q < 2; ++q) {                                                           \
         rart_dma_load16(avoff[q], srd_ah, so_, st_ + (wave + NW * q) * 1024);                                   \
@@ -224,12 +249,14 @@
 }
 extern "C" int rart_gemm_pair_get_schedule(void) { return gp_schedule(); }
 
-extern "C" int rart_gemm_pair_bf16(const rart_gemm_pair_desc* h, rart_stream_t stream) {
+static int gp_launch(const rart_gemm_pair_desc* h, const rart_gemm_pair2_desc* s2, rart_stream_t stream) {
   RART_CHECK_ARG(h != nullptr, "rart_gemm_pair_bf16: null descriptor");
   RART_CHECK_ARG(h->a_hi && h->a_lo && h->w_hi && h->w_lo && h->dst_hi, "rart_gemm_pair_bf16: null operand plane");
   const bool conv = h->conv != 0;
-  GemmPairDev d;
+  GemmPairDev d{};
   d.M = h->M; d.K = h->K;
+  const bool src2 = s2 != nullptr;
+  RART_CHECK_ARG(!src2 || (conv && s2->a2_hi && s2->a2_lo), "rart_gemm_pair2_bf16: the second source is a pair (both planes) and is served by conv mode only");
   if (conv) {
     RART_CHECK_ARG(h->batch > 0 && h->grid_h > 0 && h->grid_w > 0 && h->src_h > 0 && h->src_w > 0 && h->dst_h > 0 && h->dst_w > 0,
                    "rart_gemm_pair_bf16 (conv): empty geometry");
@@ -246,6 +273,18 @@
     RART_CHECK_ARG(h->lda % 8 == 0 || h->lda == 4, "rart_gemm_pair_bf16 (conv): source pixels must keep 16-byte alignment of the K chunks");
     d.M = (int)M;
     d.K = h->k_per_tap * h->n_taps;
+    if (src2) {
+      RART_CHECK_ARG(s2->k2 >= 32 && s2->k2 % GP_BK == 0, "rart_gemm_pair2_bf16: k2 must be a positive multiple of 32");
+      RART_CHECK_ARG(s2->lda2 % 8 == 0 && s2->lda2 >= s2->k2, "rart_gemm_pair2_bf16: lda2 must cover k2 and keep 16-byte alignment of the K chunks");
+      RART_CHECK_ARG(s2->src2_h > 0 && s2->src2_w > 0 && s2->sy2 > 0 && s2->sx2 > 0 && (long long)(h->grid_h - 1) * s2->sy2 < s2->src2_h &&
+                         (long long)(h->grid_w - 1) * s2->sx2 < s2->src2_w,
+                     "rart_gemm_pair2_bf16: every row's pixel must lie inside the second source's image");
+      RART_CHECK_ARG((long long)h->batch * s2->src2_h * s2->src2_w * s2->lda2 < (1ll << 30),
+                     "rart_gemm_pair2_bf16: the second source plane must stay below 2 GiB (split the batch)");
+      d.a2_hi = (const uint16_t*)s2->a2_hi; d.a2_lo = (const uint16_t*)s2->a2_lo;
+      d.lda2 = s2->lda2; d.kt1 = d.K / GP_BK; d.src2_h = s2->src2_h; d.src2_w = s2->src2_w; d.sy2 = s2->sy2; d.sx2 = s2->sx2;
+      d.K += s2->k2;
+    }
     d.grid_h = h->grid_h; d.grid_w = h->grid_w; d.src_h = h->src_h; d.src_w = h->src_w; d.sy = h->sy; d.sx = h->sx; d.n_taps = h->n_taps;
     int sh = 0;
     while ((32 << sh) < h->k_per_tap) ++sh;
@@ -327,7 +366,7 @@
   RART_CHECK_ARG(blocks < (1ll << 31), "rart_gemm_pair_bf16: grid too large");
   const dim3 grid((uint32_t)blocks, nz);
   hipStream_t st = (hipStream_t)stream;
-  if (gp_schedule() == 2 && tm == 256 && tn >= 128 && h->tile_n == 0 && h->tile_m == 0 && nz == 1 && !d.map_rows && d.src_off == 0 &&
+  if (gp_schedule() == 2 && !src2 && tm == 256 && tn >= 128 && h->tile_n == 0 && h->tile_m == 0 && nz == 1 && !d.map_rows && d.src_off == 0 &&
       (conv ? d.n_taps == 1 : true) && !(h->flags & (GP_GELU | GP_GELU_BWD | GP_GELU_KEEP)) && d.K / GP_BK >= 6) {
     const int cus = gp_cu_count();
     const long long tiles = (long long)((d.M + 255) / 256) * ((d.N + 127) / 128);
@@ -377,7 +416,7 @@
       }
     }
   }
-  const unsigned walk_wgs = (gp_schedule() == 3 && nz == 1 && blocks > (long long)gp_cu_count()) ? (unsigned)(gp_cu_count() & ~7) : 0u;
+  const unsigned walk_wgs = (gp_schedule() == 3 && !src2 && nz == 1 && blocks > (long long)gp_cu_count()) ? (unsigned)(gp_cu_count() & ~7) : 0u;
   if (tm == 256 && tn >= 128 && gp_schedule() >= 1 && rart_gemm_pair_pp_launch(&d, tn, conv, grid.x, grid.y, st, walk_wgs)) {
     RART_CHECK_LAUNCH("rart_gemm_pair_bf16 (ping-pong)");
     return RART_OK;
@@ -393,14 +432,17 @@
       grid2 = dim3((uint32_t)((mt2 >= 16 ? (mt2 + 7) / 8 * 8 : mt2) * n_tiles), nz);
     }
   }
-#define RART_GP_LAUNCH(TM_, TN_, CONV_) hipLaunchKernelGGL((k_gemm_pair<TM_, TN_, CONV_>), grid2, dim3(TM_ * 2), 0, st, d)
-#define RART_GP_BY_TN(TM_, CONV_)                                          \
+#define RART_GP_LAUNCH(TM_, TN_, ...) hipLaunchKernelGGL((k_gemm_pair<TM_, TN_, __VA_ARGS__>), grid2, dim3(TM_ * 2), 0, st, d)
+#define RART_GP_BY_TN(TM_, ...)                                            \
   do {                                                                     \
-    if (tn == 64) RART_GP_LAUNCH(TM_, 64, CONV_);                          \
-    else if (tn == 128) RART_GP_LAUNCH(TM_, 128, CONV_);                   \
-    else RART_GP_LAUNCH(TM_, 256, CONV_);                                  \
+    if (tn == 64) RART_GP_LAUNCH(TM_, 64, __VA_ARGS__);                    \
+    else if (tn == 128) RART_GP_LAUNCH(TM_, 128, __VA_ARGS__);             \
+    else RART_GP_LAUNCH(TM_, 256, __VA_ARGS__);                            \
   } while (0)
-  if (conv) {
+  if (src2) {
+    if (tm == 128) RART_GP_BY_TN(128, true, true);
+    else RART_GP_BY_TN(256, true, true);
+  } else if (conv) {
     if (tm == 128) RART_GP_BY_TN(128, true);
     else RART_GP_BY_TN(256, true);
   } else {
@@ -412,3 +454,12 @@
   RART_CHECK_LAUNCH("rart_gemm_pair_bf16");
   return RART_OK;
 }
+
+extern "C" int rart_gemm_pair_bf16(const rart_gemm_pair_desc* h, rart_stream_t stream) { return gp_launch(h, nullptr, stream); }
+
+extern "C" int rart_gemm_pair2_bf16(const rart_gemm_pair2_desc* h, rart_stream_t stream) {
+  RART_CHECK_ARG(h != nullptr, "rart_gemm_pair2_bf16: null descriptor");
+  RART_CHECK_ARG((h->a2_hi == nullptr) == (h->a2_lo == nullptr), "rart_gemm_pair2_bf16: the second source is a pair: both planes or none");
+  return gp_launch(&h->one, h->a2_hi ? h : nullptr, stream);
+}
+extern "C" int rart_gemm_pair_max_sources(void) { return 2; }
diff --git a/robustart_amd/csrc/gemm_pair_pp.hip b/robustart_amd/csrc/gemm_pair_pp.hip
--- a/robustart_amd/csrc/gemm_pair_pp.hip
+++ b/robustart_amd/csrc/gemm_pair_pp.hip
@@ -39,9 +39,10 @@
 #define PP_VM(N) pp_vmcnt<N>()
 #endif
 
-template <int TN, bool CONV, int OPT>
+template <int TN, bool CONV, int OPT, bool SRC2 = false>
 __global__ __launch_bounds__(512, 1) void k_gemm_pair_pp(const GemmPairDev d) {
   constexpr bool BAL = OPT & 1, WALK = OPT & 2;
+  static_assert(!SRC2 || (CONV && !WALK), "the second source is served by the conv instances that do not walk");
   constexpr int TM = 256, NW = 8, WN = TN / 64, WM = NW / WN, RW = TM / WM, MI = RW / 32, MH = MI / 2;
   static_assert(TN == 256 || TN == 128, "column tiles of 256 or 128");
   constexpr int PLANE_A = TM * 64, PLANE_B = TN * 64, STAGE = 2 * PLANE_A + 2 * PLANE_B;
@@ -105,9 +106,24 @@
     const int hh = q == 0 ? og : g;
     pr[q] = (WM == 2) ? og * 128 + hh * 64 + 16 * w4 : (2 * og + (w4 >> 1)) * 64 + hh * 32 + (w4 & 1) * 16;
   }
-  uint32_t avoff[2], nok[2];
+  uint32_t avoff[2], nok[2], avoff2[2] = {PP_OOR, PP_OOR};
   int tapreg = 0, tap_min = 0;
   const bool one_tap = !CONV || d.n_taps == 1;
+  if (SRC2) {
+#pragma unroll
+    for (int q = 0; q < 2; ++q) {
+      const int r = pr[q] + (lane >> 2);
+      const int csrc = (lane & 3) ^ ((r >> 2) & 3);
+      const int m = m0 + r;
+      if (m < d.M && r < d.tile_rows) {
+        const uint32_t t = gp_fastdiv((uint32_t)m, d.gw_magic, d.gw_shift);
+        const int ox = (int)((uint32_t)m - t * (uint32_t)d.grid_w);
+        const int n = (int)gp_fastdiv(t, d.gh_magic, d.gh_shift);
+        const int oy = (int)(t - (uint32_t)n * (uint32_t)d.grid_h);
+        avoff2[q] = (uint32_t)(((n * d.src2_h + oy * d.sy2) * d.src2_w + ox * d.sx2) * d.lda2 * 2 + csrc * 16);
+      }
+    }
+  }
   if (CONV) {
     for (int t = 0; t < d.n_taps; ++t) tap_min = min(tap_min, (d.tap_dy[t] * d.src_w + d.tap_dx[t]) * d.lda * 2);
     if (lane < d.n_taps) tapreg = (d.tap_dy[lane] * d.src_w + d.tap_dx[lane]) * d.lda * 2 - tap_min;
@@ -156,6 +172,8 @@
   RART_PP_ADDR(m0, n0)
   const pp_srd_t srd_ah = pp_make_srd(reinterpret_cast<const char*>(a_hi) + tap_min), srd_al = pp_make_srd(reinterpret_cast<const char*>(a_lo) + tap_min);
   const pp_srd_t srd_w = pp_make_srd(g ? w_lo : w_hi);
+  const pp_srd_t srd_a2h = pp_make_srd(SRC2 ? d.a2_hi : a_hi), srd_a2l = pp_make_srd(SRC2 ? d.a2_lo : a_lo);
+  const int kt1 = SRC2 ? d.kt1 : 0;
   const int w_step = (d.flags & GP_W_INTERLEAVED) ? 128 : 64;
   const uint32_t w_dst = lds_base + 2 * PLANE_A + g * PLANE_B + w4 * 1024;
   const int KT = d.K / GP_BK;
@@ -164,7 +182,11 @@
   {                                                                                                              \
     const int s_ = (ST);                                                                                         \
     const uint32_t dst_ = lds_base + (s_ & 1) * STAGE + pr[Q] * 64;                                              \
-    if (one_tap) {                                                                                               \
+    if (SRC2 && s_ >= kt1) {                                                                                     \
+      const uint32_t so_ = (uint32_t)(s_ - kt1) * 64u;                                                           \
+      pp_bload(avoff2[Q], srd_a2h, so_, dst_);                                                                   \
+      pp_bload(avoff2[Q], srd_a2l, so_, dst_ + PLANE_A);                                                         \
+    } else if (one_tap) {                                                                                               \
       const uint32_t so_ = tap0 + (uint32_t)s_ * 64u;                                                            \
       pp_bload(avoff[Q], srd_ah, so_, dst_);                                                                     \
       pp_bload(avoff[Q], srd_al, so_, dst_ + PLANE_A);                                                           \
@@ -624,6 +646,13 @@
 #endif
 template <int OPT>
 bool pp_launch_opt(const GemmPairDev& d, int tn, bool conv, dim3 grid, hipStream_t st, unsigned walk_wgs = 0) {
+  if (d.a2_hi) {
+    if (!conv || walk_wgs || (OPT & 2)) return false;
+    if (tn == 256) hipLaunchKernelGGL((k_gemm_pair_pp<256, true, OPT & 1, true>), grid, dim3(512), 0, st, d);
+    else if (tn == 128) hipLaunchKernelGGL((k_gemm_pair_pp<128, true, OPT & 1, true>), grid, dim3(512), 0, st, d);
+    else return false;
+    return true;
+  }
   if (walk_wgs && !(OPT & 2)) return pp_launch_opt<OPT | 2>(d, tn, conv, dim3(walk_wgs < grid.x ? walk_wgs : grid.x, 1), st);
   if (tn == 256) {
     if (conv) hipLaunchKernelGGL((k_gemm_pair_pp<256, true, OPT>), grid, dim3(512), 0, st, d);
diff --git a/robustart_amd/csrc/rart_gemm_pair_dev.h b/robustart_amd/csrc/rart_gemm_pair_dev.h
--- a/robustart_amd/csrc/rart_gemm_pair_dev.h
+++ b/robustart_amd/csrc/rart_gemm_pair_dev.h
@@ -28,6 +28,8 @@
   int m_begin;
   int tile_rows;
   int nt;
+  const uint16_t *a2_hi, *a2_lo;
+  int lda2, kt1, src2_h, src2_w, sy2, sx2;
 };
 __device__ __forceinline__ uint32_t gp_fastdiv(uint32_t n, uint32_t magic, uint32_t shift) {
   return (uint32_t)(((uint64_t)n * magic) >> shift);
diff --git a/robustart_amd/model/engine.py b/robustart_amd/model/engine.py
--- a/robustart_amd/model/engine.py
+++ b/robustart_amd/model/engine.py
@@ -20,6 +20,23 @@
     import torch
     t = [build(p) for p in planes]
     return _bf16(torch.cat(t + t[:1], 1) if len(t) == 2 else t[0]).to(device)
+
+
+def _cat_k(t1, k1, t2, k2):
+    import torch
+    assert t1.shape == (t2.shape[0], 3 * k1) and t2.shape[1] == 3 * k2
+    return torch.cat([t[:, i * k:(i + 1) * k] for i in range(3) for t, k in ((t1, k1), (t2, k2))], 1).contiguous()
+
+
+def fold_shortcut_tables(ca, cc, ds):
+    pow2 = lambda k: k >= 32 and (k & (k - 1)) == 0
+    if not (cc.r == 1 and cc.stride == 1 and ds.r == 1 and ds.cout == cc.cout and pow2(cc.cin) and ds.cin % 32 == 0):
+        return False
+    ds.w_cat = _cat_k(cc.w_fwd, cc.cin, ds.w_fwd, ds.cin)
+    ds.bias_cat = (cc.bias + ds.bias).contiguous()
+    if ds.stride == 1 and ca.r == 1 and ca.stride == 1 and ca.cin == ds.cin and pow2(ca.cout) and ds.cout % 32 == 0:
+        ds.w_cat_bwd = _cat_k(ca.bwd[0][2], ca.cout, ds.bwd[0][2], ds.cout)
+    return True
 
 
 class _Conv:
@@ -87,6 +104,7 @@
         self.fused_next_channels = (64,)
         self.fused_tail_channels = (64,)
         self.fused_tail_pair = True
+        self.fused_shortcut_pair = True
         self.pair_gemm_kernel = True
         self.blocks = []
         for layer in (m.layer1, m.layer2, m.layer3, m.layer4):
@@ -122,7 +140,10 @@
                 w = tab[:rows, pl * k:(pl + 1) * k]
                 out.append(w.reshape(rows // 32, 32, k // 64, 4, 2, 8).permute(2, 0, 3, 4, 1, 5).contiguous().view(-1))
             return torch.stack(out).contiguous()
+        two_sources = self.lib.rart_gemm_pair_max_sources() >= 2
         for bi, (ca, cb, cc, ds) in enumerate(self.blocks):
+            if two_sources and ds is not None and fold_shortcut_tables(ca, cc, ds) and ds.stride == 1 and ds.cin == 64 and cc.cout == 4 * cb.cout:
+                ds.tail_x = frag(ds.w_fwd, ds.cout, ds.cin)
             if not (cb.r == 3 and cb.stride == 1 and cb.pad == 1 and cb.cin == cb.cout and self.lib.rart_conv3x3_tail_pair_supported(cb.cin)):
                 continue
             if cc.cin == cb.cout and cc.cout == 4 * cb.cout and cc.r == 1 and cc.stride == 1:
@@ -336,10 +357,11 @@
 
     def _gemm(self, src, wgt, dst, batch, grid, src_hw, src_pix, k_per_tap, taps, n_cols, dst_hw, dst_pix,
               bias=None, res=None, mask=None, flags=0, stride=(1, 1), dst_stride=(1, 1), dst_off=(0, 0),
-              tap_src_off=None, sign_out=None, pair=False):
+              tap_src_off=None, sign_out=None, pair=False, src2=None):
         if pair and self.pair_gemm_kernel and len(taps) <= 16 and k_per_tap >= 32 and (k_per_tap & (k_per_tap - 1)) == 0:
             return self._gemm_pair(src, wgt, dst, batch, grid, src_hw, src_pix, k_per_tap, taps, n_cols, dst_hw, dst_pix, bias, res,
-                                   mask, flags, stride, dst_stride, dst_off, sign_out)
+                                   mask, flags, stride, dst_stride, dst_off, sign_out, src2)
+        assert src2 is None, 'a second source is served by rart_gemm_pair_bf16 only'
         dst_pair_off = res_pair_off = 0
         if pair:
             assert tap_src_off is None and src.shape[0] == 2
@@ -355,9 +377,9 @@
                                     dst_org=dst_off, tap_src_off=tap_src_off, dst_pair_off=dst_pair_off, res_pair_off=res_pair_off))
 
     def _gemm_pair(self, src, wgt, dst, batch, grid, src_hw, src_pix, k_per_tap, taps, n_cols, dst_hw, dst_pix, bias, res, mask, flags,
-                   stride, dst_stride, dst_off, sign_out):
+                   stride, dst_stride, dst_off, sign_out, src2=None):
         assert src.shape[0] == 2
-        k_tot = k_per_tap * len(taps)
+        k_tot = k_per_tap * len(taps) + (src2[4] if src2 is not None else 0)
         assert wgt.shape[1] == 3 * k_tot
         il = None
         if self.pair_w_interleaved:
@@ -369,13 +391,15 @@
             rows = batch * grid[0] * grid[1]
             nbytes = 4.0 * batch * src_hw[0] * src_hw[1] * k_per_tap + 4.0 * rows * n_cols * (2 if res is not None else 1) + 4.0 * k_tot * n_cols \
                 + rows * n_cols / 8.0 * ((mask is not None) + (sign_out is not None))
+            if src2 is not None:
+                nbytes += 4.0 * batch * src2[1][0] * src2[1][1] * src2[4]
         self._launch_pair(gemm_pair_desc(src, wgt, dst, n_cols, src_pix, 3 * k_tot, dst_pix, wgt.shape[0], bias=bias, res=res, mask_bits=mask,
                                          sign_out=sign_out, flags=flags & (F_RELU | F_OUT_F32), w_lo_off=k_tot, w_il=il, batch=batch,
                                          grid=grid, src_hw=src_hw, stride=stride, k_per_tap=k_per_tap, taps=taps, dst_hw=dst_hw,
-                                         dst_stride=dst_stride, dst_org=dst_off, tile=self.pair_tile), nbytes)
+                                         dst_stride=dst_stride, dst_org=dst_off, tile=self.pair_tile, src2=src2), nbytes)
 
     def _tail(self, src, wgt, taps, tail, dst, batch, hw, c_mid, bias_mid=None, bias_out=None, res=None, mask_mid=None, mask_out=None,
-              sign_mid=None, sign_out=None, relu=False, nxt=None):
+              sign_mid=None, sign_out=None, relu=False, nxt=None, xsrc=None):
         k_tot = 9 * c_mid
         assert src.shape[0] == 2 and wgt.shape[1] == 3 * k_tot and len(taps) == 9
         d = _lib.ConvTailDesc()
@@ -391,6 +415,9 @@
         d.relu_mid = d.relu_out = 1 if relu else 0
         for i, (dy, dx) in enumerate(taps):
             d.tap_dy[i], d.tap_dx[i] = dy, dx
+        if xsrc is not None:
+            assert res is None and c_mid == 64 and xsrc[0].shape[-1] == 64
+            d.x_hi, d.x_lo, d.tx_hi, d.tx_lo = xsrc[0][0].data_ptr(), xsrc[0][1].data_ptr(), xsrc[1][0].data_ptr(), xsrc[1][1].data_ptr()
         if nxt is not None:
             d.n_hi, d.n_lo = nxt['tab'][0].data_ptr(), nxt['tab'][1].data_ptr()
             d.dstn_hi, d.dstn_lo = nxt['dst'][0].data_ptr(), nxt['dst'][1].data_ptr()
@@ -400,9 +427,9 @@
         _lib.check(self.lib.rart_conv3x3_tail_pair(ctypes.byref(d), _lib.stream_ptr()))
         if ev is not None:
             px = batch * hw[0] * hw[1]
-            nbytes = 4.0 * px * c_mid * (1 + 4 + (4 if res is not None else 0) + (1 if nxt is not None else 0)) \
-                + 4.0 * c_mid * c_mid * (9 + 4 + (4 if nxt is not None else 0))
-            self._prof_end(ev, 3 * 2.0 * px * (k_tot * c_mid + (8 if nxt is not None else 4) * c_mid * c_mid), 'conv_tail_pair',
+            nx, xs = (1 if nxt is not None else 0), (1 if xsrc is not None else 0)
+            nbytes = 4.0 * px * c_mid * (1 + 4 + (4 if res is not None else 0) + nx + xs) + 4.0 * c_mid * c_mid * (9 + 4 + 4 * nx + 4 * xs)
+            self._prof_end(ev, 3 * 2.0 * px * (k_tot * c_mid + (4 + 4 * nx + 4 * xs) * c_mid * c_mid), 'conv_tail_pair',
                            nbytes)
 
     def _fc(self, a, w, out, m, n, k, bias=None):
@@ -647,21 +674,28 @@
             ya = get('b%d_a' % bi, lead + (xhw[0], xhw[1], ca.cout))
             if not pre_a:
                 self._conv_fwd(ca, x, xhw, ya, True, sign=sa, pair=x3)
+            fold = x3 and ds is not None and self.fused_shortcut_pair and self.pair_gemm_kernel and \
+                getattr(ds, 'tail_x' if kind == 'tail' else 'w_cat', None) is not None
             if x3:
-                sk = x if ds is None else self._shortcut_fwd(bi, ds, x, xhw, ohw, B)
+                sk = x if ds is None else (None if fold else self._shortcut_fwd(bi, ds, x, xhw, ohw, B))
             if kind == 'tail':
                 na = self.blocks[bi + 1][0] if bi + 1 < len(self.blocks) else None
                 if self.fused_next_pair and na is not None and getattr(na, 'next_fwd', None) is not None and cb.cout in self.fused_next_channels:
                     nxt = dict(tab=na.next_fwd, bias=na.bias, relu=True, dst=get('b%d_a' % (bi + 1), lead + (ohw[0], ohw[1], na.cout)),
                                sign=get('b%d_a_sign' % (bi + 1), (B, ohw[0], ohw[1], na.cout // 8), torch.uint8) if keep else None)
-                self._tail(ya, cb.w_fwd, cb.fwd_taps, cc.tail_fwd, yc, B, ohw, cb.cout, bias_mid=cb.bias, bias_out=cc.bias, res=sk,
-                           sign_mid=sb, sign_out=sc, relu=True, nxt=nxt)
+                self._tail(ya, cb.w_fwd, cb.fwd_taps, cc.tail_fwd, yc, B, ohw, cb.cout, bias_mid=cb.bias,
+                           bias_out=ds.bias_cat if fold else cc.bias, res=sk, sign_mid=sb, sign_out=sc, relu=True, nxt=nxt,
+                           xsrc=(x, ds.tail_x) if fold else None)
             else:
                 yb = get('b%d_b' % bi, lead + (ohw[0], ohw[1], cb.cout))
                 self._conv_fwd(cb, ya, xhw, yb, True, sign=sb, pair=x3)
                 if not x3:
                     sk = x if ds is None else self._shortcut_fwd(bi, ds, x, xhw, ohw, B)
-                self._conv_fwd(cc, yb, ohw, yc, True, res=sk, sign=sc, pair=x3)
+                if fold:
+                    self._gemm(yb, ds.w_cat, yc, B, ohw, ohw, cc.cin, cc.cin, cc.fwd_taps, cc.cout, ohw, cc.cout, bias=ds.bias_cat,
+                               flags=F_RELU, sign_out=sc, pair=True, src2=(x, xhw, (ds.stride, ds.stride), ca.cin, ds.cin))
+                else:
+                    self._conv_fwd(cc, yb, ohw, yc, True, res=sk, sign=sc, pair=x3)
         acts['b%d' % bi] = (x, xhw, ya, yb, yc, ohw)
         acts['b%d_masks' % bi] = (xs, sa, sb) if (bits or x3 or kind is not None) else (x, ya, yb)
         return yc, ohw, sc, nxt is not None
@@ -741,6 +775,9 @@
             self._conv_bwd(cb, dzb, ohw, dza, xhw, mask=ma, pair=x3)
             if ds is None:
                 self._conv_bwd(ca, dza, xhw, dx, xhw, res=dz, mask=mx, pair=x3)
+            elif x3 and self.fused_shortcut_pair and self.pair_gemm_kernel and getattr(ds, 'w_cat_bwd', None) is not None:
+                self._gemm(dza, ds.w_cat_bwd, dx, B, xhw, xhw, ca.cout, ca.cout, ca.bwd[0][1], ca.cin, xhw, ca.cin, mask=mx,
+                           flags=F_MASK_BITS, pair=True, src2=(dz, ohw, (1, 1), ds.cout, ds.cout))
             else:
                 self._conv_bwd(ca, dza, xhw, dx, xhw, mask=mx, pair=x3)
                 self._conv_bwd(ds, dz, ohw, dx, xhw, res=dx, mask=mx, pair=x3)
diff --git a/robustart_amd/model/engine_base.py b/robustart_amd/model/engine_base.py
--- a/robustart_amd/model/engine_base.py
+++ b/robustart_amd/model/engine_base.py
@@ -130,10 +130,11 @@
 def gemm_pair_desc(a, w, dst, N, lda, ldw, ldc, w_rows, M=0, K=0, bias=None, res=None, aux=None, mask_bits=None, sign_out=None, flags=0,
                    a_off=0, w_off=0, dst_off=0, w_lo_off=None, w_il=None, rows_per_image=0, src_rows_per_image=0, src_row_off=0,
                    dst_rows_per_image=0, dst_row_off=0, batched=None, batch=0, grid=None, src_hw=(0, 0), stride=(1, 1), k_per_tap=0,
-                   taps=(), dst_hw=(0, 0), dst_stride=(1, 1), dst_org=(0, 0), tile=(0, 0)):
-    d = _lib.GemmPairDesc()
+                   taps=(), dst_hw=(0, 0), dst_stride=(1, 1), dst_org=(0, 0), tile=(0, 0), src2=None):
+    d2 = _lib.GemmPair2Desc() if src2 is not None else None
+    d = d2.one if d2 is not None else _lib.GemmPairDesc()
     if grid is not None:
-        M, K = batch * grid[0] * grid[1], k_per_tap * len(taps)
+        M, K = batch * grid[0] * grid[1], k_per_tap * len(taps) + (src2[4] if src2 is not None else 0)
     d.a_hi, d.a_lo = a[0].data_ptr() + 2 * a_off, a[1].data_ptr() + 2 * a_off
     if w_il is not None:
         d.w_hi, d.w_lo, ldw = w_il.data_ptr(), w_il.data_ptr() + 64, 2 * K
@@ -172,6 +173,11 @@
         d.dst_oy, d.dst_ox = dst_org
     d.mask_bits, d.sign_out = _addr(mask_bits), _addr(sign_out)
     d.tile_m, d.tile_n = tile
+    if d2 is not None:
+        a2, hw2, st2, lda2, k2 = src2
+        d2.a2_hi, d2.a2_lo = a2[0].data_ptr(), a2[1].data_ptr()
+        d2.lda2, d2.k2, d2.src2_h, d2.src2_w, d2.sy2, d2.sx2 = lda2, k2, hw2[0], hw2[1], st2[0], st2[1]
+        return d2
     return d
 
 
@@ -301,7 +307,11 @@
 
     def _launch_pair(self, d, nbytes=None):
         ev = self._prof_begin()
-        _lib.check(self.lib.rart_gemm_pair_bf16(ctypes.byref(d), _lib.stream_ptr()))
+        if isinstance(d, _lib.GemmPair2Desc):
+            _lib.check(self.lib.rart_gemm_pair2_bf16(ctypes.byref(d), _lib.stream_ptr()))
+            d = d.one
+        else:
+            _lib.check(self.lib.rart_gemm_pair_bf16(ctypes.byref(d), _lib.stream_ptr()))
         if ev is not None:
             self._prof_end(ev, 3 * 2.0 * max(d.n_batched, 1) * d.M * d.N * d.K, 'gemm_pair', nbytes)
 
diff --git a/scratch/prof_engine2.py b/scratch/prof_engine2.py
--- a/scratch/prof_engine2.py
+++ b/scratch/prof_engine2.py
@@ -22,6 +22,8 @@
     M = batch * grid[0] * grid[1]; K = k_per_tap * len(taps)
     stride = kw.get('stride', (1, 1))
     src_bytes = min(src.numel() * src.element_size(), M * K * 2) if len(taps) > 1 else M * K * 2
+    if kw.get('src2') is not None:
+        K += kw['src2'][4]; src_bytes += M * kw['src2'][4] * 2
     by = src_bytes + K * n_cols * 2 + M * n_cols * (4 if kw.get('flags', 0) & 2 else 2)
     if kw.get('res') is not None: by += M * n_cols * 2
     mk = kw.get('mask')
diff --git a/scratch/sweep_shortcut_tiles.py b/scratch/sweep_shortcut_tiles.py
--- /dev/null
+++ b/scratch/sweep_shortcut_tiles.py
@@ -0,0 +1,75 @@
+import ctypes, sys, os
+sys.path.insert(0, os.path.dirname(os.path.dirname(os.path.abspath(__file__))))
+import torch
+from robustart_amd import _lib
+from robustart_amd.model.engine_base import gemm_pair_desc
+
+lib = _lib.load()
+sp = _lib.stream_ptr
+
+
+def pairt(*shape):
+    return (torch.randn(2, *shape, device='cuda') * 0.5).to(torch.bfloat16)
+
+
+def launch(d):
+    if isinstance(d, _lib.GemmPair2Desc):
+        _lib.check(lib.rart_gemm_pair2_bf16(ctypes.byref(d), sp()))
+    else:
+        _lib.check(lib.rart_gemm_pair_bf16(ctypes.byref(d), sp()))
+
+
+def timeit(descs, reps=8, groups=3):
+    for _ in range(3):
+        for d in descs:
+            launch(d)
+    torch.cuda.synchronize()
+    ts = []
+    for _ in range(groups):
+        a, b = torch.cuda.Event(enable_timing=True), torch.cuda.Event(enable_timing=True)
+        a.record()
+        for _ in range(reps):
+            for d in descs:
+                launch(d)
+        b.record()
+        torch.cuda.synchronize()
+        ts.append(a.elapsed_time(b) / reps * 1000)
+    return sorted(ts)
+
+
+B = 256
+cases = [('layer2.0 fwd', 28, 128, 2, 256, 512, False), ('layer3.0 fwd', 14, 256, 2, 512, 1024, False), ('layer4.0 fwd', 7, 512, 2, 1024, 2048, False),
+         ('layer1.0 bwd', 56, 64, 1, 256, 64, True)]
+only = sys.argv[1:] 
+for name, g, c1, s2, c2, n, bwd in cases:
+    if only and not any(o in name for o in only):
+        continue
+    a1, a2 = pairt(B, g, g, c1), pairt(B, g * s2, g * s2, c2)
+    k = c1 + c2
+    rows = max(n, 128)
+    wcat = (torch.randn(rows, 3 * k, device='cuda') * 0.05).to(torch.bfloat16)
+    w1 = (torch.randn(rows, 3 * c1, device='cuda') * 0.05).to(torch.bfloat16)
+    w2 = (torch.randn(rows, 3 * c2, device='cuda') * 0.05).to(torch.bfloat16)
+    bias = torch.randn(n, device='cuda')
+    out, sk = pairt(B, g, g, n), pairt(B, g, g, n)
+    sign = torch.zeros(B, g, g, n // 8, dtype=torch.uint8, device='cuda')
+    mask = torch.randint(0, 256, (B, g, g, n // 8), dtype=torch.uint8, device='cuda')
+    kw = dict(batch=B, grid=(g, g), dst_hw=(g, g), taps=[(0, 0)])
+    ep = dict(mask_bits=mask) if bwd else dict(bias=bias, sign_out=sign, flags=1)
+    if bwd:
+        da = gemm_pair_desc(a1, w1, out, n, c1, 3 * c1, n, rows, w_lo_off=c1, src_hw=(g, g), k_per_tap=c1, mask_bits=mask, **kw)
+        db = gemm_pair_desc(a2, w2, out, n, c2, 3 * c2, n, rows, w_lo_off=c2, src_hw=(g, g), k_per_tap=c2, res=out, mask_bits=mask, **kw)
+    else:
+        da = gemm_pair_desc(a2, w2, sk, n, c2, 3 * c2, n, rows, w_lo_off=c2, src_hw=(g * s2, g * s2), stride=(s2, s2), k_per_tap=c2, bias=bias, **kw)
+        db = gemm_pair_desc(a1, w1, out, n, c1, 3 * c1, n, rows, w_lo_off=c1, src_hw=(g, g), k_per_tap=c1, res=sk, **ep, **kw)
+    ta, tb, tab = timeit([da]), timeit([db]), timeit([da, db])
+    print('%s  M=%d K=%d+%d N=%d: separate %s + %s us, back to back %s us' % (name, B * g * g, c1, c2, n, ['%.0f' % t for t in ta], ['%.0f' % t for t in tb], ['%.0f' % t for t in tab]), flush=True)
+    for tile in ((0, 0), (256, 64), (128, 64), (128, 128), (256, 128), (256, 256), (224, 256), (224, 128)):
+        if tile[1] > max(n, 64) and tile != (0, 0):
+            continue
+        d = gemm_pair_desc(a1, wcat, out, n, c1, 3 * k, n, rows, w_lo_off=k, src_hw=(g, g), k_per_tap=c1, tile=tile,
+                           src2=(a2, (g * s2, g * s2), (s2, s2), c2, c2), **ep, **kw)
+        t = timeit([d])
+        print('    fused tile_m x tile_n = %3d x %3d: %s us' % (tile[0], tile[1], ['%.0f' % x for x in t]), flush=True)
+    del a1, a2, out, sk
+    torch.cuda.empty_cache()
```

Measured after the change: 8881 images/s, median of 6. 4.3% higher.
